# GrafikXxxxxxxYyyyyyyyyyy/StableDiffusion

Measured on AMD Instinct MI355X. Metric: denoise-loop latents/s (512px, 50-step DDIM, batch 4), higher is better.
Workload: dtype f16; 1 GPU; SD1.5 512x512, 50-step DDIM, batch 4/GPU, CFG on (UNet batch 8), UNet + VAE decode HIP kernels; global_batch=4, parallelism=dp1

## Files before the change

include/sd_engine.h:

```cpp
#ifndef SD_ENGINE_H
#define SD_ENGINE_H

#include <stdint.h>

#ifdef __cplusplus
extern "C" {
#endif

#define SD_OK 0
#define SD_ERR_INVALID 1
#define SD_ERR_STATE 2
#define SD_ERR_HIP 3
#define SD_ERR_UNSUPPORTED 4

#define SD_DTYPE_F16 0
#define SD_DTYPE_F32 1

#define SD_MAX_BLOCKS 4

typedef struct sd_unet_config {
    int32_t in_channels;
    int32_t out_channels;
    int32_t num_blocks;
    int32_t block_out_channels[SD_MAX_BLOCKS];
// ... 49 lines not shown
int sd_unet_num_weights(const sd_unet* u);
int sd_unet_weight_info(const sd_unet* u, int index, const char** key, int64_t* shape4, int* ndim);
int sd_unet_set_weight(sd_unet* u, const char* diffusers_key, const void* data,
                       const int64_t* shape, int ndim, int dtype);
int sd_unet_finalize(sd_unet* u);
int sd_unet_forward(sd_unet* u, const void* sample, const float* timesteps, const void* ehs,
                    int ehs_len, const void* add_text, const float* add_time_ids, void* out,
                    int B, int H, int W, void* stream);
int sd_unet_use_graph(sd_unet* u, int enable);
int sd_unet_text_kv_cache(sd_unet* u, int enable);
int sd_unet_forward_ex(sd_unet* u, const void* sample, const float* timesteps, const void* ehs, int ehs_len,
                       const void* add_text, const float* add_time_ids, const void* image_embeds, int n_img, void* out,
                       int B, int H, int W, void* stream);
int sd_unet_set_ip_adapter(sd_unet* u, sd_ip_adapter* adapter);
int sd_unet_set_ip_adapter_scale(sd_unet* u, float scale);
int sd_unet_set_controlnet(sd_unet* u, sd_controlnet* cn);
int sd_unet_forward_cn(sd_unet* u, const void* sample, const float* timesteps, const void* ehs, int ehs_len,
                       const void* add_text, const float* add_time_ids, const void* image_embeds, int n_img,
                       const void* control_image, int n_ctrl, float cond_scale, void* out, int B, int H, int W,
                       void* stream);
int sd_unet_forward_cfg(sd_unet* u, const void* latents, const float* timesteps, const void* ehs, int ehs_len,
                        const void* add_text, const float* add_time_ids, const void* image_embeds, int n_img,
                        float in_scale, int share, void* out, int B, int H, int W, void* stream);
int sd_unet_cfg_share(const sd_unet_config* cfg);
int sd_unet_set_freeu(sd_unet* u, int enable, float s1, float s2, float b1, float b2);
int sd_unet_memory(const sd_unet* u, int64_t* weight_bytes, int64_t* workspace_bytes);

int sd_ip_adapter_create(const sd_unet* u, int image_embed_dim, int num_tokens, sd_ip_adapter** out);
int sd_ip_adapter_destroy(sd_ip_adapter* a);
int sd_ip_adapter_num_weights(const sd_ip_adapter* a);
int sd_ip_adapter_weight_info(const sd_ip_adapter* a, int index, const char** key, int64_t* shape4, int* ndim);
int sd_ip_adapter_set_weight(sd_ip_adapter* a, const char* key, const void* data, const int64_t* shape, int ndim,
                             int dtype);
int sd_ip_adapter_finalize(sd_ip_adapter* a);

int sd_controlnet_create(const sd_unet* u, const sd_unet_config* cn_cfg, int conditioning_channels, sd_controlnet** out);
int sd_controlnet_destroy(sd_controlnet* cn);
int sd_controlnet_num_weights(const sd_controlnet* cn);
int sd_controlnet_weight_info(const sd_controlnet* cn, int index, const char** key, int64_t* shape4, int* ndim);
int sd_controlnet_set_weight(sd_controlnet* cn, const char* key, const void* data, const int64_t* shape, int ndim,
                             int dtype);
int sd_controlnet_finalize(sd_controlnet* cn);

int sd_vae_create(const sd_vae_config* cfg, sd_vae** out);
int sd_vae_destroy(sd_vae* v);
int sd_vae_num_weights(const sd_vae* v);
int sd_vae_weight_info(const sd_vae* v, int index, const char** key, int64_t* shape4, int* ndim);
int sd_vae_set_weight(sd_vae* v, const char* diffusers_key, const void* data,
                      const int64_t* shape, int ndim, int dtype);
int sd_vae_finalize(sd_vae* v);
int sd_vae_decode(sd_vae* v, const void* z, void* img, int B, int h, int w, void* stream);
int sd_vae_encode(sd_vae* v, const void* img, void* moments, int B, int H, int W, void* stream);
int sd_vae_encode_range_shift(sd_vae* v, int shift);
int sd_vae_memory(const sd_vae* v, int64_t* weight_bytes, int64_t* workspace_bytes);

int sd_clip_create(const sd_clip_config* cfg, sd_clip** out);
int sd_clip_destroy(sd_clip* c);
int sd_clip_num_weights(const sd_clip* c);
int sd_clip_weight_info(const sd_clip* c, int index, const char** key, int64_t* shape4, int* ndim);
int sd_clip_set_weight(sd_clip* c, const char* key, const void* data, const int64_t* shape, int ndim, int dtype);
int sd_clip_finalize(sd_clip* c);
int sd_clip_forward(sd_clip* c, const int32_t* input_ids, const int32_t* eos_index, void* hidden_states,
                    void* last_hidden, void* pooled, void* text_embeds, int B, int T, void* stream);
int sd_clip_final_layer_norm(sd_clip* c, const void* x, void* y, int64_t rows, void* stream);
int sd_clip_memory(const sd_clip* c, int64_t* weight_bytes, int64_t* workspace_bytes);

int sd_cfg_duplicate(const void* latents, void* out2b, int64_t n_per_batch, int B, float in_scale,
                     void* stream);
int sd_cfg_ddim_step(const void* noise_pred_2b, void* latents, int64_t n, float guidance_scale,
                     float c_x, float c_eps, void* stream);

int sd_cfg_linear_step(const void* noise_pred_2b, void* latents, float* hist_f32, int64_t n,
                       float guidance_scale, float c_x, float c_eps, float c_hist, float h_x, float h_eps,
                       void* stream);

int sd_cfg_rescale_linear_step(const void* noise_pred_2b, void* latents, float* hist_f32, int B, int64_t n_per_sample,
                               float guidance_scale, float guidance_rescale, float c_x, float c_eps, float c_hist,
                               float h_x, float h_eps, float* factors_out, void* stream);

int sd_inpaint_blend(void* latents, const void* image_latents, const void* noise, const void* mask,
                     float a, float b, int B, int C, int H, int W, void* stream);

int sd_images_to_uint8(const void* images_nchw_f16, void* out_nhwc_u8, int B, int C, int H, int W, void* stream);

typedef struct sd_prof_entry {
    char kernel[64];
    double flops;
    double bytes;
    double ms;
    int64_t launches;
} sd_prof_entry;
int sd_prof_enable(int on);
int sd_prof_collect(sd_prof_entry* out, int max_entries, int* n_entries);

int sd_probe_mfma(int iters, float* tflops, void* stream);
int sd_probe_copy(int64_t bytes, int iters, float* gbs, void* stream);
int sd_probe_lds_dma(int64_t region_bytes, int passes, int depth, int shared, float* gbs, void* stream);

int sd_igemm_force(int variant, int splits);
int sd_igemm_plan(const int* geom, const int* flags, int64_t* out, char* name);

int sd_op_conv2d(const void* x_nhwc, const void* w_oihw, const void* bias, const void* rowadd,
                 const void* res_nhwc, void* y_nhwc, int N, int H, int W, int Cin, int Cout,
                 int ksize, int stride, int upsample2x, int geglu, void* stream);
int sd_op_conv3x3_small_cout(const void* x_nhwc, const void* w_oihw, const void* bias, void* y_nchw, int N, int H,
                             int W, int Cin, int Cout, void* stream);
int sd_op_conv2d_groupnorm(const void* x_nhwc, const void* w_oihw, const void* bias, const void* rowadd,
                           const void* res_nhwc, void* y_conv_nhwc, const void* gamma, const void* beta,
                           void* y_gn_nhwc, int N, int H, int W, int Cin, int Cout, int ksize, int stride,
                           int upsample2x, int groups, float eps, int silu, int* stats_from_epilogue, void* stream);
int sd_op_groupnorm_conv2d(const void* x_nhwc, const void* gamma, const void* beta, int groups, float eps, int silu,
                           const void* w_oihw, const void* bias, const void* rowadd, const void* res_nhwc, void* y_nhwc,
                           int N, int H, int W, int Cin, int Cout, int ksize, int iters, float* ms_per_launch, int* fused,
                           void* stream);
int sd_op_unet_conv_in(const void* x_nchw, const void* w_oihw, const void* bias, void* y_nhwc, float* gn_summaries, int groups,
                       int N, int Cin, int H, int W, int Cout, int iters, float* ms_per_launch, void* stream);
int sd_op_unet_conv_out(const void* x_nhwc, const void* gamma, const void* beta, int groups, float eps, int silu,
                        const void* w_oihw, const void* bias, void* y_nchw, int N, int H, int W, int C, int Cout, int iters,
                        float* ms_per_launch, void* stream);
int sd_op_ffn_geglu(const void* x, const void* ln_gamma, const void* ln_beta, float ln_eps, const void* w1, const void* b1,
                    const void* w2, const void* b2, void* y, int M, int C, int iters, float* ms_per_launch, int* fused,
                    void* stream);
int sd_op_linear_rowstats(const void* x, const void* w0, const void* b0, const void* res, void* y1, float* stat, int M,
                          int K, int C, int* parts, int* part_w, int* producer, void* stream);
int sd_op_ln_linear(const void* y1, const float* stat, int parts, int part_w, const void* gamma, const void* beta, float eps,
                    const void* w1, const void* b1, void* y2, int M, int C, int O, int geglu, int rows_scaled, float row_scale,
                    int* consumer, void* stream);
int sd_op_ln_ffn_geglu(const void* x, const float* stat, int parts, int part_w, const void* ln_gamma, const void* ln_beta,
                       float ln_eps, const void* w1, const void* b1, const void* w2, const void* b2, void* y, int M, int C,
                       int* fused, void* stream);
int sd_bench_conv2d(const void* x_nhwc, const void* w_oihw, void* y_nhwc, int N, int H, int W, int Cin,
                    int Cout, int ksize, int stride, int upsample2x, int geglu, int iters,
                    float* ms_per_launch, void* stream);
int sd_op_groupnorm(const void* x_nhwc, const void* gamma, const void* beta, void* y_nhwc,
                    int N, int HW, int C, int groups, float eps, int silu, void* stream);
int sd_op_groupnorm_concat(const void* x_nhwc, int Ca, int Cb, const void* gamma, const void* beta, void* y_nhwc, int N, int HW,
                           int groups, float eps, int silu, void* stream);
int sd_bench_groupnorm(const void* x_nhwc, const void* gamma, const void* beta, void* y_nhwc,
                       int N, int HW, int C, int groups, float eps, int silu, int iters,
                       float* ms_per_launch, void* stream);
int sd_op_timestep_sinusoid(const float* t, float* out, int count, int dim, int flip_sin_to_cos, float freq_shift,
                            void* stream);
int sd_op_small_linear(const float* x, const void* w_f16, const float* bias, float* y, int B, int K, int n_out,
                       int silu_in, int silu_out, void* stream);
int sd_op_freeu(void* cat_nhwc, int N, int H, int W, int C1, int C2, float b, float s, void* stream);
int sd_op_layernorm(const void* x, const void* gamma, const void* beta, void* y, int rows, int C,
                    float eps, void* stream);
int sd_op_attention(const void* q, const void* k, const void* v, void* out, int B, int Tq, int Tk,
                    int heads, int d, int ldq, int ldk, int ldv, int ldo, void* stream);
int sd_op_attention_ex(const void* q, const void* k, const void* v, void* out, int B, int Tq, int Tk,
                       int heads, int d, int ldq, int ldk, int ldv, int ldo, int causal, int prescaled,
                       void* stream);
int sd_attention_plan(int B, int Tq, int Tk, int heads, int d, int causal, int prescaled, int* out5);
int sd_op_ip_cross_attention(const void* q, const void* k, const void* v, const void* k_ip, const void* v_ip, void* out,
                             int B, int Tq, int L, int T_ip, int heads, int d, int ldq, int ldk, int ldv, int ldk_ip,
                             int ldv_ip, int ldo, float ip_scale, int prescaled, int iters, float* ms_per_launch,
                             void* stream);

typedef struct sd_cn_problem {
    const void* x; int64_t ldx;
    const void* w;
    const float* bias;
    void* y; int64_t ldy;
    int M, C;
} sd_cn_problem;
int sd_op_controlnet_residuals(const sd_cn_problem* problems, int count, float scale, int mode, int iters,
                               float* ms_per_launch, void* stream);
int sd_op_controlnet_cond_embed(sd_controlnet* cn, const void* image, int n, int H, int W, void* out, int iters,
                                float* ms_per_launch, void* stream);

#ifdef __cplusplus
}
#endif
#endif
```

stablediffusion_amd/_lib.py:

```python
from __future__ import annotations

import ctypes as C
import os

_HERE = os.path.dirname(os.path.abspath(__file__))
LIB_PATH = os.path.join(_HERE, "libsd_engine.so")

SD_MAX_BLOCKS = 4
SD_DTYPE_F16 = 0
SD_DTYPE_F32 = 1


class SdUNetConfig(C.Structure):
    _fields_ = [
        ("in_channels", C.c_int32),
        ("out_channels", C.c_int32),
        ("num_blocks", C.c_int32),
        ("block_out_channels", C.c_int32 * SD_MAX_BLOCKS),
        ("down_block_has_attn", C.c_int32 * SD_MAX_BLOCKS),
        ("up_block_has_attn", C.c_int32 * SD_MAX_BLOCKS),
        ("num_heads", C.c_int32 * SD_MAX_BLOCKS),
        ("transformer_layers", C.c_int32 * SD_MAX_BLOCKS),
        ("layers_per_block", C.c_int32),
        ("cross_attention_dim", C.c_int32),
        ("use_linear_projection", C.c_int32),
        ("norm_num_groups", C.c_int32),
        ("norm_eps", C.c_float),
        ("flip_sin_to_cos", C.c_int32),
        ("freq_shift", C.c_float),
        ("addition_time_embed_dim", C.c_int32),
        ("projection_class_embeddings_input_dim", C.c_int32),
    ]


class SdVAEConfig(C.Structure):
    _fields_ = [
        ("in_channels", C.c_int32),
        ("out_channels", C.c_int32),
        ("latent_channels", C.c_int32),
        ("num_blocks", C.c_int32),
        ("block_out_channels", C.c_int32 * SD_MAX_BLOCKS),
        ("layers_per_block", C.c_int32),
        ("norm_num_groups", C.c_int32),
    ]


class SdClipConfig(C.Structure):
    _fields_ = [
        ("vocab_size", C.c_int32),
        ("hidden_size", C.c_int32),
        ("intermediate_size", C.c_int32),
        ("num_layers", C.c_int32),
        ("num_heads", C.c_int32),
        ("max_positions", C.c_int32),
        ("hidden_act", C.c_int32),
        ("projection_dim", C.c_int32),
        ("layer_norm_eps", C.c_float),
    ]


class SdProfEntry(C.Structure):
    _fields_ = [("kernel", C.c_char * 64), ("flops", C.c_double), ("bytes", C.c_double),
                ("ms", C.c_double), ("launches", C.c_int64)]


class SdCnProblem(C.Structure):
    _fields_ = [("x", C.c_void_p), ("ldx", C.c_int64), ("w", C.c_void_p), ("bias", C.c_void_p),
                ("y", C.c_void_p), ("ldy", C.c_int64), ("M", C.c_int), ("C", C.c_int)]


_P = C.c_void_p
_I = C.c_int
_I64 = C.c_int64
_F = C.c_float
SIGNATURES = {
    "sd_last_error": (C.c_char_p, []),
    "sd_engine_version": (_I, []),
    "sd_engine_arch": (C.c_char_p, []),
    "sd_unet_create": (_I, [C.POINTER(SdUNetConfig), C.POINTER(_P)]),
    "sd_unet_destroy": (_I, [_P]),
    "sd_unet_num_weights": (_I, [_P]),
    "sd_unet_weight_info": (_I, [_P, _I, C.POINTER(C.c_char_p), C.POINTER(_I64), C.POINTER(_I)]),
    "sd_unet_set_weight": (_I, [_P, C.c_char_p, _P, C.POINTER(_I64), _I, _I]),
    "sd_unet_finalize": (_I, [_P]),
    "sd_unet_forward": (_I, [_P, _P, _P, _P, _I, _P, _P, _P, _I, _I, _I, _P]),
    "sd_unet_use_graph": (_I, [_P, _I]),
    "sd_unet_text_kv_cache": (_I, [_P, _I]),
    "sd_unet_memory": (_I, [_P, C.POINTER(_I64), C.POINTER(_I64)]),
    "sd_unet_forward_ex": (_I, [_P, _P, _P, _P, _I, _P, _P, _P, _I, _P, _I, _I, _I, _P]),
    "sd_unet_forward_cfg": (_I, [_P, _P, _P, _P, _I, _P, _P, _P, _I, _F, _I, _P, _I, _I, _I, _P]),
    "sd_unet_cfg_share": (_I, [C.POINTER(SdUNetConfig)]),
    "sd_unet_set_ip_adapter": (_I, [_P, _P]),
    "sd_unet_set_ip_adapter_scale": (_I, [_P, _F]),
    "sd_unet_set_freeu": (_I, [_P, _I, _F, _F, _F, _F]),
    "sd_ip_adapter_create": (_I, [_P, _I, _I, C.POINTER(_P)]),
    "sd_ip_adapter_destroy": (_I, [_P]),
    "sd_ip_adapter_num_weights": (_I, [_P]),
    "sd_ip_adapter_weight_info": (_I, [_P, _I, C.POINTER(C.c_char_p), C.POINTER(_I64), C.POINTER(_I)]),
    "sd_ip_adapter_set_weight": (_I, [_P, C.c_char_p, _P, C.POINTER(_I64), _I, _I]),
    "sd_ip_adapter_finalize": (_I, [_P]),
    "sd_unet_set_controlnet": (_I, [_P, _P]),
    "sd_unet_forward_cn": (_I, [_P, _P, _P, _P, _I, _P, _P, _P, _I, _P, _I, _F, _P, _I, _I, _I, _P]),
    "sd_controlnet_create": (_I, [_P, C.POINTER(SdUNetConfig), _I, C.POINTER(_P)]),
    "sd_controlnet_destroy": (_I, [_P]),
    "sd_controlnet_num_weights": (_I, [_P]),
    "sd_controlnet_weight_info": (_I, [_P, _I, C.POINTER(C.c_char_p), C.POINTER(_I64), C.POINTER(_I)]),
    "sd_controlnet_set_weight": (_I, [_P, C.c_char_p, _P, C.POINTER(_I64), _I, _I]),
    "sd_controlnet_finalize": (_I, [_P]),
    "sd_vae_create": (_I, [C.POINTER(SdVAEConfig), C.POINTER(_P)]),
    "sd_vae_destroy": (_I, [_P]),
    "sd_vae_num_weights": (_I, [_P]),
    "sd_vae_weight_info": (_I, [_P, _I, C.POINTER(C.c_char_p), C.POINTER(_I64), C.POINTER(_I)]),
    "sd_vae_set_weight": (_I, [_P, C.c_char_p, _P, C.POINTER(_I64), _I, _I]),
    "sd_vae_finalize": (_I, [_P]),
    "sd_vae_decode": (_I, [_P, _P, _P, _I, _I, _I, _P]),
    "sd_vae_encode": (_I, [_P, _P, _P, _I, _I, _I, _P]),
    "sd_vae_encode_range_shift": (_I, [_P, _I]),
    "sd_vae_memory": (_I, [_P, C.POINTER(_I64), C.POINTER(_I64)]),
    "sd_clip_create": (_I, [C.POINTER(SdClipConfig), C.POINTER(_P)]),
    "sd_clip_destroy": (_I, [_P]),
    "sd_clip_num_weights": (_I, [_P]),
    "sd_clip_weight_info": (_I, [_P, _I, C.POINTER(C.c_char_p), C.POINTER(_I64), C.POINTER(_I)]),
    "sd_clip_set_weight": (_I, [_P, C.c_char_p, _P, C.POINTER(_I64), _I, _I]),
    "sd_clip_finalize": (_I, [_P]),
    "sd_clip_forward": (_I, [_P, _P, _P, _P, _P, _P, _P, _I, _I, _P]),
    "sd_clip_final_layer_norm": (_I, [_P, _P, _P, _I64, _P]),
    "sd_clip_memory": (_I, [_P, C.POINTER(_I64), C.POINTER(_I64)]),
    "sd_op_attention_ex": (_I, [_P, _P, _P, _P, _I, _I, _I, _I, _I, _I, _I, _I, _I, _I, _I, _P]),
    "sd_cfg_duplicate": (_I, [_P, _P, _I64, _I, _F, _P]),
    "sd_cfg_ddim_step": (_I, [_P, _P, _I64, _F, _F, _F, _P]),
    "sd_inpaint_blend": (_I, [_P, _P, _P, _P, _F, _F, _I, _I, _I, _I, _P]),
    "sd_images_to_uint8": (_I, [_P, _P, _I, _I, _I, _I, _P]),
    "sd_cfg_linear_step": (_I, [_P, _P, _P, _I64, _F, _F, _F, _F, _F, _F, _P]),
    "sd_cfg_rescale_linear_step": (_I, [_P, _P, _P, _I, _I64, _F, _F, _F, _F, _F, _F, _F, _P, _P]),
    "sd_igemm_force": (_I, [_I, _I]),
    "sd_igemm_plan": (_I, [C.POINTER(_I), C.POINTER(_I), C.POINTER(_I64), C.c_char_p]),
    "sd_probe_mfma": (_I, [_I, C.POINTER(_F), _P]),
    "sd_probe_lds_dma": (_I, [_I64, _I, _I, _I, C.POINTER(_F), _P]),
    "sd_probe_copy": (_I, [_I64, _I, C.POINTER(_F), _P]),
    "sd_prof_enable": (_I, [_I]),
    "sd_prof_collect": (_I, [C.POINTER(SdProfEntry), _I, C.POINTER(_I)]),
    "sd_op_conv2d": (_I, [_P, _P, _P, _P, _P, _P, _I, _I, _I, _I, _I, _I, _I, _I, _I, _P]),
    "sd_op_conv3x3_small_cout": (_I, [_P, _P, _P, _P, _I, _I, _I, _I, _I, _P]),
    "sd_op_conv2d_groupnorm": (_I, [_P, _P, _P, _P, _P, _P, _P, _P, _P, _I, _I, _I, _I, _I, _I, _I, _I, _I, _F, _I,
                                    C.POINTER(_I), _P]),
    "sd_op_groupnorm_conv2d": (_I, [_P, _P, _P, _I, _F, _I, _P, _P, _P, _P, _P, _I, _I, _I, _I, _I, _I, _I, C.POINTER(_F),
                                    C.POINTER(_I), _P]),
    "sd_op_unet_conv_in": (_I, [_P, _P, _P, _P, _P, _I, _I, _I, _I, _I, _I, _I, C.POINTER(_F), _P]),
    "sd_op_unet_conv_out": (_I, [_P, _P, _P, _I, _F, _I, _P, _P, _P, _I, _I, _I, _I, _I, _I, C.POINTER(_F), _P]),
    "sd_op_ffn_geglu": (_I, [_P, _P, _P, _F, _P, _P, _P, _P, _P, _I, _I, _I, C.POINTER(_F), C.POINTER(_I), _P]),
    "sd_op_linear_rowstats": (_I, [_P, _P, _P, _P, _P, _P, _I, _I, _I, C.POINTER(_I), C.POINTER(_I), C.POINTER(_I), _P]),
    "sd_op_ln_linear": (_I, [_P, _P, _I, _I, _P, _P, _F, _P, _P, _P, _I, _I, _I, _I, _I, _F, C.POINTER(_I), _P]),
    "sd_op_ln_ffn_geglu": (_I, [_P, _P, _I, _I, _P, _P, _F, _P, _P, _P, _P, _P, _I, _I, C.POINTER(_I), _P]),
    "sd_bench_conv2d": (_I, [_P, _P, _P, _I, _I, _I, _I, _I, _I, _I, _I, _I, _I, C.POINTER(_F), _P]),
    "sd_op_groupnorm": (_I, [_P, _P, _P, _P, _I, _I, _I, _I, _F, _I, _P]),
    "sd_op_groupnorm_concat": (_I, [_P, _I, _I, _P, _P, _P, _I, _I, _I, _F, _I, _P]),
    "sd_bench_groupnorm": (_I, [_P, _P, _P, _P, _I, _I, _I, _I, _F, _I, _I, C.POINTER(_F), _P]),
    "sd_op_timestep_sinusoid": (_I, [_P, _P, _I, _I, _I, _F, _P]),
    "sd_op_small_linear": (_I, [_P, _P, _P, _P, _I, _I, _I, _I, _I, _P]),
    "sd_op_freeu": (_I, [_P, _I, _I, _I, _I, _I, _F, _F, _P]),
    "sd_op_layernorm": (_I, [_P, _P, _P, _P, _I, _I, _F, _P]),
    "sd_op_attention": (_I, [_P, _P, _P, _P, _I, _I, _I, _I, _I, _I, _I, _I, _I, _P]),
    "sd_attention_plan": (_I, [_I, _I, _I, _I, _I, _I, _I, C.POINTER(_I)]),
    "sd_op_ip_cross_attention": (_I, [_P, _P, _P, _P, _P, _P, _I, _I, _I, _I, _I, _I, _I, _I, _I, _I, _I, _I, _F, _I, _I,
                                      C.POINTER(_F), _P]),
    "sd_op_controlnet_residuals": (_I, [C.POINTER(SdCnProblem), _I, _F, _I, _I, C.POINTER(_F), _P]),
    "sd_op_controlnet_cond_embed": (_I, [_P, _P, _I, _I, _I, _P, _I, C.POINTER(_F), _P]),
}

_lib = None


class EngineError(RuntimeError):
    pass


def load():
    global _lib
    if _lib is not None:
        return _lib
    if not os.path.exists(LIB_PATH):
        raise EngineError(
            f"{LIB_PATH} not found: build it with `python -m stablediffusion_amd.build` "
            "(hipcc --offload-arch=gfx950). The HIP engine is mandatory; there is no CPU fallback.")
    import torch
    lib = C.CDLL(LIB_PATH)
    for name, (res, args) in SIGNATURES.items():
        fn = getattr(lib, name)
        fn.restype = res
        fn.argtypes = args
    _lib = lib
    return lib


def check(rc: int, what: str = ""):
    if rc != 0:
        msg = load().sd_last_error()
        raise EngineError(f"{what}: error {rc}: {msg.decode() if msg else '?'}")


def require_gpu():
    import torch
    if not torch.cuda.is_available():
        raise EngineError("no HIP device visible: the gfx950 engine cannot run (and nothing else will run in its place)")
```

stablediffusion_amd/build.py:

```python
from __future__ import annotations

import os
import subprocess
import sys
from concurrent.futures import ThreadPoolExecutor

HERE = os.path.dirname(os.path.abspath(__file__))
CSRC = os.path.join(HERE, "csrc")
OUT = os.path.join(HERE, "libsd_engine.so")
SOURCES = ["igemm.hip", "igemm2.hip", "igemm3.hip", "wsgemm.hip", "pgemm.hip", "ffn.hip", "edge.hip", "norm.hip", "attention.hip", "ip_attention.hip", "controlnet.hip", "freeu.hip", "misc.hip", "probe.hip", "runtime.cpp", "unet.cpp", "controlnet.cpp", "vae.cpp", "clip.cpp", "capi.cpp"]
FLAGS = ["-O3", "--offload-arch=gfx950", "-fPIC", "-std=c++17", "-Wall", "-Wno-unused-function",
         "-ffp-contract=fast", "-mllvm", "-amdgpu-mfma-vgpr-form"]


def _stale(target, deps):
    if not os.path.exists(target):
        return True
    t = os.path.getmtime(target)
    return any(os.path.getmtime(d) > t for d in deps)


def build(force: bool = False, verbose: bool = False) -> str:
    hipcc = os.environ.get("HIPCC", "/opt/rocm/bin/hipcc")
    objdir = os.path.join(HERE, "build")
    os.makedirs(objdir, exist_ok=True)
    headers = [os.path.join(CSRC, f) for f in os.listdir(CSRC) if f.endswith((".h", ".inc"))]
    headers.append(os.path.join(os.path.dirname(HERE), "include", "sd_engine.h"))
    jobs = []
    objs = []
    for src in SOURCES:
        s = os.path.join(CSRC, src)
        o = os.path.join(objdir, src + ".o")
        objs.append(o)
        if force or _stale(o, [s] + headers):
            jobs.append([hipcc, *FLAGS, "-x", "hip", "-c", s, "-o", o])

    def run(cmd):
        if verbose:
            print(" ".join(cmd), flush=True)
        r = subprocess.run(cmd, capture_output=True, text=True)
        if r.returncode != 0:
            raise RuntimeError("build failed: %s\n%s\n%s" % (" ".join(cmd), r.stdout, r.stderr))
        if verbose and r.stderr.strip():
            print(r.stderr, file=sys.stderr)

    if jobs:
        with ThreadPoolExecutor(max_workers=min(8, len(jobs))) as ex:
            list(ex.map(run, jobs))
    if jobs or force or _stale(OUT, objs):
        run([hipcc, "--offload-arch=gfx950", "-shared", "-fPIC", "-o", OUT, *objs])
    return OUT


if __name__ == "__main__":
    print(build(force="--force" in sys.argv, verbose=True))
```

stablediffusion_amd/csrc/capi.cpp:

```cpp
#include <cmath>
#include <cstdio>
#include <new>

#include "model.h"
#include <cstdlib>

using namespace sd;

struct sd_unet { UNet impl; explicit sd_unet(const sd_unet_config& c) : impl(c) {} };
struct sd_vae { VAE impl; explicit sd_vae(const sd_vae_config& c) : impl(c) {} };
struct sd_clip { CLIP impl; explicit sd_clip(const sd_clip_config& c) : impl(c) {} };
struct sd_controlnet {
    ControlNet impl;
    sd_controlnet(const sd_unet_config& c, int cc) : impl(c, cc) {}
};
struct sd_ip_adapter {
    IPAdapter impl;
    sd_ip_adapter(const sd_unet_config& c, int d, int n) : impl(c, d, n) {}
    ~sd_ip_adapter() { if (impl.attached) impl.attached->set_ip_adapter(nullptr); }
};

namespace {

int weight_info(const WeightStore& ws, int index, const char** key, int64_t* shape4, int* ndim) {
    if (index < 0 || index >= (int)ws.order.size()) { set_error("weight index out of range"); return SD_ERR_INVALID; }
    const std::string& k = ws.order[(size_t)index];
    const RawTensor& t = ws.tensors.at(k);
    *key = k.c_str();
    *ndim = (int)t.shape.size();
    for (int i = 0; i < 4; ++i) shape4[i] = i < *ndim ? t.shape[(size_t)i] : 1;
    return SD_OK;
}

bool bad_cfg(const sd_unet_config* c) {
    if (!c || c->num_blocks < 1 || c->num_blocks > SD_MAX_BLOCKS) return true;
    for (int i = 0; i < c->num_blocks; ++i) {
        if (c->block_out_channels[i] % 64 != 0 || c->block_out_channels[i] % c->norm_num_groups != 0) return true;
        if (c->num_heads[i] <= 0 || c->block_out_channels[i] % c->num_heads[i] != 0) return true;
        if ((c->down_block_has_attn[i] || c->up_block_has_attn[c->num_blocks - 1 - i]) &&
            !attention_supported(c->block_out_channels[i] / c->num_heads[i])) return true;
    }
    if (c->addition_time_embed_dim > 0) {
        const int ad = c->addition_time_embed_dim, pin = c->projection_class_embeddings_input_dim;
        if ((ad & 1) || pin % 64 != 0 || pin - 6 * ad <= 0) return true;
    }
    return c->cross_attention_dim % 64 != 0 || c->in_channels <= 0 || c->in_channels > 16;
}

bool same_topology(const sd_unet_config& a, const sd_unet_config& b) {
    if (a.in_channels != b.in_channels || a.out_channels != b.out_channels || a.num_blocks != b.num_blocks ||
        a.layers_per_block != b.layers_per_block || a.cross_attention_dim != b.cross_attention_dim ||
        a.use_linear_projection != b.use_linear_projection || a.norm_num_groups != b.norm_num_groups ||
        a.norm_eps != b.norm_eps || a.flip_sin_to_cos != b.flip_sin_to_cos || a.freq_shift != b.freq_shift ||
        a.addition_time_embed_dim != b.addition_time_embed_dim ||
        a.projection_class_embeddings_input_dim != b.projection_class_embeddings_input_dim)
        return false;
    for (int i = 0; i < SD_MAX_BLOCKS; ++i)
        if (a.block_out_channels[i] != b.block_out_channels[i] || a.down_block_has_attn[i] != b.down_block_has_attn[i] ||
            a.up_block_has_attn[i] != b.up_block_has_attn[i] || a.num_heads[i] != b.num_heads[i] ||
            a.transformer_layers[i] != b.transformer_layers[i])
            return false;
    return true;
}

bool controlnet_fits(const sd_unet_config& u, const sd_unet_config& n, std::string* why) {
    if (n.num_blocks != u.num_blocks || n.layers_per_block != u.layers_per_block) {
        *why = "num_blocks / layers_per_block differ from the UNet's";
        return false;
    }
    for (int i = 0; i < u.num_blocks; ++i)
        if (n.block_out_channels[i] != u.block_out_channels[i]) { *why = "block_out_channels differ from the UNet's"; return false; }
    if (n.cross_attention_dim != u.cross_attention_dim) { *why = "cross_attention_dim differs from the UNet's"; return false; }
    if (n.in_channels != u.in_channels) { *why = "in_channels differs from the UNet's (9-channel inpaint UNets take no ControlNet)"; return false; }
    if (n.addition_time_embed_dim != u.addition_time_embed_dim ||
        n.projection_class_embeddings_input_dim != u.projection_class_embeddings_input_dim) {
        *why = "text_time conditioning differs from the UNet's";
        return false;
    }
    return true;
}

}

extern "C" {

const char* sd_last_error(void) { return sd::last_error().c_str(); }
int sd_engine_version(void) { return 1; }
const char* sd_engine_arch(void) { return "gfx950"; }

int sd_unet_create(const sd_unet_config* cfg, sd_unet** out) {
    if (!out) { set_error("null out"); return SD_ERR_INVALID; }
    if (bad_cfg(cfg)) {
        set_error("sd_unet_create: unsupported config (channels must be multiples of 64 and of the group "
                  "count, head dims in {32,40,64,80,128,160}, cross_attention_dim % 64 == 0, text_time: even "
                  "addition_time_embed_dim and projection_class_embeddings_input_dim % 64 == 0 and > 6 x it)");
        return SD_ERR_UNSUPPORTED;
    }
    *out = new (std::nothrow) sd_unet(*cfg);
    if (!*out) { set_error("out of host memory"); return SD_ERR_INVALID; }
    return SD_OK;
}
int sd_unet_destroy(sd_unet* u) { delete u; return SD_OK; }
int sd_unet_num_weights(const sd_unet* u) { return u ? (int)u->impl.ws.order.size() : 0; }
int sd_unet_weight_info(const sd_unet* u, int index, const char** key, int64_t* shape4, int* ndim) {
    if (!u) { set_error("null handle"); return SD_ERR_INVALID; }
    return weight_info(u->impl.ws, index, key, shape4, ndim);
}
int sd_unet_set_weight(sd_unet* u, const char* key, const void* data, const int64_t* shape, int ndim, int dtype) {
    if (!u || !key || !data || !shape) { set_error("null argument"); return SD_ERR_INVALID; }
    if (u->impl.finalized) { set_error("set_weight after finalize"); return SD_ERR_STATE; }
    return u->impl.ws.set(key, data, shape, ndim, dtype);
}
int sd_unet_finalize(sd_unet* u) {
    if (!u) { set_error("null handle"); return SD_ERR_INVALID; }
    return u->impl.finalize();
}
int sd_unet_forward(sd_unet* u, const void* sample, const float* timesteps, const void* ehs, int ehs_len,
                    const void* add_text, const float* add_time_ids, void* out, int B, int H, int W,
                    void* stream) {
    if (!u || !sample || !timesteps || !ehs || !out) { set_error("null argument"); return SD_ERR_INVALID; }
    return u->impl.forward(static_cast<const half_t*>(sample), timesteps, static_cast<const half_t*>(ehs),
                           ehs_len, static_cast<const half_t*>(add_text), add_time_ids,
                           static_cast<half_t*>(out), B, H, W, static_cast<hipStream_t>(stream));
}
int sd_unet_use_graph(sd_unet* u, int enable) {
    if (!u) { set_error("null handle"); return SD_ERR_INVALID; }
    u->impl.graph_enabled = enable != 0;
    return SD_OK;
}
int sd_unet_text_kv_cache(sd_unet* u, int enable) {
    if (!u) { set_error("null handle"); return SD_ERR_INVALID; }
    u->impl.kv_cache_on = enable != 0;
    u->impl.kv_valid = false;
    u->impl.ipkv_valid = false;
    u->impl.cond_valid = false;
    u->impl.cnkv_valid = false;
    return SD_OK;
}
int sd_unet_forward_ex(sd_unet* u, const void* sample, const float* timesteps, const void* ehs, int ehs_len,
                       const void* add_text, const float* add_time_ids, const void* image_embeds, int n_img, void* out,
                       int B, int H, int W, void* stream) {
    if (!u || !sample || !timesteps || !ehs || !out) { set_error("null argument"); return SD_ERR_INVALID; }
    return u->impl.forward(static_cast<const half_t*>(sample), timesteps, static_cast<const half_t*>(ehs),
                           ehs_len, static_cast<const half_t*>(add_text), add_time_ids,
                           static_cast<half_t*>(out), B, H, W, static_cast<hipStream_t>(stream),
                           static_cast<const half_t*>(image_embeds), image_embeds ? n_img : 0);
}
int sd_unet_set_ip_adapter(sd_unet* u, sd_ip_adapter* a) {
    if (!u) { set_error("null handle"); return SD_ERR_INVALID; }
    if (a) {
        if (!a->impl.finalized) { set_error("sd_unet_set_ip_adapter: adapter not finalized"); return SD_ERR_STATE; }
        if (!same_topology(a->impl.cfg, u->impl.cfg)) {
            set_error("sd_unet_set_ip_adapter: the adapter was created for another UNet configuration");
            return SD_ERR_INVALID;
        }
    }
    u->impl.set_ip_adapter(a ? &a->impl : nullptr);
    return SD_OK;
}
int sd_unet_set_controlnet(sd_unet* u, sd_controlnet* cn) {
    if (!u) { set_error("null handle"); return SD_ERR_INVALID; }
    if (cn) {
        if (!cn->impl.finalized) { set_error("sd_unet_set_controlnet: ControlNet not finalized"); return SD_ERR_STATE; }
        std::string why;
        if (!controlnet_fits(u->impl.cfg, cn->impl.cfg, &why)) { set_error("sd_unet_set_controlnet: " + why); return SD_ERR_INVALID; }
    }
    u->impl.set_controlnet(cn ? &cn->impl : nullptr);
    return SD_OK;
}
int sd_unet_forward_cn(sd_unet* u, const void* sample, const float* timesteps, const void* ehs, int ehs_len,
                       const void* add_text, const float* add_time_ids, const void* image_embeds, int n_img,
                       const void* control_image, int n_ctrl, float cond_scale, void* out, int B, int H, int W,
                       void* stream) {
    if (!u || !sample || !timesteps || !ehs || !out) { set_error("null argument"); return SD_ERR_INVALID; }
    return u->impl.forward(static_cast<const half_t*>(sample), timesteps, static_cast<const half_t*>(ehs),
                           ehs_len, static_cast<const half_t*>(add_text), add_time_ids,
                           static_cast<half_t*>(out), B, H, W, static_cast<hipStream_t>(stream),
                           static_cast<const half_t*>(image_embeds), image_embeds ? n_img : 0,
                           static_cast<const half_t*>(control_image), control_image ? n_ctrl : 0, cond_scale);
}
int sd_unet_forward_cfg(sd_unet* u, const void* latents, const float* timesteps, const void* ehs, int ehs_len,
                        const void* add_text, const float* add_time_ids, const void* image_embeds, int n_img,
                        float in_scale, int share, void* out, int B, int H, int W, void* stream) {
    if (!u || !latents || !timesteps || !ehs || !out) { set_error("null argument"); return SD_ERR_INVALID; }
    if (!(in_scale == in_scale)) { set_error("sd_unet_forward_cfg: in_scale is NaN"); return SD_ERR_INVALID; }
    return u->impl.forward_cfg(static_cast<const half_t*>(latents), timesteps, static_cast<const half_t*>(ehs), ehs_len,
                               static_cast<const half_t*>(add_text), add_time_ids,
                               static_cast<const half_t*>(image_embeds), image_embeds ? n_img : 0, in_scale, share != 0,
                               static_cast<half_t*>(out), B, H, W, static_cast<hipStream_t>(stream));
}
int sd_unet_cfg_share(const sd_unet_config* cfg) { return cfg && sd::unet_cfg_share_eligible(*cfg) ? 1 : 0; }
int sd_unet_set_ip_adapter_scale(sd_unet* u, float scale) {
    if (!u) { set_error("null handle"); return SD_ERR_INVALID; }
    if (!(scale == scale)) { set_error("sd_unet_set_ip_adapter_scale: NaN"); return SD_ERR_INVALID; }
    u->impl.ip_scale = scale;
    return SD_OK;
}
int sd_unet_set_freeu(sd_unet* u, int enable, float s1, float s2, float b1, float b2) {
    if (!u) { set_error("null handle"); return SD_ERR_INVALID; }
    if (!enable) { u->impl.freeu_on = false; return SD_OK; }
    if (!std::isfinite(s1) || !std::isfinite(s2) || !std::isfinite(b1) || !std::isfinite(b2)) {
        set_error("sd_unet_set_freeu: s1, s2, b1, b2 must be finite");
        return SD_ERR_INVALID;
    }
    u->impl.freeu_on = true;
    u->impl.freeu_s1 = s1; u->impl.freeu_s2 = s2; u->impl.freeu_b1 = b1; u->impl.freeu_b2 = b2;
    return SD_OK;
}

int sd_ip_adapter_create(const sd_unet* u, int image_embed_dim, int num_tokens, sd_ip_adapter** out) {
    if (!u || !out) { set_error("null argument"); return SD_ERR_INVALID; }
    const sd_unet_config& c = u->impl.cfg;
    if (c.cross_attention_dim % 64 != 0) { set_error("sd_ip_adapter_create: cross_attention_dim % 64 != 0"); return SD_ERR_UNSUPPORTED; }
    if (num_tokens < 1 || num_tokens > 16) { set_error("sd_ip_adapter_create: num_tokens must be in [1, 16]"); return SD_ERR_UNSUPPORTED; }
    if (image_embed_dim <= 0 || image_embed_dim % 64 != 0) {
        set_error("sd_ip_adapter_create: image_embed_dim must be a positive multiple of 64");
        return SD_ERR_UNSUPPORTED;
    }
    for (const auto& site : unet_xattn_sites(c, true)) {
        int heads = 0;
        for (int i = 0; i < c.num_blocks; ++i)
            if (c.block_out_channels[i] == site.second) heads = c.num_heads[i];
        if (heads <= 0 || !ip_attention_supported(site.second / heads)) {
            set_error("sd_ip_adapter_create: head dim of " + site.first + " not in {32, 40, 64, 80, 160}");
            return SD_ERR_UNSUPPORTED;
        }
    }
    *out = new (std::nothrow) sd_ip_adapter(c, image_embed_dim, num_tokens);
    if (!*out) { set_error("out of host memory"); return SD_ERR_INVALID; }
    return SD_OK;
}
int sd_ip_adapter_destroy(sd_ip_adapter* a) { delete a; return SD_OK; }
int sd_ip_adapter_num_weights(const sd_ip_adapter* a) { return a ? (int)a->impl.ws.order.size() : 0; }
int sd_ip_adapter_weight_info(const sd_ip_adapter* a, int index, const char** key, int64_t* shape4, int* ndim) {
    if (!a) { set_error("null handle"); return SD_ERR_INVALID; }
    return weight_info(a->impl.ws, index, key, shape4, ndim);
}
int sd_ip_adapter_set_weight(sd_ip_adapter* a, const char* key, const void* data, const int64_t* shape, int ndim,
                             int dtype) {
    if (!a || !key || !data || !shape) { set_error("null argument"); return SD_ERR_INVALID; }
    if (a->impl.finalized) { set_error("set_weight after finalize"); return SD_ERR_STATE; }
    return a->impl.ws.set(key, data, shape, ndim, dtype);
}
int sd_ip_adapter_finalize(sd_ip_adapter* a) {
    if (!a) { set_error("null handle"); return SD_ERR_INVALID; }
    return a->impl.finalize();
}
int sd_controlnet_create(const sd_unet* u, const sd_unet_config* cn_cfg, int conditioning_channels, sd_controlnet** out) {
    if (!u || !cn_cfg || !out) { set_error("null argument"); return SD_ERR_INVALID; }
    if (conditioning_channels != 3) { set_error("sd_controlnet_create: conditioning_channels must be 3"); return SD_ERR_UNSUPPORTED; }
    sd_unet_config c = *cn_cfg;
    for (int i = 0; i < SD_MAX_BLOCKS; ++i) c.up_block_has_attn[i] = 0;
    if (bad_cfg(&c)) { set_error("sd_controlnet_create: unsupported encoder configuration"); return SD_ERR_UNSUPPORTED; }
    std::string why;
    if (!controlnet_fits(u->impl.cfg, c, &why)) { set_error("sd_controlnet_create: " + why); return SD_ERR_INVALID; }
    if (u->impl.cfg.in_channels != 4) { set_error("sd_controlnet_create: the UNet must take 4 latent channels"); return SD_ERR_INVALID; }
    if (1 + c.num_blocks * c.layers_per_block + (c.num_blocks - 1) + 1 > kCnMaxProblems) {
        set_error("sd_controlnet_create: more residual sites than one grouped launch takes (16)");
        return SD_ERR_UNSUPPORTED;
    }
    *out = new (std::nothrow) sd_controlnet(c, conditioning_channels);
    if (!*out) { set_error("out of host memory"); return SD_ERR_INVALID; }
    return SD_OK;
}
int sd_controlnet_destroy(sd_controlnet* cn) { delete cn; return SD_OK; }
int sd_controlnet_num_weights(const sd_controlnet* cn) { return cn ? (int)cn->impl.ws.order.size() : 0; }
int sd_controlnet_weight_info(const sd_controlnet* cn, int index, const char** key, int64_t* shape4, int* ndim) {
    if (!cn) { set_error("null handle"); return SD_ERR_INVALID; }
    return weight_info(cn->impl.ws, index, key, shape4, ndim);
}
int sd_controlnet_set_weight(sd_controlnet* cn, const char* key, const void* data, const int64_t* shape, int ndim,
                             int dtype) {
    if (!cn || !key || !data || !shape) { set_error("null argument"); return SD_ERR_INVALID; }
    if (cn->impl.finalized) { set_error("set_weight after finalize"); return SD_ERR_STATE; }
    return cn->impl.ws.set(key, data, shape, ndim, dtype);
}
int sd_controlnet_finalize(sd_controlnet* cn) {
    if (!cn) { set_error("null handle"); return SD_ERR_INVALID; }
    return cn->impl.finalize();
}
int sd_unet_memory(const sd_unet* u, int64_t* weight_bytes, int64_t* workspace_bytes) {
    if (!u) { set_error("null handle"); return SD_ERR_INVALID; }
    if (weight_bytes) *weight_bytes = u->impl.ws.packed_bytes();
    if (workspace_bytes) *workspace_bytes = (int64_t)u->impl.arena.capacity();
    return SD_OK;
}

int sd_vae_create(const sd_vae_config* cfg, sd_vae** out) {
    if (!out || !cfg) { set_error("null argument"); return SD_ERR_INVALID; }
    bool bad = cfg->num_blocks < 1 || cfg->num_blocks > SD_MAX_BLOCKS || cfg->latent_channels > 8;
    for (int i = 0; !bad && i < cfg->num_blocks; ++i)
        bad = cfg->block_out_channels[i] % 64 != 0;
    if (!bad) bad = !attention_supported(cfg->block_out_channels[cfg->num_blocks - 1]);
    if (bad) { set_error("sd_vae_create: unsupported config"); return SD_ERR_UNSUPPORTED; }
    *out = new (std::nothrow) sd_vae(*cfg);
    if (!*out) { set_error("out of host memory"); return SD_ERR_INVALID; }
    return SD_OK;
}
int sd_vae_destroy(sd_vae* v) { delete v; return SD_OK; }
int sd_vae_num_weights(const sd_vae* v) { return v ? (int)v->impl.ws.order.size() : 0; }
int sd_vae_weight_info(const sd_vae* v, int index, const char** key, int64_t* shape4, int* ndim) {
    if (!v) { set_error("null handle"); return SD_ERR_INVALID; }
    return weight_info(v->impl.ws, index, key, shape4, ndim);
}
int sd_vae_set_weight(sd_vae* v, const char* key, const void* data, const int64_t* shape, int ndim, int dtype) {
    if (!v || !key || !data || !shape) { set_error("null argument"); return SD_ERR_INVALID; }
    if (v->impl.finalized) { set_error("set_weight after finalize"); return SD_ERR_STATE; }
    return v->impl.ws.set(key, data, shape, ndim, dtype);
}
int sd_vae_finalize(sd_vae* v) {
    if (!v) { set_error("null handle"); return SD_ERR_INVALID; }
    return v->impl.finalize();
}
int sd_vae_decode(sd_vae* v, const void* z, void* img, int B, int h, int w, void* stream) {
    if (!v || !z || !img) { set_error("null argument"); return SD_ERR_INVALID; }
    return v->impl.decode(static_cast<const half_t*>(z), static_cast<half_t*>(img), B, h, w,
                          static_cast<hipStream_t>(stream));
}
int sd_vae_encode(sd_vae* v, const void* img, void* moments, int B, int H, int W, void* stream) {
    if (!v || !img || !moments) { set_error("null argument"); return SD_ERR_INVALID; }
    return v->impl.encode(static_cast<const half_t*>(img), static_cast<half_t*>(moments), B, H, W,
                          static_cast<hipStream_t>(stream));
}
int sd_vae_encode_range_shift(sd_vae* v, int shift) {
    if (!v || shift < 0 || shift > 14) { set_error("sd_vae_encode_range_shift: shift in 0..14"); return SD_ERR_INVALID; }
    v->impl.encode_shift = shift;
    return SD_OK;
}
int sd_vae_memory(const sd_vae* v, int64_t* weight_bytes, int64_t* workspace_bytes) {
    if (!v) { set_error("null handle"); return SD_ERR_INVALID; }
    if (weight_bytes) *weight_bytes = v->impl.ws.packed_bytes();
    if (workspace_bytes) *workspace_bytes = (int64_t)v->impl.arena.capacity();
    return SD_OK;
}

int sd_clip_create(const sd_clip_config* cfg, sd_clip** out) {
    if (!out || !cfg) { set_error("null argument"); return SD_ERR_INVALID; }
    const bool bad = cfg->vocab_size < 1 || cfg->num_layers < 1 || cfg->num_heads < 1 || cfg->max_positions < 1 ||
                     cfg->hidden_size % 64 != 0 || cfg->intermediate_size % 64 != 0 || cfg->hidden_size > 2048 ||
                     cfg->hidden_size % cfg->num_heads != 0 || !attention_supported(cfg->hidden_size / cfg->num_heads) ||
                     (cfg->hidden_act != 0 && cfg->hidden_act != 1) || cfg->projection_dim < 0;
    if (bad) { set_error("sd_clip_create: unsupported config (hidden / intermediate % 64, head dim, activation)"); return SD_ERR_UNSUPPORTED; }
    *out = new (std::nothrow) sd_clip(*cfg);
    if (!*out) { set_error("out of host memory"); return SD_ERR_INVALID; }
    return SD_OK;
}
int sd_clip_destroy(sd_clip* c) { delete c; return SD_OK; }
// ... 608 lines not shown
    const int n = timed ? iters + 2 : 1;
    for (int it = 0; it < n && !rc; ++it) {
        if (timed && it == 2) SD_HIP_CHECK(hipEventRecord(e0, s));
        rc = launch_conv_tail(p, s);
    }
    if (timed && !rc) {
        SD_HIP_CHECK(hipEventRecord(e1, s));
        SD_HIP_CHECK(hipEventSynchronize(e1));
        float ms = 0.f;
        SD_HIP_CHECK(hipEventElapsedTime(&ms, e0, e1));
        *ms_per_launch = ms / (float)iters;
    }
    if (e0) { (void)hipEventDestroy(e0); (void)hipEventDestroy(e1); }
    hipError_t e = hipStreamSynchronize(s);
    if (!rc && e != hipSuccess) { set_error(hipGetErrorString(e)); rc = SD_ERR_HIP; }
    return rc;
}

int sd_bench_conv2d(const void* x, const void* w_oihw, void* y, int N, int H, int W, int Cin, int Cout, int ksize,
                    int stride, int upsample2x, int geglu, int iters, float* ms_per_launch, void* stream) {
    if (iters < 1 || !ms_per_launch) { set_error("sd_bench_conv2d: bad arguments"); return SD_ERR_INVALID; }
    return conv2d_impl(x, w_oihw, nullptr, nullptr, nullptr, y, N, H, W, Cin, Cout, ksize, stride, upsample2x, geglu,
                       stream, iters, ms_per_launch);
}

int sd_op_groupnorm(const void* x, const void* gamma_f32, const void* beta_f32, void* y, int N, int HW, int C,
                    int groups, float eps, int silu, void* stream) {
    hipStream_t s = static_cast<hipStream_t>(stream);
    DevScope scope;
    float* scratch = nullptr;
    SD_DEV_ALLOC(scope, scratch, (size_t)gn_scratch_floats(N, HW, C, groups) * 4);
    int rc = launch_groupnorm(static_cast<const half_t*>(x), C, static_cast<const float*>(gamma_f32),
                              static_cast<const float*>(beta_f32), static_cast<half_t*>(y), C, N, HW, C, groups,
                              eps, silu, scratch, s);
    hipError_t e = hipStreamSynchronize(s);
    if (!rc && e != hipSuccess) { set_error(hipGetErrorString(e)); rc = SD_ERR_HIP; }
    return rc;
}

int sd_op_groupnorm_concat(const void* x, int Ca, int Cb, const void* gamma_f32, const void* beta_f32, void* y, int N, int HW,
                           int groups, float eps, int silu, void* stream) {
    hipStream_t s = static_cast<hipStream_t>(stream);
    const int C = Ca + Cb;
    if (!x || !gamma_f32 || !beta_f32 || !y || Ca < 8 || Cb < 8 || groups < 1 || C % groups != 0 || Cb % groups != 0) {
        set_error("sd_op_groupnorm_concat: bad arguments"); return SD_ERR_INVALID;
    }
    const int u = gn_cat_unit(Ca, Cb, groups), ub = Cb / groups;
    if (!(u >= 8 || u == 4) || (C / groups) % ub != 0 || Ca % ub != 0 || !(ub >= 8 || ub == 4)) {
        set_error("sd_op_groupnorm_concat: the halves' sub-groups do not tile the groups"); return SD_ERR_INVALID;
    }
    const int Ga = Ca / u;
    DevScope scope;
    float *sa = nullptr, *sb = nullptr, *fin = nullptr, *scratch = nullptr;
    SD_DEV_ALLOC(scope, sa, (size_t)gn_scratch_floats(N, HW, Ca, Ga) * 4);
    SD_DEV_ALLOC(scope, sb, (size_t)gn_scratch_floats(N, HW, Cb, groups) * 4);
    SD_DEV_ALLOC(scope, fin, (size_t)N * groups * 2 * 4);
    SD_DEV_ALLOC(scope, scratch, (size_t)gn_scratch_floats(N, HW, C, groups) * 4);
    const half_t* xh = static_cast<const half_t*>(x);
    GnStats sta, stb, stc;
    int rc = launch_gn_stats(xh, C, N, HW, Ca, Ga, sa, &sta, s);
    if (!rc) rc = launch_gn_stats(xh + Ca, C, N, HW, Cb, groups, sb, &stb, s);
    if (!rc) rc = launch_gn_cat_finalize(sta, Ga, Ca, stb, groups, Cb, fin, N, HW, groups, s);
    stc.part = fin; stc.S = 1; stc.rows = HW;
    if (!rc) rc = launch_groupnorm(xh, C, static_cast<const float*>(gamma_f32), static_cast<const float*>(beta_f32),
                                   static_cast<half_t*>(y), C, N, HW, C, groups, eps, silu, scratch, s, &stc);
    hipError_t e = hipStreamSynchronize(s);
    if (!rc && e != hipSuccess) { set_error(hipGetErrorString(e)); rc = SD_ERR_HIP; }
    return rc;
}

int sd_bench_groupnorm(const void* x, const void* gamma_f32, const void* beta_f32, void* y, int N, int HW, int C,
                       int groups, float eps, int silu, int iters, float* ms_per_launch, void* stream) {
    if (iters < 1 || !ms_per_launch) { set_error("sd_bench_groupnorm: bad arguments"); return SD_ERR_INVALID; }
    hipStream_t s = static_cast<hipStream_t>(stream);
    DevScope scope;
    float* scratch = nullptr;
    SD_DEV_ALLOC(scope, scratch, (size_t)gn_scratch_floats(N, HW, C, groups) * 4);
    hipEvent_t e0, e1;
    SD_HIP_CHECK(hipEventCreate(&e0));
    SD_HIP_CHECK(hipEventCreate(&e1));
    int rc = 0;
    static const bool apply_only = getenv("SD_GN_BENCH_APPLY") != nullptr;
    GnStats st;
    float* scratch2 = nullptr;
    if (apply_only && gn_wants_stats(HW, C, groups)) {
        SD_DEV_ALLOC(scope, scratch2, (size_t)gn_scratch_floats(N, HW, C, groups) * 4);
        rc = launch_gn_stats(static_cast<const half_t*>(x), C, N, HW, C, groups, scratch2, &st, s);
    }
    for (int i = 0; i < iters + 2 && !rc; ++i) {
        if (i == 2) (void)hipEventRecord(e0, s);
        rc = launch_groupnorm(static_cast<const half_t*>(x), C, static_cast<const float*>(gamma_f32),
                              static_cast<const float*>(beta_f32), static_cast<half_t*>(y), C, N, HW, C, groups,
                              eps, silu, scratch, s, st.part ? &st : nullptr);
    }
    (void)hipEventRecord(e1, s);
    hipError_t e = hipEventSynchronize(e1);
    float ms = 0.f;
    if (e == hipSuccess) e = hipEventElapsedTime(&ms, e0, e1);
    *ms_per_launch = ms / iters;
    (void)hipEventDestroy(e0);
    (void)hipEventDestroy(e1);
    if (!rc && e != hipSuccess) { set_error(hipGetErrorString(e)); rc = SD_ERR_HIP; }
    return rc;
}

int sd_op_timestep_sinusoid(const float* t, float* out, int count, int dim, int flip_sin_to_cos, float freq_shift,
                            void* stream) {
    if (!t || !out || count < 1 || dim < 2 || (dim & 1)) { set_error("sd_op_timestep_sinusoid: bad arguments"); return SD_ERR_INVALID; }
    return launch_timestep_sinusoid(t, 1, out, count, dim, flip_sin_to_cos, freq_shift, dim, static_cast<hipStream_t>(stream));
}

int sd_op_small_linear(const float* x, const void* w_f16, const float* bias, float* y, int B, int K, int n_out, int silu_in,
                       int silu_out, void* stream) {
    if (!x || !w_f16 || !y || B < 1 || K < 1 || n_out < 1) { set_error("sd_op_small_linear: bad arguments"); return SD_ERR_INVALID; }
    return launch_small_linear(x, K, static_cast<const half_t*>(w_f16), bias, y, n_out, B, K, n_out, silu_in, silu_out,
                               static_cast<hipStream_t>(stream));
}

int sd_op_layernorm(const void* x, const void* gamma_f32, const void* beta_f32, void* y, int rows, int C, float eps,
                    void* stream) {
    return launch_layernorm(static_cast<const half_t*>(x), C, static_cast<const float*>(gamma_f32),
                            static_cast<const float*>(beta_f32), static_cast<half_t*>(y), C, rows, C, eps,
                            static_cast<hipStream_t>(stream));
}

int sd_op_freeu(void* cat_nhwc, int N, int H, int W, int C1, int C2, float b, float s, void* stream) {
    if (!cat_nhwc) { set_error("sd_op_freeu: null argument"); return SD_ERR_INVALID; }
    return launch_freeu(static_cast<half_t*>(cat_nhwc), (long)C1 + C2, N, H, W, C1, C2, b, s, static_cast<hipStream_t>(stream));
}

int sd_op_attention(const void* q, const void* k, const void* v, void* out, int B, int Tq, int Tk, int heads, int d,
                    int ldq, int ldk, int ldv, int ldo, void* stream) {
    return launch_attention(static_cast<const half_t*>(q), static_cast<const half_t*>(k),
                            static_cast<const half_t*>(v), static_cast<half_t*>(out), B, Tq, Tk, heads, d, ldq, ldk,
                            ldv, ldo, static_cast<hipStream_t>(stream));
}

int sd_op_attention_ex(const void* q, const void* k, const void* v, void* out, int B, int Tq, int Tk, int heads, int d,
                       int ldq, int ldk, int ldv, int ldo, int causal, int prescaled, void* stream) {
    return launch_attention(static_cast<const half_t*>(q), static_cast<const half_t*>(k),
                            static_cast<const half_t*>(v), static_cast<half_t*>(out), B, Tq, Tk, heads, d, ldq, ldk,
                            ldv, ldo, static_cast<hipStream_t>(stream), causal, prescaled);
}

int sd_attention_plan(int B, int Tq, int Tk, int heads, int d, int causal, int prescaled, int* out5) {
    if (!out5) { set_error("sd_attention_plan: null argument"); return SD_ERR_INVALID; }
    const AttnPlan pl = attention_plan(B, Tq, Tk, heads, d, causal, prescaled);
    if (pl.D == 0) { set_error("attention: unsupported head dim " + std::to_string(d)); return SD_ERR_UNSUPPORTED; }
    const int o[5] = {pl.D, pl.QT, pl.KT, pl.PRESC, pl.NWV};
    for (int i = 0; i < 5; ++i) out5[i] = o[i];
    return SD_OK;
}

int sd_op_ip_cross_attention(const void* q, const void* k, const void* v, const void* k_ip, const void* v_ip, void* out,
                             int B, int Tq, int L, int T_ip, int heads, int d, int ldq, int ldk, int ldv, int ldk_ip,
                             int ldv_ip, int ldo, float ip_scale, int prescaled, int iters, float* ms_per_launch,
                             void* stream) {
    const half_t *qh = static_cast<const half_t*>(q), *kh = static_cast<const half_t*>(k), *vh = static_cast<const half_t*>(v);
    const half_t *kih = static_cast<const half_t*>(k_ip), *vih = static_cast<const half_t*>(v_ip);
    half_t* oh = static_cast<half_t*>(out);
    hipStream_t s = static_cast<hipStream_t>(stream);
    auto fused = [&]() {
        return launch_ip_attention(qh, kh, vh, kih, vih, oh, B, Tq, L, T_ip, heads, d, ldq, ldk, ldv, ldk_ip, ldv_ip, ldo,
                                   ip_scale, prescaled, s);
    };
    int rc = fused();
    if (rc || iters <= 0) return rc;
    if (!ms_per_launch) { set_error("sd_op_ip_cross_attention: ms_per_launch required with iters > 0"); return SD_ERR_INVALID; }
    if (!attention_supported(d)) { set_error("sd_op_ip_cross_attention: timing needs a head dim of the text kernel"); return SD_ERR_UNSUPPORTED; }
    half_t* tmp = nullptr;
    SD_HIP_CHECK(hipMalloc(reinterpret_cast<void**>(&tmp), (size_t)B * Tq * heads * d * sizeof(half_t)));
    const long ldt = (long)heads * d;
    auto text = [&]() {
        return launch_attention(qh, kh, vh, oh, B, Tq, L, heads, d, ldq, ldk, ldv, ldo, s, 0, prescaled);
    };
    auto unfused = [&]() {
        int r = text();
        if (!r) r = launch_attention(qh, kih, vih, tmp, B, Tq, T_ip, heads, d, ldq, ldk_ip, ldv_ip, ldt, s, 0, prescaled);
        if (!r) r = launch_axpy_f16(oh, ldo, tmp, ldt, (long)B * Tq, heads * d, ip_scale, s);
        return r;
    };
    hipEvent_t e0 = nullptr, e1 = nullptr;
    if (hipEventCreate(&e0) != hipSuccess || hipEventCreate(&e1) != hipSuccess) rc = SD_ERR_HIP;
    for (int variant = 0; variant < 3 && !rc; ++variant) {
        auto one = [&]() { return variant == 0 ? fused() : variant == 1 ? text() : unfused(); };
        for (int it = 0; it < 2 && !rc; ++it) rc = one();
        if (rc) break;
        (void)hipEventRecord(e0, s);
        for (int it = 0; it < iters && !rc; ++it) rc = one();
        (void)hipEventRecord(e1, s);
        float ms = 0.f;
        hipError_t e = hipEventSynchronize(e1);
        if (e == hipSuccess) e = hipEventElapsedTime(&ms, e0, e1);
        if (e != hipSuccess) { set_error(hipGetErrorString(e)); rc = SD_ERR_HIP; }
        ms_per_launch[variant] = ms / (float)iters;
    }
    if (!rc) rc = fused();
    if (!rc && hipStreamSynchronize(s) != hipSuccess) rc = SD_ERR_HIP;
    if (e0) (void)hipEventDestroy(e0);
    if (e1) (void)hipEventDestroy(e1);
    (void)hipFree(tmp);
    return rc;
}

}

namespace {
template <class F>
int run_op_on_arena(hipStream_t s, int iters, float* ms, F body) {
    Arena arena;
    Ctx dry{&arena, s, true};
    arena.begin(true);
    body(dry);
    if (dry.err) return dry.err;
    if (int rc = arena.reserve(arena.peak() > 0 ? arena.peak() : 256)) return rc;
    auto live = [&]() {
        Ctx c{&arena, s, false};
        arena.begin(false);
        body(c);
        return c.err;
    };
    int rc = live();
    if (!rc && iters > 0) {
        if (!ms) { set_error("ms_per_launch required with iters > 0"); return SD_ERR_INVALID; }
        hipEvent_t e0 = nullptr, e1 = nullptr;
        if (hipEventCreate(&e0) != hipSuccess || hipEventCreate(&e1) != hipSuccess) rc = SD_ERR_HIP;
        if (!rc) rc = live();
        if (!rc) (void)hipEventRecord(e0, s);
        for (int it = 0; it < iters && !rc; ++it) rc = live();
        if (!rc) {
            (void)hipEventRecord(e1, s);
            float t = 0.f;
            hipError_t e = hipEventSynchronize(e1);
            if (e == hipSuccess) e = hipEventElapsedTime(&t, e0, e1);
            if (e != hipSuccess) { set_error(hipGetErrorString(e)); rc = SD_ERR_HIP; }
            *ms = t / (float)iters;
        }
        if (e0) (void)hipEventDestroy(e0);
        if (e1) (void)hipEventDestroy(e1);
    }
    const hipError_t e = hipStreamSynchronize(s);
    if (!rc && e != hipSuccess) { set_error(hipGetErrorString(e)); rc = SD_ERR_HIP; }
    return rc;
}
}

extern "C" {

int sd_op_controlnet_residuals(const sd_cn_problem* problems, int count, float scale, int mode, int iters,
                               float* ms_per_launch, void* stream) {
    if (!problems || count < 1 || count > kCnMaxProblems) { set_error("sd_op_controlnet_residuals: 1..16 problems"); return SD_ERR_INVALID; }
    if (mode != 0 && mode != 1) { set_error("sd_op_controlnet_residuals: mode must be 0 (grouped) or 1 (unfused)"); return SD_ERR_INVALID; }
    hipStream_t s = static_cast<hipStream_t>(stream);
    CnResParams rp;
    rp.scale = scale;
    for (int i = 0; i < count; ++i) {
        const sd_cn_problem& q = problems[i];
        CnResProblem& d = rp.p[rp.count++];
        d.x = static_cast<const half_t*>(q.x); d.ldx = q.ldx; d.w = static_cast<const half_t*>(q.w); d.bias = q.bias;
        d.y = static_cast<half_t*>(q.y); d.ldy = q.ldy; d.M = q.M; d.C = q.C; d.first = rp.total;
        if (q.C <= 0 || q.C % 64 != 0 || q.M <= 0) { set_error("sd_op_controlnet_residuals: C % 64 == 0 and M >= 1 required"); return SD_ERR_UNSUPPORTED; }
        rp.total += cn_residual_tiles(q.M, q.C);
    }
    if (!cn_residual_supported(rp)) { set_error("sd_op_controlnet_residuals: unsupported strides or alignment"); return SD_ERR_UNSUPPORTED; }
    if (mode == 0) return run_op_on_arena(s, iters, ms_per_launch, [&](Ctx& c) { if (!c.dry) c.err = launch_cn_residual(rp, s); });
    std::vector<ConvW> ws((size_t)count);
    std::vector<void*> owned;
    int rc = 0;
    for (int i = 0; i < count && !rc; ++i) {
        const sd_cn_problem& q = problems[i];
        const long rows = ((long)q.C + kWeightRowPad - 1) / kWeightRowPad * kWeightRowPad;
        void *w = nullptr, *b = nullptr;
        if (hipMalloc(&w, (size_t)rows * q.C * sizeof(half_t)) != hipSuccess || hipMalloc(&b, (size_t)rows * sizeof(float)) != hipSuccess) {
            set_error("sd_op_controlnet_residuals: out of device memory"); rc = SD_ERR_HIP;
        }
        if (w) owned.push_back(w);
        if (b) owned.push_back(b);
        if (rc) break;
        if (hipMemsetAsync(w, 0, (size_t)rows * q.C * sizeof(half_t), s) != hipSuccess ||
            hipMemsetAsync(b, 0, (size_t)rows * sizeof(float), s) != hipSuccess ||
            hipMemcpyAsync(w, q.w, (size_t)q.C * q.C * sizeof(half_t), hipMemcpyDeviceToDevice, s) != hipSuccess ||
            hipMemcpyAsync(b, q.bias, (size_t)q.C * sizeof(float), hipMemcpyDeviceToDevice, s) != hipSuccess) {
            set_error("sd_op_controlnet_residuals: copy failed"); rc = SD_ERR_HIP;
        }
        ConvW& cw = ws[(size_t)i];
        cw.w = static_cast<half_t*>(w); cw.bias = static_cast<float*>(b); cw.cin = q.C; cw.cout = q.C; cw.ks = 1; cw.K = q.C;
    }
    if (!rc && scale != 0.f)
        rc = run_op_on_arena(s, iters, ms_per_launch, [&](Ctx& c) {
            for (int i = 0; i < count; ++i) {
                const sd_cn_problem& q = problems[i];
                View y(static_cast<half_t*>(q.y), q.ldy, q.C);
                ConvFuse f;
                f.acc_scale = scale; f.bias_scale = scale;
                op_conv(c, ws[(size_t)i], View(const_cast<half_t*>(static_cast<const half_t*>(q.x)), q.ldx, q.C), 1, q.M, 1,
                        y, 1, 0, nullptr, 0, &y, 0, -1, 0, &f);
            }
        });
    (void)hipStreamSynchronize(s);
    for (void* p : owned) (void)hipFree(p);
    return rc;
}

int sd_op_controlnet_cond_embed(sd_controlnet* cn, const void* image, int n, int H, int W, void* out, int iters,
                                float* ms_per_launch, void* stream) {
    if (!cn || !image || !out) { set_error("null argument"); return SD_ERR_INVALID; }
// ... 10 lines not shown
```

stablediffusion_amd/csrc/controlnet.cpp:

```cpp
#include "model.h"

namespace sd {

namespace {
const char* kCond = "controlnet_cond_embedding";
const int kCondOut[ControlNet::kCondLayers] = {16, 16, 32, 32, 96, 96, 256};
const int kCondStride[ControlNet::kCondLayers] = {1, 1, 2, 1, 2, 1, 2};
std::string cond_name(int l) { return l == 0 ? std::string(kCond) + ".conv_in" : std::string(kCond) + ".blocks." + std::to_string(l - 1); }
}

ControlNet::ControlNet(const sd_unet_config& c, int conditioning_channels) : Encoder(c), cond_channels(conditioning_channels) {
    declare_encoder();
    int cin = cond_channels;
    for (int l = 0; l < kCondLayers; ++l) {
        cond_cin[l] = cin; cond_cout[l] = kCondOut[l]; cond_stride[l] = kCondStride[l];
        ws.declare(cond_name(l) + ".weight", {kCondOut[l], cin, 3, 3});
        ws.declare(cond_name(l) + ".bias", {kCondOut[l]});
        cin = kCondOut[l];
    }
    const int c0 = cfg.block_out_channels[0];
    ws.declare(std::string(kCond) + ".conv_out.weight", {c0, cin, 3, 3});
    ws.declare(std::string(kCond) + ".conv_out.bias", {c0});
    int si = 0;
    auto zc = [&](int C) {
        const std::string p = "controlnet_down_blocks." + std::to_string(si++);
        ws.declare(p + ".weight", {C, C, 1, 1});
        ws.declare(p + ".bias", {C});
    };
    zc(c0);
    for (int i = 0; i < cfg.num_blocks; ++i) {
        for (int j = 0; j < cfg.layers_per_block; ++j) zc(cfg.block_out_channels[i]);
        if (i != cfg.num_blocks - 1) zc(cfg.block_out_channels[i]);
    }
    const int mid = cfg.block_out_channels[cfg.num_blocks - 1];
    ws.declare("controlnet_mid_block.weight", {mid, mid, 1, 1});
    ws.declare("controlnet_mid_block.bias", {mid});
}

ControlNet::~ControlNet() {
    if (attached) attached->set_controlnet(nullptr);
}

int ControlNet::finalize() {
    if (finalized) return 0;
    std::string missing;
    if (!ws.complete(&missing)) { set_error("controlnet finalize: weight not set: " + missing); return 2; }
    int rc;
    std::vector<std::string> tw, tb;
    temb_total = 0;
    kv_total = 0;
    kv_keys.clear();
    if ((rc = pack_encoder(&tw, &tb))) return rc;
    for (int l = 0; l < kCondLayers; ++l) {
        cond_w[l] = static_cast<float*>(ws.dmalloc((size_t)cond_cout[l] * cond_cin[l] * 9 * sizeof(float)));
        cond_b[l] = static_cast<float*>(ws.dmalloc((size_t)cond_cout[l] * sizeof(float)));
        if (!cond_w[l] || !cond_b[l]) return 3;
        if ((rc = launch_cn_pack_cond(ws.raw(cond_name(l) + ".weight")->dev, cond_w[l], cond_cout[l], cond_cin[l], 0))) return rc;
        if ((rc = launch_f16_to_f32(ws.raw(cond_name(l) + ".bias")->dev, cond_b[l], cond_cout[l], 0))) return rc;
    }
    if ((rc = ws.pack_conv(std::string(kCond) + ".conv_out", &cond_out))) return rc;
    zero.assign((size_t)num_skips(), ConvW());
    for (int si = 0; si < num_skips(); ++si)
        if ((rc = ws.pack_conv("controlnet_down_blocks." + std::to_string(si), &zero[(size_t)si]))) return rc;
    if ((rc = ws.pack_conv("controlnet_mid_block", &zero_mid))) return rc;
    if ((rc = ws.pack_rows(tw, tb, &temb_stack))) return rc;
    if (!kv_keys.empty() && (rc = ws.pack_rows(kv_keys, {}, &kv_all))) return rc;
    kv_keys.clear();
    SD_HIP_CHECK(hipDeviceSynchronize());
    ws.free_raw();
    finalized = true;
    return 0;
}

void ControlNet::run_cond_embed(Ctx& c, const half_t* image, int n, int H, int W, View out) {
    Arena& a = *c.arena;
    const size_t mk = a.mark();
    const half_t* x = image;
    int ih = 8 * H, iw = 8 * W;
    for (int l = 0; l < kCondLayers; ++l) {
        CnCondConvParams p;
        p.x = x; p.nchw = l == 0;
        p.w = cond_w[l]; p.bias = cond_b[l];
        p.N = n; p.IH = ih; p.IW = iw; p.Cin = cond_cin[l]; p.Cout = cond_cout[l]; p.stride = cond_stride[l]; p.silu = 1;
        p.OH = (ih - 1) / p.stride + 1; p.OW = (iw - 1) / p.stride + 1;
        half_t* y = a.alloc_h((long)n * p.OH * p.OW * p.Cout);
        p.y = y;
        if (!c.dry && !c.err) {
            const double M = (double)n * p.OH * p.OW;
            prof_open(c.stream, "cn_cond_conv_kernel", 2.0 * M * p.Cout * 9.0 * p.Cin, 2.0 * (M * p.Cout + (double)n * ih * iw * p.Cin));
            c.err = launch_cn_cond_conv(p, c.stream);
            prof_close(c.stream);
        }
        x = y; ih = p.OH; iw = p.OW;
    }
    op_conv(c, cond_out, View(const_cast<half_t*>(x), cond_cout[kCondLayers - 1], cond_cout[kCondLayers - 1]), n, H, W, out);
    a.release(mk);
}

int ControlNet::run(Ctx& c, const half_t* sample, const float* timesteps, View text_kv, int L, const half_t* add_text,
                    const float* add_time_ids, int B, int H, int W, View emb, const std::vector<View>& sites, View mid) {
    Arena& a = *c.arena;
    const int G = cfg.norm_num_groups;
    const size_t mk = a.mark();
    float* tproj = nullptr;
    if (int rc = run_temb(c, timesteps, add_text, add_time_ids, B, &tproj)) return rc;
    ctx_gnpool_init(c, B, (long)H * W, G);
    auto stat = [&](int, long HW, int C) -> GnStatBuf* { return gn_wants_stats(HW, C, G) ? ctx_gnbuf(c) : nullptr; };
    GnStatBuf* xs = nullptr;
    run_conv_in(c, sample, B, H, W, sites[0], stat(0, (long)H * W, cfg.block_out_channels[0]), &emb, &xs);
    int h = H, w = W;
    View x = run_down(c, sites[0], xs, B, h, w, text_kv, L, tproj, [&](int si) { return sites[(size_t)si]; }, stat);
    run_mid(c, x, xs, B, h, w, text_kv, L, tproj, mid);
    a.release(mk);
    return c.err;
}

void UNet::set_controlnet(ControlNet* n) {
    if (cn == n) return;
    if (cn) cn->attached = nullptr;
    if (n) {
        if (n->attached && n->attached != this) n->attached->set_controlnet(nullptr);
        n->attached = this;
    }
    cn = n;
    cond_valid = false;
    cnkv_valid = false;
    planned_key = -1;
}

int UNet::run_controlnet(Ctx& c, const half_t* sample, const float* timesteps, const half_t* ehs, int L,
                         const half_t* add_text, const float* add_time_ids, int B, int H, int W, const half_t* control,
                         int n_ctrl, const std::vector<View>& sites, View mid) {
    Arena& a = *c.arena;
    const bool go = !c.dry;
    hipStream_t s = c.stream;
    const int C0 = cn->cfg.block_out_channels[0];
    const long HWC = (long)H * W * C0;
    const bool cached = kv_cache_on && !graph_enabled && cond_cache != nullptr;
    half_t* cond = cached ? cond_cache : a.alloc_h((long)B * HWC);
    const bool hit = cached && cond_valid && cond_src == control && cond_B == B && cond_n == n_ctrl && cond_H == H &&
                     cond_W == W;
    if (c.dry || !hit) {
        cn->run_cond_embed(c, control, n_ctrl, H, W, View(cond, C0, C0));
        for (int b = n_ctrl; b < B && go && !c.err; b += n_ctrl) {
            const hipError_t e = hipMemcpyAsync(cond + (long)b * HWC, cond, (size_t)n_ctrl * HWC * sizeof(half_t),
                                                hipMemcpyDeviceToDevice, s);
            if (e != hipSuccess) { set_error(hipGetErrorString(e)); c.err = 3; }
        }
        if (cached && go && !c.err) { cond_valid = true; cond_src = control; cond_B = B; cond_n = n_ctrl; cond_H = H; cond_W = W; }
    }
    const int ctx = cfg.cross_attention_dim;
    const bool kc = kv_cache_on && !graph_enabled && cnkv_cache != nullptr;
    View kv(kc ? cnkv_cache : a.alloc_h((long)B * L * cn->kv_total), cn->kv_total, cn->kv_total);
    const bool khit = kc && cnkv_valid && cnkv_src == ehs && cnkv_B == B && cnkv_L == L;
    if (c.dry || !khit) {
        op_conv(c, cn->kv_all, View(const_cast<half_t*>(ehs), ctx, ctx), B, L, 1, kv);
        if (kc && go && !c.err) { cnkv_valid = true; cnkv_src = ehs; cnkv_B = B; cnkv_L = L; }
    }
    const View ip_kv = c.ip_kv;
    c.ip_kv = View();
    const int rc = cn->run(c, sample, timesteps, kv, L, add_text, add_time_ids, B, H, W, View(cond, C0, C0), sites, mid);
    c.ip_kv = ip_kv;
    return rc;
}

}
```

stablediffusion_amd/csrc/engine.h:

```cpp
#pragma once
#include <map>
#include <string>
#include <unordered_map>
#include <vector>

#include "kernels.h"

namespace sd {

struct View {
    half_t* p = nullptr;
    long ld = 0;
    int C = 0;
    View() {}
    View(half_t* p_, long ld_, int C_) : p(p_), ld(ld_), C(C_) {}
    View slice(int c0, int c) const { return View(p + c0, ld, c); }
};

class Arena {
  public:
    ~Arena();
    int reserve(size_t bytes);
    void begin(bool dry) { dry_ = dry; off_ = 0; if (dry) peak_ = 0; }
    void* alloc(size_t bytes);
    half_t* alloc_h(long n) { return static_cast<half_t*>(alloc((size_t)n * sizeof(half_t))); }
    float* alloc_f(long n) { return static_cast<float*>(alloc((size_t)n * sizeof(float))); }
    size_t mark() const { return off_; }
    void release(size_t m) { off_ = m; }
    size_t peak() const { return peak_; }
    size_t capacity() const { return cap_; }
    bool dry() const { return dry_; }
    bool overflow() const { return overflow_; }

  private:
    char* base_ = nullptr;
    size_t cap_ = 0, off_ = 0, peak_ = 0;
    bool dry_ = false, overflow_ = false;
};

struct ConvW {
    half_t* w = nullptr;
    float* bias = nullptr;
    int cin = 0, cout = 0, ks = 1;
    long K = 0;
    float* wsum = nullptr;
};
struct RowStat {
    float* p = nullptr;
    int parts = 0;
    int width = 0;
};
struct GnStatBuf {
    float* buf = nullptr;
    GnStats st;
};
struct ConvFuse {
    const RowStat* ln_in = nullptr;
    float ln_eps = 0.f;
    RowStat* stat_out = nullptr;
    GnStatBuf* gn_out = nullptr;
    int gn_groups = 0;
    const struct NormW* gn_in = nullptr;
    GnStats gn_in_stats;
    int gn_in_groups = 0;
    float gn_in_eps = 0.f;
    int gn_in_silu = 0;
    float acc_scale = 1.f, bias_scale = 1.f;
};
struct NormW {
    float* gamma = nullptr;
    float* beta = nullptr;
    float* gb = nullptr;
    int C = 0;
};

struct RawTensor {
    std::vector<int64_t> shape;
    half_t* dev = nullptr;
    long numel = 0;
};

class WeightStore {
  public:
    ~WeightStore();
    void declare(const std::string& key, std::vector<int64_t> shape);
    int set(const std::string& key, const void* data, const int64_t* shape, int ndim, int dtype);
    bool complete(std::string* missing) const;
    const RawTensor* raw(const std::string& key) const;
    int pack_conv(const std::string& prefix, ConvW* out, bool has_bias = true);
    int pack_rows(const std::vector<std::string>& weight_keys, const std::vector<std::string>& bias_keys,
                  ConvW* out);
    int pack_geglu(const std::string& prefix, ConvW* out);
    int pack_norm(const std::string& prefix, NormW* out);
    int fold_ln(ConvW* w, const NormW& ln, int rows_scaled, float row_scale);
    void free_raw();
    void* dmalloc(size_t bytes);
    int64_t packed_bytes() const { return packed_bytes_; }

    std::vector<std::string> order;
    std::unordered_map<std::string, RawTensor> tensors;

  private:
    int host_floats(const std::string& key, std::vector<float>* out) const;
    std::vector<void*> owned_;
    int64_t packed_bytes_ = 0;
};

struct Ctx {
    Arena* arena;
    hipStream_t stream;
    bool dry;
    int err = 0;
    static constexpr int kGnPool = 4;
    GnStatBuf gnpool[kGnPool];
    int gn_next = 0;
    int gn_groups = 0;
    View ip_kv;
    int ip_T = 0;
    float ip_scale = 1.f;
};
void ctx_gnpool_init(Ctx& c, int N, long HW_max, int G);
GnStatBuf* ctx_gnbuf(Ctx& c);

struct ProfAgg { double flops = 0, bytes = 0, ms = 0; long launches = 0; };
void prof_enable(bool on);
bool prof_enabled();
void prof_open(hipStream_t s, const char* kernel, double flops, double bytes);
void prof_close(hipStream_t s);
int prof_collect(std::map<std::string, ProfAgg>* out);

void op_conv(Ctx& c, const ConvW& w, View x, int N, int H, int W, View y, int stride = 1, int up = 0,
             const float* rowadd = nullptr, int rowadd_ld = 0, const View* res = nullptr, int geglu = 0,
             int pad = -1, int act = 0, const ConvFuse* fuse = nullptr);
inline long rowstat_floats(long M, int C) { return M * ((C + 63) / 64) * 2; }
inline long gnstat_floats(int N, long HW, int G) { const long t = (HW + 63) / 64; return (long)N * (t > 64 ? t : 64) * G * 2; }
void op_groupnorm(Ctx& c, const NormW& n, View x, View y, int N, long HW, int G, float eps, int silu,
                  const GnStatBuf* pre = nullptr);
void op_gn_conv(Ctx& c, const NormW& n, const ConvW& w, View x, int N, int H, int W, View y, int G, float eps, int silu,
                const GnStatBuf* pre, const float* rowadd = nullptr, int rowadd_ld = 0, const View* res = nullptr,
                const ConvFuse* fuse = nullptr);
void op_layernorm(Ctx& c, const NormW& n, View x, View y, long rows, float eps);
bool op_ffn_fused(Ctx& c, const ConvW& ff1, const ConvW& ff2, View x, const RowStat& x_stat, float ln_eps, long M, View y);
void op_attention(Ctx& c, View q, View k, View v, View out, int B, int Tq, int Tk, int heads, int d, int causal = 0,
                  int prescaled = 0);
void op_ip_attention(Ctx& c, View q, View k, View v, View k_ip, View v_ip, View out, int B, int Tq, int L, int T_ip,
                     int heads, int d, float ip_scale);

}
```

stablediffusion_amd/csrc/kernels.h:

```cpp
#pragma once
#include "common.h"

namespace sd {

struct IGemmParams {
    const half_t* x; long ldx;
    const half_t* w;
    const float* bias;
    const float* rowadd; int rowadd_ld;
    const half_t* res; long ldres;
    half_t* y; long ldy;
    int N, H, W, Cin;
    int OH, OW, Cout;
    int KS, stride, pad, up;
    int M, K;
    int geglu;
    int mfast = 0;
    int act = 0;
    float* rowstat_out = nullptr;
    int rowstat_parts = 0;
    const float* ln_stat = nullptr;
    int ln_parts = 0, ln_C = 0, ln_part_w = 0;
    float ln_eps = 0.f;
    const float* ln_wsum = nullptr;
    float* gnstat_out = nullptr;
    int gn_groups = 0;
    const float* gni_part = nullptr;
    int gni_S = 0;
    long gni_rows = 0;
    int gni_groups = 0;
    float gni_eps = 0.f;
    int gni_silu = 0;
    const float* gni_gb = nullptr;
    int dbg_unchecked = 0;
    float acc_scale = 1.f, bias_scale = 1.f;
};
bool igemm2_gn_fusable(const IGemmParams& p, int groups);
int launch_igemm(const IGemmParams& p, hipStream_t s);
const char* igemm_variant(const IGemmParams& p);
bool igemm2_supported(const IGemmParams& p);
void igemm2_force(int variant, int splits);
struct IGemmRequest {
    float* rowstat = nullptr;
    float* gnstat = nullptr;
    int gn_groups = 0;
    bool no_workspace = false;
};
constexpr int kKindPgemmGeglu = 100;
constexpr int kKindIgemm1 = -1;
constexpr int kKindBadVariant = -2;
struct IGemmPlan {
    int kind = kKindIgemm1;
    int variant = -1;
    int splits = 1;
    long partial_floats = 0;
    int bm = 0, bn = 0;
    bool rowstats = false;
    int rs_parts = 1, rs_part_w = 0;
    bool gnstats = false;
    int gn_rows = 0;
    bool scales_ok = false;
    char name[64] = "";
};
IGemmPlan igemm2_plan(IGemmParams& p, const IGemmRequest& rq = IGemmRequest());
int launch_igemm2(const IGemmParams& p, float* partial, hipStream_t s, const IGemmPlan* plan = nullptr);
bool igemm3_supported(const IGemmParams& p);
int launch_igemm3(const IGemmParams& p, int mfast, hipStream_t s);
constexpr int kWeightRowPad = 256;
bool wsgemm_supported(const IGemmParams& p);
int wsgemm_rowstat_parts(const IGemmParams& p);
int launch_wsgemm(const IGemmParams& p, hipStream_t s);
bool pgemm_geglu_supported(const IGemmParams& p);
int launch_pgemm_geglu(const IGemmParams& p, hipStream_t s);

struct FfnParams {
    const half_t* x; long ldx;
    half_t* y; long ldy;
    const half_t* w1; const float* b1; const float* wsum1; int w1_rows;
    const half_t* w2; const float* b2; int w2_rows;
    const float* ln_stat; int ln_parts; float ln_eps;
    int M, C, hidden;
    int ln_part_w;
};
bool ffn_fused_supported(const FfnParams& p);
int launch_ffn_fused(const FfnParams& p, hipStream_t s);

long gn_scratch_floats(int N, long HW, int C, int G);
struct GnStats {
    const float* part = nullptr;
    int S = 0;
    long rows = 0;
};
bool gn_wants_stats(long HW, int C, int G);
int launch_groupnorm(const half_t* x, long ldx, const float* gamma, const float* beta,
                     half_t* y, long ldy, int N, long HW, int C, int G, float eps, int silu,
                     float* scratch, hipStream_t s, const GnStats* pre = nullptr);
int launch_gn_stats(const half_t* x, long ldx, int N, long HW, int C, int G, float* scratch, GnStats* st, hipStream_t s);
int launch_gn_finalize(GnStats* st, float* out, int N, long HW, int C, int G, hipStream_t s);
int gn_cat_unit(int Ca, int Cb, int G);
int launch_gn_cat_finalize(const GnStats& sa, int Ga, int Ca, const GnStats& sb, int Gb, int Cb, float* out, int N, long HW, int G,
                           hipStream_t s);
int launch_layernorm(const half_t* x, long ldx, const float* gamma, const float* beta,
                     half_t* y, long ldy, long rows, int C, float eps, hipStream_t s);
int launch_row_stats(const half_t* x, long ldx, float* stat, long rows, int C, hipStream_t s);
int launch_ln_fold(half_t* w, long K, int rows, const float* gamma, const float* beta, const float* bias_in,
                   float* bias, float* wsum, int rows_scaled, float row_scale, hipStream_t s);

int launch_attention(const half_t* q, const half_t* k, const half_t* v, half_t* out,
                     int B, int Tq, int Tk, int heads, int d,
                     long ldq, long ldk, long ldv, long ldo, hipStream_t s, int causal = 0, int prescaled = 0);
bool attention_supported(int d);
struct AttnPlan { int D, QT, KT, PRESC, NWV; };
AttnPlan attention_plan(int B, int Tq, int Tk, int heads, int d, int causal, int prescaled);
int launch_ip_attention(const half_t* q, const half_t* k, const half_t* v, const half_t* kip, const half_t* vip,
                        half_t* out, int B, int Tq, int L, int Tip, int heads, int d, long ldq, long ldk, long ldv,
                        long ldki, long ldvi, long ldo, float ip_scale, int prescaled, hipStream_t s);
bool ip_attention_supported(int d);
int launch_axpy_f16(half_t* y, long ldy, const half_t* x, long ldx, long rows, int cols, float a, hipStream_t s);

constexpr int kCnMaxProblems = 16;
struct CnResProblem {
    const half_t* x = nullptr; long ldx = 0;
    const half_t* w = nullptr;
    const float* bias = nullptr;
    half_t* y = nullptr; long ldy = 0;
    int M = 0, C = 0;
    int first = 0;
};
struct CnResParams {
    CnResProblem p[kCnMaxProblems];
    int count = 0, total = 0;
    float scale = 1.f;
};
int cn_residual_tiles(int M, int C);
bool cn_residual_supported(const CnResParams& p);
int launch_cn_residual(const CnResParams& p, hipStream_t s);
struct CnCondConvParams {
    const half_t* x = nullptr; int nchw = 0;
    const float* w = nullptr; const float* bias = nullptr;
    half_t* y = nullptr;
    int N = 0, IH = 0, IW = 0, Cin = 0, OH = 0, OW = 0, Cout = 0, stride = 1, silu = 1;
};
bool cn_cond_conv_supported(const CnCondConvParams& p);
int launch_cn_cond_conv(const CnCondConvParams& p, hipStream_t s);
int launch_cn_pack_cond(const half_t* w_oihw, float* out, int O, int I, hipStream_t s);

int launch_freeu(half_t* x, long ld, int N, int H, int W, int C1, int C2, float b, float s, hipStream_t st);

int launch_timestep_sinusoid(const float* t, int t_stride, float* out, int count, int dim, int flip, float shift,
                             long out_ld, hipStream_t s);
int launch_small_linear(const float* x, long ldx, const half_t* w, const float* bias, float* y,
                        long ldy, int B, int K, int Nout, int silu_in, int silu_out, hipStream_t s);
int launch_add_f32(float* y, const float* x, long n, int silu, hipStream_t s);
int launch_f16_to_f32(const half_t* x, float* y, long n, hipStream_t s);
int launch_f32_to_f16(const float* x, half_t* y, long n, hipStream_t s);
int launch_im2col_nchw3x3(const half_t* x, half_t* col, int N, int C, int H, int W, int Kpad,
                          hipStream_t s);
int launch_nhwc_to_nchw(const half_t* x, long ldx, half_t* y, int N, long HW, int C, hipStream_t s);
int launch_nchw_to_nhwc(const half_t* x, half_t* y, long ldy, int N, long HW, int C, hipStream_t s);
int launch_pointwise_nchw(const half_t* x, const half_t* w, const float* bias, half_t* y, int N,
                          int Cin, int Cout, long HW, hipStream_t s);
constexpr long kSmallCoutMinPixels = 131072;
int launch_conv3x3_small_cout(const half_t* x, long ldx, const half_t* w, long K, const float* bias, half_t* y_nchw,
                              int N, int H, int W, int Cin, int Cout, hipStream_t s);
struct HeadParams {
    const half_t* x_nchw = nullptr;
    const half_t* w = nullptr; long K = 0;
    const float* bias = nullptr;
    half_t* y = nullptr; long ldy = 0;
    float* gnstat_out = nullptr; int G = 0;
    int N = 0, Cin = 0, H = 0, W = 0, Cout = 0;
};
bool conv_head_supported(const HeadParams& p);
int launch_conv_head(const HeadParams& p, hipStream_t s);
struct TailParams {
    const half_t* x = nullptr; long ldx = 0;
    const float* gn_part = nullptr; int gn_S = 0; long gn_rows = 0;
    int G = 0; float eps = 0.f; const float* gamma = nullptr; const float* beta = nullptr; int silu = 0;
    const half_t* w = nullptr; long K = 0; const float* bias = nullptr;
    half_t* y = nullptr;
    int N = 0, H = 0, W = 0, C = 0, Cout = 0;
};
bool conv_tail_supported(const TailParams& p);
int launch_conv_tail(const TailParams& p, hipStream_t s);
int launch_pack_conv(const half_t* w_oihw, half_t* wp, int O, int I, int KH, int KW, long Kpad,
                     hipStream_t s);
int launch_cfg_duplicate(const half_t* lat, half_t* out, long n_total, float scale, hipStream_t s);
constexpr int kRowDupMax = 8;
struct RowDupSeg {
    const void* src = nullptr;
    void* dst = nullptr;
    long ld_bytes = 0, row_bytes = 0, rows = 0;
};
int launch_row_dup(const RowDupSeg* segs, int count, hipStream_t s);
int launch_scale_copy_f16(const half_t* x, half_t* out, long n, float scale, hipStream_t s);
int launch_dup_f32(const float* x, float* out, long n, hipStream_t s);
int launch_clip_embed(const int* ids, const half_t* tok, const half_t* pos, half_t* out, int B, int T, int H, int vocab,
                      hipStream_t s);
int launch_gather_rows(const half_t* x, long ldx, const int* idx, half_t* out16, float* out32, int B, int T, int H,
                       hipStream_t s);
int launch_inpaint_blend(half_t* lat, const half_t* img, const half_t* noise, const half_t* mask, float a, float b, int B,
                         int C, long HW, hipStream_t s);
int launch_scale_f16(half_t* x, long n, float scale, hipStream_t s);
int launch_image_to_uint8(const half_t* img, unsigned char* out, int B, int C, long HW, hipStream_t s);
int launch_cfg_linear(const half_t* eps2b, half_t* lat, float* hist, long n, float g, float cx, float ce, float ch,
                      float hx, float he, hipStream_t s);
int launch_cfg_ddim(const half_t* eps2b, half_t* lat, long n, float g, float cx, float ce,
                    hipStream_t s);
int launch_cfg_rescale_linear(const half_t* eps2b, half_t* lat, float* hist, int B, long n, float g, float phi, float cx,
                              float ce, float ch, float hx, float he, float* factors, hipStream_t s);

int probe_mfma(int iters, float* tflops, hipStream_t s);
int probe_copy(long bytes, int iters, float* gbs, hipStream_t s);
int probe_dma(long region_bytes, int passes, int depth, int shared, float* gbs, hipStream_t s);

}
```

stablediffusion_amd/csrc/model.h:

```cpp
#pragma once
#include "../../include/sd_engine.h"
#include "engine.h"

#include <functional>

namespace sd {

const std::string& last_error();

struct Resnet {
    NormW n1, n2;
    ConvW c1, c2, sc;
    bool has_sc = false;
    int temb_off = -1;
    int cin = 0, cout = 0;
};
struct TBlock {
    NormW ln1, ln2, ln3;
    ConvW qkv, out1, q2, out2, ff1, ff2;
    int kv_off = 0;
    int ip_kv_off = 0;
    bool fold = false;
};
struct Xformer {
    NormW gn;
    ConvW pin, pout;
    std::vector<TBlock> blocks;
    int C = 0, heads = 1;
};
struct VaeAttn {
    NormW gn;
    ConvW qkv, out;
    int C = 0;
};

struct CfgShare {
    std::vector<RowDupSeg> segs;
};

void run_resnet(Ctx& c, const Resnet& r, View x, int N, int H, int W, View out, int G, float eps,
                const float* tproj, int tproj_ld, const GnStatBuf* x_stats = nullptr, GnStatBuf** out_stats = nullptr,
                float stream_scale = 1.f, GnStatBuf* out_buf = nullptr, int out_groups = 0);
void run_xformer(Ctx& c, const Xformer& t, View x, int N, int H, int W, View out, int G, View text_kv, int L,
                 const GnStatBuf* x_stats = nullptr, GnStatBuf** out_stats = nullptr, GnStatBuf* out_buf = nullptr,
                 int out_groups = 0, const CfgShare* share = nullptr);

struct UNet;

std::vector<std::pair<std::string, int>> unet_xattn_sites(const sd_unet_config& cfg, bool mid_last);

struct IPAdapter {
    IPAdapter(const sd_unet_config& c, int image_embed_dim, int num_tokens);
    int finalize();

    sd_unet_config cfg;
    int d_img = 0, n_tok = 0;
    WeightStore ws;
    bool finalized = false;
    ConvW proj;
    NormW norm;
    ConvW kv_all;
    int kv_total = 0;
    UNet* attached = nullptr;
};

struct Encoder {
    explicit Encoder(const sd_unet_config& c) : cfg(c) {}

    sd_unet_config cfg;
    WeightStore ws;
    ConvW conv_in, te1, te2, ae1, ae2, temb_stack;
    ConvW kv_all;
    std::vector<std::string> kv_keys;
    std::vector<std::vector<Resnet>> down_res;
    std::vector<std::vector<Xformer>> down_att;
    std::vector<ConvW> down_ds;
    Resnet mid_r0, mid_r1;
    Xformer mid_att;
    int temb_total = 0;
    int kv_total = 0;

    int num_skips() const;
    using SkipDst = std::function<View(int si)>;
    using SkipStat = std::function<GnStatBuf*(int si, long HW, int C)>;

  protected:
    void declare_encoder();
    int pack_encoder(std::vector<std::string>* tw, std::vector<std::string>* tb);
    int pack_resnet(const std::string& p, Resnet* r, std::vector<std::string>* tw, std::vector<std::string>* tb);
    int pack_xformer(const std::string& p, Xformer* x, int heads, int depth);
    int run_temb(Ctx& c, const float* timesteps, const half_t* add_text, const float* add_time_ids, int B, float** tproj,
                 int rows_alloc = 0);
    void run_conv_in(Ctx& c, const half_t* sample, int B, int H, int W, View y0, GnStatBuf* gb, const View* res,
                     GnStatBuf** xs);
    View run_down(Ctx& c, View x, GnStatBuf*& xs, int B, int& h, int& w, View text_kv, int L, const float* tproj,
                  const SkipDst& dst, const SkipStat& stat, const CfgShare* share = nullptr);
    void run_mid(Ctx& c, View x, GnStatBuf* xs, int B, int h, int w, View text_kv, int L, const float* tproj, View dst);
};

struct ControlNet : Encoder {
    ControlNet(const sd_unet_config& c, int conditioning_channels);
    ~ControlNet();
    int finalize();

    int cond_channels = 3;
    bool finalized = false;
    static constexpr int kCondLayers = 7;
    float* cond_w[kCondLayers] = {};
    float* cond_b[kCondLayers] = {};
    int cond_cin[kCondLayers] = {}, cond_cout[kCondLayers] = {}, cond_stride[kCondLayers] = {};
    ConvW cond_out;
    std::vector<ConvW> zero;
    ConvW zero_mid;
    UNet* attached = nullptr;

    void run_cond_embed(Ctx& c, const half_t* image, int n, int H, int W, View out);
    int run(Ctx& c, const half_t* sample, const float* timesteps, View text_kv, int L, const half_t* add_text,
            const float* add_time_ids, int B, int H, int W, View emb, const std::vector<View>& sites, View mid);
};

bool unet_cfg_share_eligible(const sd_unet_config& cfg);

struct CfgIn {
    const half_t* latents = nullptr;
    float in_scale = 1.f;
};

struct UNet : Encoder {
    explicit UNet(const sd_unet_config& c);
    int finalize();
    int forward_cfg(const half_t* latents, const float* timesteps, const half_t* ehs, int L, const half_t* add_text,
                    const float* add_time_ids, const half_t* image_embeds, int n_img, float in_scale, bool share,
                    half_t* out, int B, int H, int W, hipStream_t stream);
    bool cfg_share_active(bool share) const;
    char* cfg_slab = nullptr;
    size_t cfg_cap = 0;
    int forward(const half_t* sample, const float* timesteps, const half_t* ehs, int L,
                const half_t* add_text, const float* add_time_ids, half_t* out, int B, int H, int W,
                hipStream_t stream, const half_t* image_embeds = nullptr, int n_img = 0,
                const half_t* control = nullptr, int n_ctrl = 0, float cn_scale = 0.f, const CfgIn* cfg_in = nullptr);
    void set_ip_adapter(IPAdapter* a);
    void set_controlnet(ControlNet* n);

    Arena arena;
    bool finalized = false;
    long planned_key = -1;
    long planned_cn = -1;

    bool graph_enabled = false;
    hipStream_t gstream = nullptr;
    hipEvent_t ev_in = nullptr, ev_out = nullptr;
    hipGraphExec_t gexec = nullptr;
    long graph_key = -1;
    char* io_slab = nullptr;
    size_t io_cap = 0;
    int forward_graph(const half_t* sample, const float* timesteps, const half_t* ehs, int L, const half_t* add_text,
                      const float* add_time_ids, half_t* out, int B, int H, int W, hipStream_t stream);
    ~UNet();

    bool kv_cache_on = false, kv_valid = false;
    half_t* kv_cache = nullptr;
    size_t kv_cap = 0;
    const half_t* kv_src = nullptr;
    int kv_B = 0, kv_L = 0;

    IPAdapter* ip = nullptr;
    float ip_scale = 1.f;
    bool ipkv_valid = false;
    half_t* ipkv_cache = nullptr;
    size_t ipkv_cap = 0;
    const half_t* ipkv_src = nullptr;
    int ipkv_B = 0, ipkv_n = 0;

    ControlNet* cn = nullptr;
    bool cond_valid = false, cnkv_valid = false;
    half_t* cond_cache = nullptr;
    size_t cond_cap = 0;
    const half_t* cond_src = nullptr;
    int cond_B = 0, cond_n = 0, cond_H = 0, cond_W = 0;
    half_t* cnkv_cache = nullptr;
    size_t cnkv_cap = 0;
    const half_t* cnkv_src = nullptr;
    int cnkv_B = 0, cnkv_L = 0;

    bool freeu_on = false;
    float freeu_s1 = 1.f, freeu_s2 = 1.f, freeu_b1 = 1.f, freeu_b2 = 1.f;

    ConvW conv_out;
    NormW norm_out;
    std::vector<std::vector<Resnet>> up_res;
    std::vector<std::vector<Xformer>> up_att;
    std::vector<ConvW> up_us;

  private:
    int run(Ctx& c, const half_t* sample, const float* timesteps, const half_t* ehs, int L,
            const half_t* add_text, const float* add_time_ids, half_t* out, int B, int H, int W,
            const half_t* image_embeds = nullptr, int n_img = 0, const half_t* control = nullptr, int n_ctrl = 0,
            float cn_scale = 0.f, const CfgIn* cfg_in = nullptr);
    int run_controlnet(Ctx& c, const half_t* sample, const float* timesteps, const half_t* ehs, int L,
                       const half_t* add_text, const float* add_time_ids, int B, int H, int W, const half_t* control,
                       int n_ctrl, const std::vector<View>& sites, View mid);
};

struct VAE {
    explicit VAE(const sd_vae_config& c);
    int finalize();
    int decode(const half_t* z, half_t* img, int B, int h, int w, hipStream_t stream);
    int encode(const half_t* img, half_t* moments, int B, int H, int W, hipStream_t stream);
    int encode_shift = 0;

    sd_vae_config cfg;
    WeightStore ws;
    Arena arena;
    bool finalized = false;
    long planned_key = -1;

    half_t* pq_w = nullptr; float* pq_b = nullptr;
    ConvW d_conv_in, d_conv_out;
    NormW d_norm_out;
    Resnet d_mid0, d_mid1;
    VaeAttn d_attn;
    std::vector<std::vector<Resnet>> d_up;
    std::vector<ConvW> d_us;
    half_t* q_w = nullptr; float* q_b = nullptr;
    ConvW e_conv_in, e_conv_out;
    NormW e_norm_out;
    Resnet e_mid0, e_mid1;
    VaeAttn e_attn;
    std::vector<std::vector<Resnet>> e_down;
    std::vector<ConvW> e_ds;

  private:
    int pack_resnet(const std::string& p, Resnet* r);
    int pack_attn(const std::string& p, VaeAttn* a);
    int pack_pointwise(const std::string& p, half_t** w, float** b);
    void run_attn(Ctx& c, const VaeAttn& a, View x, int N, int H, int W, View out, const GnStatBuf* x_stats,
                  GnStatBuf** out_stats, float stream_scale = 1.f);
    int run_decode(Ctx& c, const half_t* z, half_t* img, int B, int h, int w);
    int run_encode(Ctx& c, const half_t* img, half_t* moments, int B, int H, int W, float stream_scale);
};

struct ClipLayer {
    NormW ln1, ln2;
    ConvW qkv, out, fc1, fc2;
};
struct CLIP {
    explicit CLIP(const sd_clip_config& c);
    int finalize();
    int forward(const int* ids, const int* eos_index, half_t* hidden_states, half_t* last_hidden, half_t* pooled,
                half_t* text_embeds, int B, int T, hipStream_t stream);
    int final_layer_norm(const half_t* x, half_t* y, long rows, hipStream_t stream);

    sd_clip_config cfg;
    WeightStore ws;
    Arena arena;
    bool finalized = false;
    long planned_key = -1;
    half_t* tok = nullptr;
    half_t* pos = nullptr;
    half_t* proj = nullptr;
    std::vector<ClipLayer> layers;
    NormW final_ln;

  private:
    int run(Ctx& c, const int* ids, const int* eos_index, half_t* hidden_states, half_t* last_hidden, half_t* pooled,
            half_t* text_embeds, int B, int T);
};

}
```

stablediffusion_amd/csrc/runtime.cpp:

```cpp
#include "engine.h"

#include <atomic>
#include <cstdio>
#include <mutex>
#include <cstdlib>
#include <cstring>

namespace sd {

static thread_local std::string g_last_error;
void set_error(const std::string& msg) { g_last_error = msg; }
const std::string& last_error() { return g_last_error; }

Arena::~Arena() {
    if (base_) (void)hipFree(base_);
}

int Arena::reserve(size_t bytes) {
    if (bytes <= cap_) return 0;
    if (base_) { (void)hipFree(base_); base_ = nullptr; cap_ = 0; }
    SD_HIP_CHECK(hipMalloc(reinterpret_cast<void**>(&base_), bytes));
    cap_ = bytes;
    return 0;
}
// ... 301 lines not shown
    GnStatBuf* gn_out = fuse ? fuse->gn_out : nullptr;
    IGemmParams p;
    p.x = x.p; p.ldx = x.ld;
    p.w = w.w; p.bias = w.bias;
    p.rowadd = rowadd; p.rowadd_ld = rowadd_ld;
    p.res = res ? res->p : nullptr; p.ldres = res ? res->ld : 0;
    p.y = y.p; p.ldy = y.ld;
    p.N = N; p.H = H; p.W = W; p.Cin = (w.ks == 1) ? (int)w.K : w.cin;
    p.KS = w.ks; p.stride = stride; p.up = up;
    p.pad = pad >= 0 ? pad : (w.ks == 3 ? 1 : 0);
    const int IH = H << up, IW = W << up;
    if (stride == 1) {
        p.OH = IH; p.OW = IW;
    } else if (p.pad == 0) {
        p.OH = (IH + 1 - w.ks) / stride + 1; p.OW = (IW + 1 - w.ks) / stride + 1;
    } else {
        p.OH = (IH + 2 * p.pad - w.ks) / stride + 1; p.OW = (IW + 2 * p.pad - w.ks) / stride + 1;
    }
    p.Cout = w.cout;
    p.M = N * p.OH * p.OW;
    p.K = (int)w.K;
    p.geglu = geglu;
    p.act = act;
    if (ln_in) {
        if (!w.wsum) { set_error("op_conv: LayerNorm statistics passed to a linear without folded weights"); c.err = 1; return; }
        p.ln_stat = ln_in->p; p.ln_parts = ln_in->parts; p.ln_part_w = ln_in->width; p.ln_C = (int)w.K; p.ln_eps = ln_eps; p.ln_wsum = w.wsum;
    }
    if (fuse && fuse->gn_in) {
        p.gni_part = fuse->gn_in_stats.part; p.gni_S = fuse->gn_in_stats.S; p.gni_rows = fuse->gn_in_stats.rows;
        p.gni_groups = fuse->gn_in_groups; p.gni_eps = fuse->gn_in_eps; p.gni_silu = fuse->gn_in_silu;
        p.gni_gb = fuse->gn_in->gb;
        if (c.dry) p.gni_part = reinterpret_cast<const float*>(8);
    }
    if (fuse && (fuse->acc_scale != 1.f || fuse->bias_scale != 1.f)) { p.acc_scale = fuse->acc_scale; p.bias_scale = fuse->bias_scale; }
    const IGemmPlan plan = igemm2_plan(p, IGemmRequest{stat_out ? stat_out->p : nullptr, gn_out ? gn_out->buf : nullptr,
                                                       fuse ? fuse->gn_groups : 0});
    const bool v2 = plan.kind != kKindIgemm1;
    if ((p.acc_scale != 1.f || p.bias_scale != 1.f) && !plan.scales_ok) { set_error("op_conv: output scaling needs the LDS-DMA kernels (not GEGLU / weight-stationary)"); c.err = 1; return; }
    if (ln_in && !v2) { set_error("op_conv: the LayerNorm fold needs the LDS-DMA kernel"); c.err = 1; return; }
    if (act && !v2) { set_error("op_conv: activation epilogue needs the LDS-DMA kernel (Cin % 64, Cout % 8)"); c.err = 1; return; }
    if (gn_out) {
        gn_out->st = GnStats();
        if (plan.gnstats) { gn_out->st.part = gn_out->buf; gn_out->st.rows = plan.gn_rows; gn_out->st.S = p.OH * p.OW / plan.gn_rows; }
    }
    const bool own_stats = plan.rowstats;
    if (stat_out) { stat_out->parts = plan.rs_parts; stat_out->width = plan.rs_part_w; }
    float* partial = plan.partial_floats > 0 ? c.arena->alloc_f(plan.partial_floats) : nullptr;
    if (c.dry || c.err) return;
    if (prof_enabled()) {
        const double kreal = (double)w.ks * w.ks * w.cin;
        const double in_px = (double)N * H * W;
        const char* name = plan.name;
        static const bool by_shape = getenv("SD_PROF_SHAPES") != nullptr;
        char nbuf[64];
        if (v2 && by_shape) {
            snprintf(nbuf, sizeof(nbuf), "%s%d/k%d %dx%dx%d ks%d%s%s%s%s%s%s", plan.kind == kKindPgemmGeglu ? "pg" : "v", plan.variant,
                     plan.splits, p.M, p.Cout, p.K, p.KS, res ? " res" : "", geglu ? " geglu" : "", p.ln_stat ? " ln" : "",
                     p.rowstat_out ? " rs" : "", p.gnstat_out ? " gs" : "", p.gni_part ? " gn" : "");
            name = nbuf;
        }
        prof_open(c.stream, name, 2.0 * p.M * w.cout * kreal,
                  2.0 * (in_px * (w.ks == 1 ? (double)w.K : w.cin) + (double)w.cout * w.K +
                         (double)p.M * (geglu ? w.cout / 2 : w.cout) * (res ? 2 : 1)));
    }
    c.err = launch_igemm2(p, partial, c.stream, &plan);
    prof_close(c.stream);
    if (stat_out && !own_stats && !c.err) {
        prof_open(c.stream, "row_stats_kernel", 0.0, 2.0 * p.M * w.cout);
        c.err = launch_row_stats(y.p, y.ld, stat_out->p, p.M, w.cout, c.stream);
        prof_close(c.stream);
    }
}

void op_groupnorm(Ctx& c, const NormW& n, View x, View y, int N, long HW, int G, float eps, int silu,
                  const GnStatBuf* pre) {
    float* scratch = c.arena->alloc_f(gn_scratch_floats(N, HW, n.C, G));
    if (c.dry || c.err) return;
    const GnStats* st = (pre && pre->st.part && gn_wants_stats(HW, n.C, G)) ? &pre->st : nullptr;
    const bool own_pass = gn_wants_stats(HW, n.C, G) && !st;
    const char* gname = own_pass ? "groupnorm(stats+apply)" : "groupnorm(apply)";
    static thread_local char gbuf[64];
    static const bool gn_by_shape = getenv("SD_PROF_SHAPES") != nullptr;
    if (gn_by_shape && prof_enabled()) {
        snprintf(gbuf, sizeof(gbuf), "gn%s %ldx%d%s", own_pass ? "(stats+apply)" : (st ? "(apply)" : "(fused)"), (long)N * HW, n.C, silu ? " silu" : "");
        gname = gbuf;
    }
    prof_open(c.stream, gname, 0.0, (own_pass ? 6.0 : 4.0) * N * HW * n.C);
    c.err = launch_groupnorm(x.p, x.ld, n.gamma, n.beta, y.p, y.ld, N, HW, n.C, G, eps, silu, scratch, c.stream, st);
    prof_close(c.stream);
}

void op_gn_conv(Ctx& c, const NormW& n, const ConvW& w, View x, int N, int H, int W, View y, int G, float eps, int silu,
                const GnStatBuf* pre, const float* rowadd, int rowadd_ld, const View* res, const ConvFuse* fuse) {
    static const bool off = getenv("SD_GN_FUSE") == nullptr || getenv("SD_NO_GN_FUSE") != nullptr;
    const long HW = (long)H * W;
    IGemmParams q;
    q.x = x.p; q.ldx = x.ld; q.N = N; q.H = H; q.W = W; q.Cin = (w.ks == 1) ? (int)w.K : w.cin;
    q.KS = w.ks; q.stride = 1; q.up = 0; q.pad = w.ks == 3 ? 1 : 0; q.OH = H; q.OW = W; q.Cout = w.cout;
    q.M = N * H * W; q.K = (int)w.K;
    const bool fused = !off && n.gb && n.C == q.Cin && igemm2_gn_fusable(q, G);
    if (!fused) {
        const size_t mk = c.arena->mark();
        View hn(c.arena->alloc_h((long)N * HW * n.C), n.C, n.C);
        op_groupnorm(c, n, x, hn, N, HW, G, eps, silu, pre);
        op_conv(c, w, hn, N, H, W, y, 1, 0, rowadd, rowadd_ld, res, 0, -1, 0, fuse);
        c.arena->release(mk);
        return;
    }
    const size_t mk = c.arena->mark();
    ConvFuse f = fuse ? *fuse : ConvFuse();
    f.gn_in = &n; f.gn_in_groups = G; f.gn_in_eps = eps; f.gn_in_silu = silu;
    float* scratch = c.arena->alloc_f(gn_scratch_floats(N, HW, n.C, G) + (long)N * G * 2);
    if (pre && pre->st.part) {
        f.gn_in_stats = pre->st;
        if (f.gn_in_stats.S > 64 && !c.dry && !c.err) {
            prof_open(c.stream, "gn_finalize_kernel", 0.0, 8.0 * N * f.gn_in_stats.S * G);
            c.err = launch_gn_finalize(&f.gn_in_stats, scratch, N, HW, n.C, G, c.stream);
            prof_close(c.stream);
        }
    } else if (!c.dry && !c.err) {
        static thread_local char gbuf[64];
        static const bool by_shape = getenv("SD_PROF_SHAPES") != nullptr;
        const char* name = "groupnorm(stats)";
        if (by_shape && prof_enabled()) { snprintf(gbuf, sizeof(gbuf), "gn(stats) %ldx%d", (long)N * HW, n.C); name = gbuf; }
        prof_open(c.stream, name, 0.0, 2.0 * N * HW * n.C);
        c.err = launch_gn_stats(x.p, x.ld, N, HW, n.C, G, scratch, &f.gn_in_stats, c.stream);
        prof_close(c.stream);
    }
    op_conv(c, w, x, N, H, W, y, 1, 0, rowadd, rowadd_ld, res, 0, -1, 0, &f);
    c.arena->release(mk);
}

bool op_ffn_fused(Ctx& c, const ConvW& ff1, const ConvW& ff2, View x, const RowStat& x_stat, float ln_eps, long M, View y) {
    FfnParams p;
    p.x = x.p; p.ldx = x.ld; p.y = y.p; p.ldy = y.ld;
    p.w1 = ff1.w; p.b1 = ff1.bias; p.wsum1 = ff1.wsum;
    p.w1_rows = (int)(((long)ff1.cout + kWeightRowPad - 1) / kWeightRowPad * kWeightRowPad);
    p.w2 = ff2.w; p.b2 = ff2.bias;
    p.w2_rows = (int)(((long)ff2.cout + kWeightRowPad - 1) / kWeightRowPad * kWeightRowPad);
    p.ln_stat = x_stat.p; p.ln_parts = x_stat.parts; p.ln_part_w = x_stat.width; p.ln_eps = ln_eps;
    p.M = (int)M; p.C = (int)ff1.K; p.hidden = (int)ff2.K;
    if (c.dry) p.ln_stat = reinterpret_cast<const float*>(8);
    if (ff1.ks != 1 || ff2.ks != 1 || ff2.cout != ff1.K || ff1.cout != 2 * ff2.K || x.C != p.C || !ff1.wsum) return false;
    if (c.dry ? !(p.C == 320 && p.hidden == 1280 && M % 128 == 0 && M / 128 >= 64 && !getenv("SD_NO_FFN_FUSE")) : !ffn_fused_supported(p))
        return false;
    if (c.dry || c.err) return true;
    prof_open(c.stream, "ffn_fused_kernel", 2.0 * M * ((double)ff1.cout * ff1.K + (double)ff2.cout * ff2.K),
              2.0 * ((double)M * p.C * 2 + (double)ff1.cout * ff1.K + (double)ff2.cout * ff2.K));
    c.err = launch_ffn_fused(p, c.stream);
    prof_close(c.stream);
    return true;
}

void op_layernorm(Ctx& c, const NormW& n, View x, View y, long rows, float eps) {
    if (c.dry || c.err) return;
    prof_open(c.stream, "layernorm_kernel", 0.0, 4.0 * rows * n.C);
    c.err = launch_layernorm(x.p, x.ld, n.gamma, n.beta, y.p, y.ld, rows, n.C, eps, c.stream);
    prof_close(c.stream);
}

void op_attention(Ctx& c, View q, View k, View v, View out, int B, int Tq, int Tk, int heads, int d, int causal,
                  int prescaled) {
    if (c.dry || c.err) return;
    if (prof_enabled()) {
        static thread_local char name[32];
        snprintf(name, sizeof(name), "attn_kernel<%d>", d);
        prof_open(c.stream, name, 4.0 * B * heads * (double)Tq * Tk * d,
                  2.0 * B * heads * d * (2.0 * Tq + 2.0 * Tk));
    }
    c.err = launch_attention(q.p, k.p, v.p, out.p, B, Tq, Tk, heads, d, q.ld, k.ld, v.ld, out.ld, c.stream, causal, prescaled);
    prof_close(c.stream);
}

void op_ip_attention(Ctx& c, View q, View k, View v, View k_ip, View v_ip, View out, int B, int Tq, int L, int T_ip,
                     int heads, int d, float ip_scale) {
    if (c.dry || c.err) return;
    if (prof_enabled()) {
        static thread_local char name[32];
        snprintf(name, sizeof(name), "ip_xattn_kernel<%d>", d);
        prof_open(c.stream, name, 4.0 * B * heads * (double)Tq * (L + T_ip) * d,
                  2.0 * B * heads * d * (2.0 * Tq + 2.0 * L + 2.0 * T_ip));
    }
    c.err = launch_ip_attention(q.p, k.p, v.p, k_ip.p, v_ip.p, out.p, B, Tq, L, T_ip, heads, d, q.ld, k.ld, v.ld, k_ip.ld,
                                v_ip.ld, out.ld, ip_scale, 1, c.stream);
    prof_close(c.stream);
}

}
```

stablediffusion_amd/csrc/unet.cpp:

```cpp
#include <algorithm>
#include <vector>

#include "model.h"
#include <cmath>
#include <cstdlib>

namespace sd {

void declare_resnet(WeightStore& ws, const std::string& p, int cin, int cout, int temb) {
    ws.declare(p + ".norm1.weight", {cin});
    ws.declare(p + ".norm1.bias", {cin});
    ws.declare(p + ".conv1.weight", {cout, cin, 3, 3});
    ws.declare(p + ".conv1.bias", {cout});
    if (temb) {
        ws.declare(p + ".time_emb_proj.weight", {cout, temb});
        ws.declare(p + ".time_emb_proj.bias", {cout});
    }
    ws.declare(p + ".norm2.weight", {cout});
    ws.declare(p + ".norm2.bias", {cout});
    ws.declare(p + ".conv2.weight", {cout, cout, 3, 3});
    ws.declare(p + ".conv2.bias", {cout});
    if (cin != cout) {
        ws.declare(p + ".conv_shortcut.weight", {cout, cin, 1, 1});
        ws.declare(p + ".conv_shortcut.bias", {cout});
// ... 74 lines not shown
    declare_xformer(ws, "mid_block.attentions.0", mid, cfg.transformer_layers[nb - 1], ctx, lin);
    declare_resnet(ws, "mid_block.resnets.1", mid, mid, temb);
}

UNet::UNet(const sd_unet_config& c) : Encoder(c) {
    declare_encoder();
    const int nb = cfg.num_blocks;
    const int* boc = cfg.block_out_channels;
    const int temb = boc[0] * 4;
    const int ctx = cfg.cross_attention_dim;
    const bool lin = cfg.use_linear_projection != 0;
    int out_ch;
    out_ch = boc[nb - 1];
    for (int i = 0; i < nb; ++i) {
        const int prev = out_ch;
        out_ch = boc[nb - 1 - i];
        const int in_ch = boc[nb - 1 - (i + 1 < nb ? i + 1 : nb - 1)];
        const std::string p = "up_blocks." + std::to_string(i);
        for (int j = 0; j < cfg.layers_per_block + 1; ++j) {
            const int skip = (j == cfg.layers_per_block) ? in_ch : out_ch;
            const int rin = (j == 0) ? prev : out_ch;
            declare_resnet(ws, p + ".resnets." + std::to_string(j), rin + skip, out_ch, temb);
            if (cfg.up_block_has_attn[i])
                declare_xformer(ws, p + ".attentions." + std::to_string(j), out_ch,
                                cfg.transformer_layers[nb - 1 - i], ctx, lin);
        }
        if (i != nb - 1) {
            ws.declare(p + ".upsamplers.0.conv.weight", {out_ch, out_ch, 3, 3});
            ws.declare(p + ".upsamplers.0.conv.bias", {out_ch});
        }
    }
    ws.declare("conv_norm_out.weight", {boc[0]});
    ws.declare("conv_norm_out.bias", {boc[0]});
    ws.declare("conv_out.weight", {cfg.out_channels, boc[0], 3, 3});
    ws.declare("conv_out.bias", {cfg.out_channels});
}

int Encoder::pack_resnet(const std::string& p, Resnet* r, std::vector<std::string>* tw, std::vector<std::string>* tb) {
    int rc;
    if ((rc = ws.pack_norm(p + ".norm1", &r->n1))) return rc;
    if ((rc = ws.pack_conv(p + ".conv1", &r->c1))) return rc;
    if ((rc = ws.pack_norm(p + ".norm2", &r->n2))) return rc;
    if ((rc = ws.pack_conv(p + ".conv2", &r->c2))) return rc;
    r->cin = r->c1.cin; r->cout = r->c1.cout;
    r->has_sc = ws.raw(p + ".conv_shortcut.weight") != nullptr;
    if (r->has_sc && (rc = ws.pack_conv(p + ".conv_shortcut", &r->sc))) return rc;
    if (tw) {
        r->temb_off = temb_total;
        temb_total += r->cout;
        tw->push_back(p + ".time_emb_proj.weight");
        tb->push_back(p + ".time_emb_proj.bias");
    }
    return 0;
}

int Encoder::pack_xformer(const std::string& p, Xformer* x, int heads, int depth) {
    int rc;
    if ((rc = ws.pack_norm(p + ".norm", &x->gn))) return rc;
    if ((rc = ws.pack_conv(p + ".proj_in", &x->pin))) return rc;
    if ((rc = ws.pack_conv(p + ".proj_out", &x->pout))) return rc;
    x->C = x->pin.cout;
    x->heads = heads;
    x->blocks.resize((size_t)depth);
    for (int d = 0; d < depth; ++d) {
        TBlock& b = x->blocks[(size_t)d];
        const std::string q = p + ".transformer_blocks." + std::to_string(d);
        if ((rc = ws.pack_norm(q + ".norm1", &b.ln1))) return rc;
        if ((rc = ws.pack_norm(q + ".norm2", &b.ln2))) return rc;
        if ((rc = ws.pack_norm(q + ".norm3", &b.ln3))) return rc;
        if ((rc = ws.pack_rows({q + ".attn1.to_q.weight", q + ".attn1.to_k.weight", q + ".attn1.to_v.weight"}, {}, &b.qkv))) return rc;
        if ((rc = ws.pack_conv(q + ".attn1.to_out.0", &b.out1))) return rc;
        if ((rc = ws.pack_conv(q + ".attn2.to_q", &b.q2, false))) return rc;
        const float qs = 1.4426950408889634f / sqrtf((float)(x->C / heads));
        b.kv_off = kv_total;
        b.ip_kv_off = kv_total;
        kv_total += 2 * x->C;
        kv_keys.push_back(q + ".attn2.to_k.weight");
        kv_keys.push_back(q + ".attn2.to_v.weight");
        if ((rc = ws.pack_conv(q + ".attn2.to_out.0", &b.out2))) return rc;
        if ((rc = ws.pack_geglu(q + ".ff.net.0.proj", &b.ff1))) return rc;
        if ((rc = ws.pack_conv(q + ".ff.net.2", &b.ff2))) return rc;
        static const bool no_fold = getenv("SD_NO_LN_FOLD") != nullptr;
        b.fold = !no_fold;
        if (b.fold) {
            if ((rc = ws.fold_ln(&b.qkv, b.ln1, x->C, qs))) return rc;
            if ((rc = ws.fold_ln(&b.q2, b.ln2, x->C, qs))) return rc;
            if ((rc = ws.fold_ln(&b.ff1, b.ln3, 0, 1.0f))) return rc;
        } else {
            if ((rc = launch_scale_f16(b.qkv.w, (long)x->C * b.qkv.K, qs, 0))) return rc;
            if ((rc = launch_scale_f16(b.q2.w, (long)x->C * b.q2.K, qs, 0))) return rc;
        }
    }
    return 0;
}

int Encoder::pack_encoder(std::vector<std::string>* tw, std::vector<std::string>* tb) {
    const int nb = cfg.num_blocks;
    int rc;
    if ((rc = ws.pack_conv("conv_in", &conv_in))) return rc;
    if ((rc = ws.pack_conv("time_embedding.linear_1", &te1))) return rc;
    if ((rc = ws.pack_conv("time_embedding.linear_2", &te2))) return rc;
    if (cfg.addition_time_embed_dim > 0) {
        if ((rc = ws.pack_conv("add_embedding.linear_1", &ae1))) return rc;
        if ((rc = ws.pack_conv("add_embedding.linear_2", &ae2))) return rc;
    }
    down_res.assign((size_t)nb, {}); down_att.assign((size_t)nb, {}); down_ds.assign((size_t)nb, ConvW());
    for (int i = 0; i < nb; ++i) {
        const std::string p = "down_blocks." + std::to_string(i);
        down_res[i].resize((size_t)cfg.layers_per_block);
        if (cfg.down_block_has_attn[i]) down_att[i].resize((size_t)cfg.layers_per_block);
        for (int j = 0; j < cfg.layers_per_block; ++j) {
            if ((rc = pack_resnet(p + ".resnets." + std::to_string(j), &down_res[i][j], tw, tb))) return rc;
            if (cfg.down_block_has_attn[i] &&
                (rc = pack_xformer(p + ".attentions." + std::to_string(j), &down_att[i][j], cfg.num_heads[i],
                                   cfg.transformer_layers[i]))) return rc;
        }
        if (i != nb - 1 && (rc = ws.pack_conv(p + ".downsamplers.0.conv", &down_ds[i]))) return rc;
    }
    if ((rc = pack_resnet("mid_block.resnets.0", &mid_r0, tw, tb))) return rc;
    if ((rc = pack_xformer("mid_block.attentions.0", &mid_att, cfg.num_heads[nb - 1], cfg.transformer_layers[nb - 1]))) return rc;
    if ((rc = pack_resnet("mid_block.resnets.1", &mid_r1, tw, tb))) return rc;
    return 0;
}

int UNet::finalize() {
    if (finalized) return 0;
    std::string missing;
    if (!ws.complete(&missing)) { set_error("finalize: weight not set: " + missing); return 2; }
    const int nb = cfg.num_blocks;
    int rc;
    std::vector<std::string> tw, tb;
    temb_total = 0;
    kv_total = 0;
    kv_keys.clear();
    if ((rc = pack_encoder(&tw, &tb))) return rc;
    up_res.assign((size_t)nb, {}); up_att.assign((size_t)nb, {}); up_us.assign((size_t)nb, ConvW());
    for (int i = 0; i < nb; ++i) {
        const std::string p = "up_blocks." + std::to_string(i);
        up_res[i].resize((size_t)cfg.layers_per_block + 1);
        if (cfg.up_block_has_attn[i]) up_att[i].resize((size_t)cfg.layers_per_block + 1);
        for (int j = 0; j < cfg.layers_per_block + 1; ++j) {
            if ((rc = pack_resnet(p + ".resnets." + std::to_string(j), &up_res[i][j], &tw, &tb))) return rc;
            if (cfg.up_block_has_attn[i] &&
                (rc = pack_xformer(p + ".attentions." + std::to_string(j), &up_att[i][j], cfg.num_heads[nb - 1 - i],
                                   cfg.transformer_layers[nb - 1 - i]))) return rc;
        }
        if (i != nb - 1 && (rc = ws.pack_conv(p + ".upsamplers.0.conv", &up_us[i]))) return rc;
    }
    if ((rc = ws.pack_norm("conv_norm_out", &norm_out))) return rc;
    if ((rc = ws.pack_conv("conv_out", &conv_out))) return rc;
    if ((rc = ws.pack_rows(tw, tb, &temb_stack))) return rc;
    if (!kv_keys.empty() && (rc = ws.pack_rows(kv_keys, {}, &kv_all))) return rc;
    kv_keys.clear();
    SD_HIP_CHECK(hipDeviceSynchronize());
    ws.free_raw();
    finalized = true;
    return 0;
}

std::vector<std::pair<std::string, int>> unet_xattn_sites(const sd_unet_config& cfg, bool mid_last) {
    const int nb = cfg.num_blocks;
    const int* boc = cfg.block_out_channels;
    std::vector<std::pair<std::string, int>> down, up, mid;
    auto add = [](std::vector<std::pair<std::string, int>>& v, const std::string& p, int depth, int C) {
        for (int k = 0; k < depth; ++k) v.emplace_back(p + ".transformer_blocks." + std::to_string(k), C);
    };
    for (int i = 0; i < nb; ++i)
        if (cfg.down_block_has_attn[i])
            for (int j = 0; j < cfg.layers_per_block; ++j)
                add(down, "down_blocks." + std::to_string(i) + ".attentions." + std::to_string(j), cfg.transformer_layers[i], boc[i]);
    add(mid, "mid_block.attentions.0", cfg.transformer_layers[nb - 1], boc[nb - 1]);
    for (int i = 0; i < nb; ++i)
        if (cfg.up_block_has_attn[i])
            for (int j = 0; j < cfg.layers_per_block + 1; ++j)
                add(up, "up_blocks." + std::to_string(i) + ".attentions." + std::to_string(j),
                    cfg.transformer_layers[nb - 1 - i], boc[nb - 1 - i]);
    std::vector<std::pair<std::string, int>> all = down;
    const auto& second = mid_last ? up : mid;
    const auto& third = mid_last ? mid : up;
    all.insert(all.end(), second.begin(), second.end());
    all.insert(all.end(), third.begin(), third.end());
    return all;
}

namespace {
const char* kIpProj = "encoder_hid_proj.image_projection_layers.0";
}

IPAdapter::IPAdapter(const sd_unet_config& c, int image_embed_dim, int num_tokens)
    : cfg(c), d_img(image_embed_dim), n_tok(num_tokens) {
    const int ctx = cfg.cross_attention_dim;
    const std::string p = kIpProj;
    ws.declare(p + ".image_embeds.weight", {(int64_t)n_tok * ctx, d_img});
    ws.declare(p + ".image_embeds.bias", {(int64_t)n_tok * ctx});
    ws.declare(p + ".norm.weight", {ctx});
    ws.declare(p + ".norm.bias", {ctx});
    for (const auto& site : unet_xattn_sites(cfg, true)) {
        ws.declare(site.first + ".attn2.processor.to_k_ip.0.weight", {site.second, ctx});
        ws.declare(site.first + ".attn2.processor.to_v_ip.0.weight", {site.second, ctx});
    }
}

int IPAdapter::finalize() {
    if (finalized) return 0;
    std::string missing;
    if (!ws.complete(&missing)) { set_error("ip adapter finalize: weight not set: " + missing); return 2; }
    const std::string p = kIpProj;
    int rc;
    if ((rc = ws.pack_conv(p + ".image_embeds", &proj))) return rc;
    if ((rc = ws.pack_norm(p + ".norm", &norm))) return rc;
    std::vector<std::string> keys;
    kv_total = 0;
    for (const auto& site : unet_xattn_sites(cfg, false)) {
        keys.push_back(site.first + ".attn2.processor.to_k_ip.0.weight");
        keys.push_back(site.first + ".attn2.processor.to_v_ip.0.weight");
        kv_total += 2 * site.second;
    }
    if ((rc = ws.pack_rows(keys, {}, &kv_all))) return rc;
    SD_HIP_CHECK(hipDeviceSynchronize());
    ws.free_raw();
    finalized = true;
    return 0;
}

void UNet::set_ip_adapter(IPAdapter* a) {
    if (ip == a) return;
    if (ip) ip->attached = nullptr;
    if (a) {
        if (a->attached && a->attached != this) a->attached->set_ip_adapter(nullptr);
        a->attached = this;
    }
    ip = a;
    ipkv_valid = false;
    planned_key = -1;
}

void run_resnet(Ctx& c, const Resnet& r, View x, int N, int H, int W, View out, int G, float eps,
                const float* tproj, int tproj_ld, const GnStatBuf* x_stats, GnStatBuf** out_stats, float stream_scale,
                GnStatBuf* out_buf, int out_groups) {
    Arena& a = *c.arena;
    const size_t mk = a.mark();
    const long M = (long)N * H * W;
    const float s = stream_scale, eps_s = eps * s * s;
    View h2(a.alloc_h(M * r.cout), r.cout, r.cout);
    const long HW = (long)H * W;
    ConvFuse f1;
    f1.gn_out = gn_wants_stats(HW, r.cout, G) ? ctx_gnbuf(c) : nullptr;
    f1.gn_groups = G;
    f1.acc_scale = s; f1.bias_scale = s;
    op_gn_conv(c, r.n1, r.c1, x, N, H, W, h2, G, eps_s, 1, x_stats, tproj ? tproj + r.temb_off : nullptr, tproj_ld, nullptr, &f1);
    View res = x;
    if (r.has_sc) {
        res = View(a.alloc_h(M * r.cout), r.cout, r.cout);
        ConvFuse fs;
        fs.bias_scale = s;
        op_conv(c, r.sc, x, N, H, W, res, 1, 0, nullptr, 0, nullptr, 0, -1, 0, s != 1.f ? &fs : nullptr);
    }
    ConvFuse f2;
    f2.gn_out = (out_stats && gn_wants_stats(HW, r.cout, G)) ? (out_buf ? out_buf : ctx_gnbuf(c)) : nullptr;
    f2.gn_groups = out_groups > 0 ? out_groups : G;
    f2.acc_scale = s; f2.bias_scale = s;
    op_gn_conv(c, r.n2, r.c2, h2, N, H, W, out, G, eps_s, 1, f1.gn_out, nullptr, 0, &res, &f2);
    if (out_stats) *out_stats = f2.gn_out;
    a.release(mk);
}

void run_xformer(Ctx& c, const Xformer& t, View x, int N, int H, int W, View out, int G, View text_kv, int L,
                 const GnStatBuf* x_stats, GnStatBuf** out_stats, GnStatBuf* out_buf, int out_groups, const CfgShare* share) {
    Arena& a = *c.arena;
    const size_t mk = a.mark();
    const int C = t.C;
    const int T = H * W;
    const long M = (long)N * T;
    const int d = C / t.heads;
    const bool fold = !t.blocks.empty() && t.blocks[0].fold;
    int Np = share ? N / 2 : N;
    long Mp = (long)Np * T;
    View hn(a.alloc_h(M * C), C, C);
    op_groupnorm(c, t.gn, x, hn, Np, T, G, 1e-6f, 0, x_stats);
    View cur(a.alloc_h(M * C), C, C), nxt(a.alloc_h(M * C), C, C);
    RowStat st_cur, st_t2, st_t3;
    if (fold) {
        st_cur.p = a.alloc_f(rowstat_floats(M, C));
        st_t2.p = a.alloc_f(rowstat_floats(M, C));
        st_t3.p = a.alloc_f(rowstat_floats(M, C));
    }
    ConvFuse f_cur, f_t2, f_t3, f_ln1, f_ln2, f_ln3;
    f_cur.stat_out = &st_cur; f_t2.stat_out = &st_t2; f_t3.stat_out = &st_t3;
    f_ln1.ln_in = &st_cur; f_ln2.ln_in = &st_t2; f_ln3.ln_in = &st_t3;
    f_ln1.ln_eps = f_ln2.ln_eps = f_ln3.ln_eps = 1e-5f;
    op_conv(c, t.pin, hn, Np, H, W, cur, 1, 0, nullptr, 0, nullptr, 0, -1, 0, fold ? &f_cur : nullptr);
    for (size_t bi = 0; bi < t.blocks.size(); ++bi) {
        const TBlock& b = t.blocks[bi];
        const bool more = bi + 1 < t.blocks.size();
        const size_t mb = a.mark();
        View n(fold ? nullptr : a.alloc_h(M * C), C, C);
        View qkv(a.alloc_h(M * 3 * C), 3 * C, 3 * C);
        if (fold) {
            op_conv(c, b.qkv, cur, Np, H, W, qkv, 1, 0, nullptr, 0, nullptr, 0, -1, 0, &f_ln1);
        } else {
            op_layernorm(c, b.ln1, cur, n, Mp, 1e-5f);
            op_conv(c, b.qkv, n, Np, H, W, qkv);
        }
        View att(a.alloc_h(M * C), C, C);
        op_attention(c, qkv.slice(0, C), qkv.slice(C, C), qkv.slice(2 * C, C), att, Np, T, T, t.heads, d, 0, 1);
        View t2(a.alloc_h(M * C), C, C);
        op_conv(c, b.out1, att, Np, H, W, t2, 1, 0, nullptr, 0, &cur, 0, -1, 0, fold ? &f_t2 : nullptr);
        View q(a.alloc_h(M * C), C, C);
        if (fold) {
            op_conv(c, b.q2, t2, Np, H, W, q, 1, 0, nullptr, 0, nullptr, 0, -1, 0, &f_ln2);
        } else {
            op_layernorm(c, b.ln2, t2, n, Mp, 1e-5f);
            op_conv(c, b.q2, n, Np, H, W, q);
        }
        if (Np != N) {
            std::vector<RowDupSeg> segs = share->segs;
            for (const View& v : {q, t2, x}) {
                RowDupSeg g;
                g.src = v.p; g.dst = v.p + Mp * v.ld;
                g.ld_bytes = v.ld * 2; g.row_bytes = (long)v.C * 2; g.rows = Mp;
                segs.push_back(g);
            }
            if (!c.dry && !c.err) {
                double bytes = 0;
                for (const RowDupSeg& g : segs) bytes += 2.0 * g.rows * g.row_bytes;
                prof_open(c.stream, "row_dup_kernel", 0.0, bytes);
                c.err = launch_row_dup(segs.data(), (int)segs.size(), c.stream);
                prof_close(c.stream);
            }
            Np = N; Mp = M;
        }
        if (c.ip_kv.p && c.ip_scale != 0.f)
            op_ip_attention(c, q, text_kv.slice(b.kv_off, C), text_kv.slice(b.kv_off + C, C), c.ip_kv.slice(b.ip_kv_off, C),
                            c.ip_kv.slice(b.ip_kv_off + C, C), att, N, T, L, c.ip_T, t.heads, d, c.ip_scale);
        else
            op_attention(c, q, text_kv.slice(b.kv_off, C), text_kv.slice(b.kv_off + C, C), att, N, T, L, t.heads, d, 0, 1);
        View t3(a.alloc_h(M * C), C, C);
        op_conv(c, b.out2, att, N, H, W, t3, 1, 0, nullptr, 0, &t2, 0, -1, 0, fold ? &f_t3 : nullptr);
        if (!(fold && !more && op_ffn_fused(c, b.ff1, b.ff2, t3, st_t3, 1e-5f, M, nxt))) {
            View g(a.alloc_h(M * 4 * C), 4 * C, 4 * C);
            if (fold) {
                op_conv(c, b.ff1, t3, N, H, W, g, 1, 0, nullptr, 0, nullptr, 1, -1, 0, &f_ln3);
            } else {
                op_layernorm(c, b.ln3, t3, n, M, 1e-5f);
                op_conv(c, b.ff1, n, N, H, W, g, 1, 0, nullptr, 0, nullptr, 1);
            }
            op_conv(c, b.ff2, g, N, H, W, nxt, 1, 0, nullptr, 0, &t3, 0, -1, 0, (fold && more) ? &f_cur : nullptr);
        }
        a.release(mb);
        View tmp = cur; cur = nxt; nxt = tmp;
    }
    ConvFuse fo;
    fo.gn_out = (out_stats && gn_wants_stats(T, C, G)) ? (out_buf ? out_buf : ctx_gnbuf(c)) : nullptr;
    fo.gn_groups = out_groups > 0 ? out_groups : G;
    op_conv(c, t.pout, cur, N, H, W, out, 1, 0, nullptr, 0, &x, 0, -1, 0, &fo);
    if (out_stats) *out_stats = fo.gn_out;
    a.release(mk);
}

int Encoder::run_temb(Ctx& c, const float* timesteps, const half_t* add_text, const float* add_time_ids, int B,
                      float** tproj_out, int rows_alloc) {
    Arena& a = *c.arena;
    const int* boc = cfg.block_out_channels;
    const int temb = boc[0] * 4;
    hipStream_t s = c.stream;
    const bool go = !c.dry;
    float* sinus = a.alloc_f((long)B * boc[0]);
    float* e1 = a.alloc_f((long)B * temb);
    float* emb = a.alloc_f((long)B * temb);
    float* tproj = a.alloc_f((long)std::max(B, rows_alloc) * temb_total);
    *tproj_out = tproj;
    if (go && !c.err) c.err = launch_timestep_sinusoid(timesteps, 1, sinus, B, boc[0], cfg.flip_sin_to_cos, cfg.freq_shift, boc[0], s);
    if (go && !c.err) c.err = launch_small_linear(sinus, boc[0], te1.w, te1.bias, e1, temb, B, boc[0], temb, 0, 1, s);
    const bool aug_path = cfg.addition_time_embed_dim > 0;
    if (go && !c.err) c.err = launch_small_linear(e1, temb, te2.w, te2.bias, emb, temb, B, temb, temb, 0, aug_path ? 0 : 1, s);
    if (aug_path) {
        const int ad = cfg.addition_time_embed_dim;
        const int pin = cfg.projection_class_embeddings_input_dim;
        const int tdim = pin - 6 * ad;
        if (!add_text || !add_time_ids) { set_error("unet: add_text / add_time_ids required for text_time conditioning"); return 1; }
        float* addin = a.alloc_f((long)B * pin);
        float* a1 = a.alloc_f((long)B * temb);
        float* aug = a.alloc_f((long)B * temb);
        float* txt = a.alloc_f((long)B * tdim);
        if (go && !c.err) c.err = launch_f16_to_f32(add_text, txt, (long)B * tdim, s);
        if (go && !c.err) {
            hipError_t e = hipMemcpy2DAsync(addin, (size_t)pin * 4, txt, (size_t)tdim * 4, (size_t)tdim * 4, (size_t)B,
                                            hipMemcpyDeviceToDevice, s);
            if (e != hipSuccess) { set_error(hipGetErrorString(e)); c.err = 3; }
        }
        if (go && !c.err) {
            for (int j = 0; j < 6 && !c.err; ++j)
                c.err = launch_timestep_sinusoid(add_time_ids + j, 6, addin + tdim + j * ad, B, ad,
                                                         cfg.flip_sin_to_cos, cfg.freq_shift, pin, s);
        }
        if (go && !c.err) c.err = launch_small_linear(addin, pin, ae1.w, ae1.bias, a1, temb, B, pin, temb, 0, 1, s);
        if (go && !c.err) c.err = launch_small_linear(a1, temb, ae2.w, ae2.bias, aug, temb, B, temb, temb, 0, 0, s);
        if (go && !c.err) c.err = launch_add_f32(emb, aug, (long)B * temb, 1, s);
    }
    if (go && !c.err) c.err = launch_small_linear(emb, temb, temb_stack.w, temb_stack.bias, tproj, temb_total, B, temb, temb_total, 0, 0, s);

    return c.err;
}

void Encoder::run_conv_in(Ctx& c, const half_t* sample, int B, int H, int W, View y0, GnStatBuf* gb, const View* res,
                          GnStatBuf** xs) {
    Arena& a = *c.arena;
    const int* boc = cfg.block_out_channels;
    const int G = cfg.norm_num_groups;
    hipStream_t s = c.stream;
    const bool go = !c.dry;
    const size_t mk = a.mark();
    const long M = (long)B * H * W;
    HeadParams hp;
    hp.x_nchw = sample; hp.w = conv_in.w; hp.K = conv_in.K; hp.bias = conv_in.bias; hp.y = y0.p; hp.ldy = y0.ld;
    hp.gnstat_out = (gb && gb->buf) ? gb->buf : nullptr; hp.G = G;
    hp.N = B; hp.Cin = cfg.in_channels; hp.H = H; hp.W = W; hp.Cout = boc[0];
    if (!res && conv_head_supported(hp)) {
        if (gb) {
            gb->st = GnStats();
            if (hp.gnstat_out) { gb->st.part = gb->buf; gb->st.rows = 128; gb->st.S = (int)((long)H * W / 128); }
        }
        if (go && !c.err) {
            prof_open(s, "conv_head_kernel", 2.0 * M * boc[0] * 9.0 * cfg.in_channels, 2.0 * M * (boc[0] + cfg.in_channels));
            c.err = launch_conv_head(hp, s);
            prof_close(s);
        }
        *xs = gb;
    } else {
        half_t* col = a.alloc_h(M * conv_in.K);
        if (go && !c.err) c.err = launch_im2col_nchw3x3(sample, col, B, cfg.in_channels, H, W, (int)conv_in.K, s);
        ConvW pw = conv_in; pw.ks = 1;
        ConvFuse f;
        f.gn_out = gb;
        f.gn_groups = G;
        op_conv(c, pw, View(col, conv_in.K, (int)conv_in.K), B, H, W, y0, 1, 0, nullptr, 0, res, 0, -1, 0, &f);
        *xs = f.gn_out;
    }
    a.release(mk);
}

View Encoder::run_down(Ctx& c, View x, GnStatBuf*& xs, int B, int& h, int& w, View text_kv, int L, const float* tproj,
                       const SkipDst& skip_view, const SkipStat& skip_stat, const CfgShare* share) {
    Arena& a = *c.arena;
    const int nb = cfg.num_blocks;
    const int G = cfg.norm_num_groups;
    const float eps = cfg.norm_eps;
    int skip_i = 1;
    for (int i = 0; i < nb; ++i) {
        for (int j = 0; j < cfg.layers_per_block; ++j) {
            const Resnet& r = down_res[i][j];
            if (cfg.down_block_has_attn[i]) {
                const size_t mk = a.mark();
                View tmp(a.alloc_h((long)B * h * w * r.cout), r.cout, r.cout);
                GnStatBuf* rs = nullptr;
                const CfgShare* sh = (i == 0 && j == 0) ? share : nullptr;
                run_resnet(c, r, x, sh ? B / 2 : B, h, w, tmp, G, eps, tproj, temb_total, xs, &rs);
                View dst = skip_view(skip_i);
                run_xformer(c, down_att[i][j], tmp, B, h, w, dst, G, text_kv, L, rs, &xs, skip_stat(skip_i, (long)h * w, r.cout),
                            0, sh);
                a.release(mk);
                x = dst;
            } else {
                View dst = skip_view(skip_i);
                run_resnet(c, r, x, B, h, w, dst, G, eps, tproj, temb_total, xs, &xs, 1.f, skip_stat(skip_i, (long)h * w, r.cout));
                x = dst;
            }
            ++skip_i;
        }
        if (i != nb - 1) {
            ConvFuse f;
            f.gn_out = skip_stat(skip_i, (long)(h / 2) * (w / 2), down_ds[i].cout);
            View dst = skip_view(skip_i++);
            f.gn_groups = G;
            op_conv(c, down_ds[i], x, B, h, w, dst, 2, 0, nullptr, 0, nullptr, 0, -1, 0, &f);
            xs = f.gn_out;
            h /= 2; w /= 2;
            x = dst;
        }
    }

    return x;
}

void Encoder::run_mid(Ctx& c, View x, GnStatBuf* xs, int B, int h, int w, View text_kv, int L, const float* tproj,
                      View dst) {
    Arena& a = *c.arena;
    const int nb = cfg.num_blocks;
    const int* boc = cfg.block_out_channels;
    const int G = cfg.norm_num_groups;
    const float eps = cfg.norm_eps;
    const int C = boc[nb - 1];
    const long M = (long)B * h * w;
    View m0(a.alloc_h(M * C), C, C), m1(a.alloc_h(M * C), C, C);
    GnStatBuf *s0 = nullptr, *s1 = nullptr;
    run_resnet(c, mid_r0, x, B, h, w, m0, G, eps, tproj, temb_total, xs, &s0);
    run_xformer(c, mid_att, m0, B, h, w, m1, G, text_kv, L, s0, &s1);
    run_resnet(c, mid_r1, m1, B, h, w, dst, G, eps, tproj, temb_total, s1);
}

int Encoder::num_skips() const { return 1 + cfg.num_blocks * cfg.layers_per_block + (cfg.num_blocks - 1); }

int UNet::run(Ctx& c, const half_t* sample, const float* timesteps, const half_t* ehs, int L,
              const half_t* add_text, const float* add_time_ids, half_t* out, int B, int H, int W,
              const half_t* image_embeds, int n_img, const half_t* control, int n_ctrl, float cn_scale, const CfgIn* cfg_in) {
    Arena& a = *c.arena;
    const int nb = cfg.num_blocks;
    const int* boc = cfg.block_out_channels;
    const int G = cfg.norm_num_groups;
    const float eps = cfg.norm_eps;
    hipStream_t s = c.stream;
    const bool go = !c.dry;

    const int Bp = cfg_in ? B / 2 : B;
    CfgShare share;
    if (cfg_in) {
        const long n = (long)Bp * cfg.in_channels * H * W;
        half_t* scaled = a.alloc_h(n);
        sample = cfg_in->latents;
        if (cfg_in->in_scale != 1.f) {
            if (go && !c.err) c.err = launch_scale_copy_f16(cfg_in->latents, scaled, n, cfg_in->in_scale, s);
            sample = scaled;
        }
    }

    float* tproj = nullptr;
    if (int rc = run_temb(c, timesteps, add_text, add_time_ids, Bp, &tproj, B)) return rc;
    if (cfg_in) {
        RowDupSeg g;
        g.src = tproj; g.dst = tproj + (long)Bp * temb_total;
        g.ld_bytes = g.row_bytes = (long)Bp * temb_total * 4; g.rows = 1;
        share.segs.push_back(g);
    }

    const bool kv_cached = kv_cache_on && !graph_enabled && kv_cache != nullptr;
    View text_kv(kv_cached ? kv_cache : a.alloc_h((long)B * L * kv_total), kv_total, kv_total);
    if (!(kv_cached && kv_valid && kv_src == ehs && kv_B == B && kv_L == L)) {
        op_conv(c, kv_all, View(const_cast<half_t*>(ehs), cfg.cross_attention_dim, cfg.cross_attention_dim), B, L, 1, text_kv);
        if (kv_cached && go && !c.err) { kv_valid = true; kv_src = ehs; kv_B = B; kv_L = L; }
    }

    if (ip && image_embeds) {
        const int ctx = cfg.cross_attention_dim, T_ip = n_img * ip->n_tok;
        const long rows = (long)B * n_img, ntc = (long)ip->n_tok * ctx;
        const bool ip_cached = kv_cache_on && !graph_enabled && ipkv_cache != nullptr;
        View ip_kv(ip_cached ? ipkv_cache : a.alloc_h((long)B * T_ip * ip->kv_total), ip->kv_total, ip->kv_total);
        const bool hit = ip_cached && ipkv_valid && ipkv_src == image_embeds && ipkv_B == B && ipkv_n == n_img;
        if (c.dry || !hit) {
            const size_t mk = a.mark();
            float* e32 = a.alloc_f(rows * ip->d_img);
            float* p32 = a.alloc_f(rows * ntc);
            half_t* p16 = a.alloc_h(rows * ntc);
            half_t* tok = a.alloc_h(rows * ntc);
            if (go && !c.err) c.err = launch_f16_to_f32(image_embeds, e32, rows * ip->d_img, s);
            if (go && !c.err) {
                prof_open(s, "small_linear_kernel", 2.0 * rows * ntc * ip->d_img, 2.0 * ntc * ip->d_img);
                c.err = launch_small_linear(e32, ip->d_img, ip->proj.w, ip->proj.bias, p32, ntc, (int)rows, ip->d_img,
                                            (int)ntc, 0, 0, s);
                prof_close(s);
            }
            if (go && !c.err) c.err = launch_f32_to_f16(p32, p16, rows * ntc, s);
            op_layernorm(c, ip->norm, View(p16, ctx, ctx), View(tok, ctx, ctx), rows * ip->n_tok, 1e-5f);
            op_conv(c, ip->kv_all, View(tok, ctx, ctx), B, T_ip, 1, ip_kv);
            a.release(mk);
            if (ip_cached && go && !c.err) { ipkv_valid = true; ipkv_src = image_embeds; ipkv_B = B; ipkv_n = n_img; }
        }
        c.ip_kv = ip_kv;
        c.ip_T = T_ip;
        c.ip_scale = ip_scale;
    }

    struct Cat { half_t* p; int c1, c2, h, w; };
    std::vector<Cat> cats;
    {
        int out_ch = boc[nb - 1];
        int h = H >> (nb - 1), w = W >> (nb - 1);
        for (int i = 0; i < nb; ++i) {
            const int prev = out_ch;
            out_ch = boc[nb - 1 - i];
            const int in_ch = boc[nb - 1 - (i + 1 < nb ? i + 1 : nb - 1)];
            for (int j = 0; j < cfg.layers_per_block + 1; ++j) {
                Cat ct;
                ct.c2 = (j == cfg.layers_per_block) ? in_ch : out_ch;
                ct.c1 = (j == 0) ? prev : out_ch;
                ct.h = h; ct.w = w;
                ct.p = a.alloc_h((long)B * h * w * (ct.c1 + ct.c2));
                cats.push_back(ct);
            }
            if (i != nb - 1) { h *= 2; w *= 2; }
        }
    }
    const int nskip = (int)cats.size();
    int skip_i = 0;
    auto skip_view = [&](int si) {
        const Cat& ct = cats[(size_t)(nskip - 1 - si)];
        return View(ct.p + ct.c1, ct.c1 + ct.c2, ct.c2);
    };

    ctx_gnpool_init(c, B, (long)H * W, G);
    GnStatBuf* xs = nullptr;
    std::vector<GnStatBuf> sst((size_t)nskip);
    GnStatBuf hid;
    if (c.gnpool[0].buf) {
        for (auto& b : sst) b.buf = a.alloc_f(gnstat_floats(B, (long)H * W, G));
        hid.buf = a.alloc_f(gnstat_floats(B, (long)H * W, 128));
    }
    auto skip_stat = [&](int si, long HWs, int C) -> GnStatBuf* {
        return (sst[(size_t)si].buf && gn_wants_stats(HWs, C, G)) ? &sst[(size_t)si] : nullptr;
    };

    const bool use_cn = cn && control && cn_scale != 0.f && !cfg_in;
    const size_t cn_mark = a.mark();
    std::vector<View> cn_sites;
    std::vector<int> cn_rows;
    View cn_mid;
    if (use_cn) {
        int hh = H, ww = W;
        auto site = [&](int C) {
            cn_sites.emplace_back(a.alloc_h((long)B * hh * ww * C), C, C);
            cn_rows.push_back(B * hh * ww);
        };
        site(boc[0]);
        for (int i = 0; i < nb; ++i) {
            for (int j = 0; j < cfg.layers_per_block; ++j) site(boc[i]);
            if (i != nb - 1) { hh /= 2; ww /= 2; site(boc[i]); }
        }
        cn_mid = View(a.alloc_h((long)B * hh * ww * boc[nb - 1]), boc[nb - 1], boc[nb - 1]);
        cn_rows.push_back(B * hh * ww);
        GnStatBuf ring[Ctx::kGnPool];
        for (int i = 0; i < Ctx::kGnPool; ++i) ring[i] = c.gnpool[i];
        const int ring_next = c.gn_next, ring_groups = c.gn_groups;
        if (int rc = run_controlnet(c, sample, timesteps, ehs, L, add_text, add_time_ids, B, H, W, control, n_ctrl, cn_sites,
                                    cn_mid)) return rc;
        for (int i = 0; i < Ctx::kGnPool; ++i) c.gnpool[i] = ring[i];
        c.gn_next = ring_next; c.gn_groups = ring_groups;
    }

    int h = H, w = W;
    run_conv_in(c, sample, Bp, H, W, skip_view(skip_i), skip_stat(skip_i, (long)H * W, boc[0]), nullptr, &xs);
    View x = skip_view(skip_i++);
    if (cfg_in) {
        RowDupSeg g;
        g.src = x.p; g.dst = x.p + (long)Bp * H * W * x.ld;
        g.ld_bytes = x.ld * 2; g.row_bytes = (long)x.C * 2; g.rows = (long)Bp * H * W;
        share.segs.push_back(g);
    }

    x = run_down(c, x, xs, B, h, w, text_kv, L, tproj, [&](int si) { return skip_view(si); },
                 [&](int si, long HWs, int C) { return skip_stat(si, HWs, C); }, cfg_in ? &share : nullptr);

    run_mid(c, x, xs, B, h, w, text_kv, L, tproj, View(cats[0].p, cats[0].c1 + cats[0].c2, cats[0].c1));

    if (use_cn) {
        ConvFuse f;
        f.acc_scale = cn_scale; f.bias_scale = cn_scale;
        for (int si = 0; si <= nskip; ++si) {
            const View xh = si < nskip ? cn_sites[(size_t)si] : cn_mid;
            const View y = si < nskip ? skip_view(si) : View(cats[0].p, cats[0].c1 + cats[0].c2, cats[0].c1);
            const ConvW& zw = si < nskip ? cn->zero[(size_t)si] : cn->zero_mid;
            op_conv(c, zw, xh, 1, cn_rows[(size_t)si], 1, y, 1, 0, nullptr, 0, &y, 0, -1, 0, &f);
        }
    }
    if (use_cn) a.release(cn_mark);

    View final_x;
    int k = 0;
    const GnStatBuf* hid_ready = nullptr;
    int hid_groups = 0;
    static const bool no_cat_env = getenv("SD_GN_CAT") == nullptr;
    const bool no_cat_stats = no_cat_env || use_cn;
    for (int i = 0; i < nb; ++i) {
        for (int j = 0; j < cfg.layers_per_block + 1; ++j, ++k) {
            const Cat& ct = cats[(size_t)k];
            const Resnet& r = up_res[i][j];
            View xin(ct.p, ct.c1 + ct.c2, ct.c1 + ct.c2);
            const bool last_in_block = (j == cfg.layers_per_block);
            const bool fu = freeu_on && i < 2;
            const bool fu_next = freeu_on && (last_in_block ? i + 1 : i) < 2;
            if (fu && go && !c.err) {
                const double elems = (double)B * h * w * (ct.c1 / 2 + ct.c2);
                prof_open(s, "freeu_kernel", 16.0 * B * h * w * ct.c2, 4.0 * elems);
                c.err = launch_freeu(xin.p, xin.ld, B, h, w, ct.c1, ct.c2, i == 0 ? freeu_b1 : freeu_b2,
                                     i == 0 ? freeu_s1 : freeu_s2, s);
                prof_close(s);
            }
            const bool last = last_in_block && i == nb - 1;
            View dst;
            const size_t mk = a.mark();
            if (!last_in_block) {
                const Cat& nx = cats[(size_t)k + 1];
                dst = View(nx.p, nx.c1 + nx.c2, nx.c1);
            } else {
                dst = View(a.alloc_h((long)B * h * w * r.cout), r.cout, r.cout);
            }
            const long HWc = (long)h * w;
            const int Ccat = ct.c1 + ct.c2, si = nskip - 1 - k;
            GnStatBuf catst;
            const GnStatBuf* xin_stats = nullptr;
            if (!no_cat_stats && !fu && hid_ready && hid_ready->st.part && sst[(size_t)si].st.part && gn_wants_stats(HWc, Ccat, G) &&
                ct.c2 % G == 0 && (Ccat / G) % (ct.c2 / G) == 0 && ct.c1 % (ct.c2 / G) == 0) {
                float* fin = a.alloc_f((long)B * G * 2);
                if (go && !c.err) {
                    prof_open(s, "gn_cat_finalize_kernel", 0.0, 8.0 * B * (hid_ready->st.S * hid_groups + sst[(size_t)si].st.S * G));
                    c.err = launch_gn_cat_finalize(hid_ready->st, hid_groups, ct.c1, sst[(size_t)si].st, G, ct.c2, fin, B, HWc, G, s);
                    prof_close(s);
                }
                catst.buf = fin;
                catst.st.part = fin; catst.st.S = 1; catst.st.rows = HWc;
                xin_stats = &catst;
            }
            hid_ready = nullptr;
            int nx_groups = 0;
            if (!last && hid.buf && !no_cat_stats && !fu_next) {
                const Cat& nx = cats[(size_t)k + 1];
                const int u = gn_cat_unit(nx.c1, nx.c2, G);
                if (gn_wants_stats(last_in_block ? HWc * 4 : HWc, nx.c1 + nx.c2, G) && (u >= 8 || u == 4) && nx.c1 / u <= 128) nx_groups = nx.c1 / u;
            }
            const bool hid_here = nx_groups > 0 && !last_in_block;
            GnStatBuf* outp = nullptr;
            xs = nullptr;
            if (cfg.up_block_has_attn[i]) {
                View tmp(a.alloc_h((long)B * h * w * r.cout), r.cout, r.cout);
                GnStatBuf* rs = nullptr;
                run_resnet(c, r, xin, B, h, w, tmp, G, eps, tproj, temb_total, xin_stats, &rs);
                if (last) run_xformer(c, up_att[i][j], tmp, B, h, w, dst, G, text_kv, L, rs, &xs);
                else if (hid_here) run_xformer(c, up_att[i][j], tmp, B, h, w, dst, G, text_kv, L, rs, &outp, &hid, nx_groups);
                else run_xformer(c, up_att[i][j], tmp, B, h, w, dst, G, text_kv, L, rs, nullptr);
            } else {
                if (last) run_resnet(c, r, xin, B, h, w, dst, G, eps, tproj, temb_total, xin_stats, &xs);
                else if (hid_here) run_resnet(c, r, xin, B, h, w, dst, G, eps, tproj, temb_total, xin_stats, &outp, 1.f, &hid, nx_groups);
                else run_resnet(c, r, xin, B, h, w, dst, G, eps, tproj, temb_total, xin_stats, nullptr);
            }
            if (last) {
                final_x = dst;
            } else {
                if (last_in_block) {
                    const Cat& nx = cats[(size_t)k + 1];
                    View up_dst(nx.p, nx.c1 + nx.c2, nx.c1);
                    ConvFuse fu;
                    fu.gn_out = nx_groups > 0 ? &hid : nullptr;
                    fu.gn_groups = nx_groups;
                    op_conv(c, up_us[i], dst, B, h, w, up_dst, 1, 1, nullptr, 0, nullptr, 0, -1, 0, nx_groups > 0 ? &fu : nullptr);
                    outp = fu.gn_out;
                    h *= 2; w *= 2;
                }
                hid_ready = outp;
                hid_groups = nx_groups;
                a.release(mk);
            }
        }
    }

    {
        const int C = boc[0];
        const long M = (long)B * h * w;
        TailParams tp;
        tp.x = final_x.p; tp.ldx = final_x.ld;
        if (xs && xs->st.part) { tp.gn_part = xs->st.part; tp.gn_S = xs->st.S; tp.gn_rows = xs->st.rows; }
        tp.G = G; tp.eps = eps; tp.gamma = norm_out.gamma; tp.beta = norm_out.beta; tp.silu = 1;
        tp.w = conv_out.w; tp.K = conv_out.K; tp.bias = conv_out.bias; tp.y = out;
        tp.N = B; tp.H = h; tp.W = w; tp.C = C; tp.Cout = cfg.out_channels;
        if (go && !c.err && conv_tail_supported(tp)) {
            prof_open(s, "conv_tail_kernel", 2.0 * M * cfg.out_channels * 9.0 * C, 2.0 * M * (C + cfg.out_channels));
            c.err = launch_conv_tail(tp, s);
            prof_close(s);
            return c.err;
        }
        View hn(a.alloc_h(M * C), C, C);
        op_groupnorm(c, norm_out, final_x, hn, B, (long)h * w, G, eps, 1, xs);
        if (cfg.out_channels <= 4 && conv_out.ks == 3 && conv_out.K == 9L * C && M >= kSmallCoutMinPixels) {
            if (go && !c.err) {
                prof_open(s, "conv3x3_small_cout_kernel", 2.0 * M * cfg.out_channels * 9.0 * C, 2.0 * M * (C + cfg.out_channels));
                c.err = launch_conv3x3_small_cout(hn.p, hn.ld, conv_out.w, conv_out.K, conv_out.bias, out, B, h, w, C,
                                                  cfg.out_channels, s);
                prof_close(s);
            }
        } else {
            View y(a.alloc_h(M * cfg.out_channels), cfg.out_channels, cfg.out_channels);
            op_conv(c, conv_out, hn, B, h, w, y);
            if (go && !c.err) c.err = launch_nhwc_to_nchw(y.p, y.ld, out, B, (long)h * w, cfg.out_channels, s);
        }
    }
    return c.err;
}

UNet::~UNet() {
    if (gexec) (void)hipGraphExecDestroy(gexec);
    if (ev_in) (void)hipEventDestroy(ev_in);
    if (ev_out) (void)hipEventDestroy(ev_out);
    if (gstream) (void)hipStreamDestroy(gstream);
    if (io_slab) (void)hipFree(io_slab);
    if (kv_cache) (void)hipFree(kv_cache);
    if (ipkv_cache) (void)hipFree(ipkv_cache);
    if (cond_cache) (void)hipFree(cond_cache);
    if (cnkv_cache) (void)hipFree(cnkv_cache);
    if (cfg_slab) (void)hipFree(cfg_slab);
    if (ip) ip->attached = nullptr;
    if (cn) cn->attached = nullptr;
}

int UNet::forward_graph(const half_t* sample, const float* timesteps, const half_t* ehs, int L,
                        const half_t* add_text, const float* add_time_ids, half_t* out, int B, int H, int W,
                        hipStream_t stream) {
    const bool sdxl = cfg.addition_time_embed_dim > 0;
    const int pdim = sdxl ? cfg.projection_class_embeddings_input_dim - 6 * cfg.addition_time_embed_dim : 0;
    auto up = [](size_t v) { return (v + 255) & ~size_t(255); };
    const size_t n_sample = up((size_t)B * cfg.in_channels * H * W * 2), n_t = up((size_t)B * 4);
    const size_t n_ehs = up((size_t)B * L * cfg.cross_attention_dim * 2), n_text = up((size_t)B * pdim * 2);
    const size_t n_ids = up((size_t)B * 6 * 4), n_out = up((size_t)B * cfg.out_channels * H * W * 2);
    const size_t need = n_sample + n_t + n_ehs + n_text + n_ids + n_out;
    if (!gstream) {
        SD_HIP_CHECK(hipStreamCreateWithFlags(&gstream, hipStreamNonBlocking));
        SD_HIP_CHECK(hipEventCreateWithFlags(&ev_in, hipEventDisableTiming));
        SD_HIP_CHECK(hipEventCreateWithFlags(&ev_out, hipEventDisableTiming));
    }
    if (need > io_cap) {
        SD_HIP_CHECK(hipDeviceSynchronize());
        if (io_slab) (void)hipFree(io_slab);
        io_slab = nullptr; io_cap = 0; graph_key = -1;
        SD_HIP_CHECK(hipMalloc(reinterpret_cast<void**>(&io_slab), need));
        io_cap = need;
    }
    char* ptr = io_slab;
    half_t* g_sample = reinterpret_cast<half_t*>(ptr); ptr += n_sample;
    float* g_t = reinterpret_cast<float*>(ptr); ptr += n_t;
    half_t* g_ehs = reinterpret_cast<half_t*>(ptr); ptr += n_ehs;
    half_t* g_text = sdxl ? reinterpret_cast<half_t*>(ptr) : nullptr; ptr += n_text;
    float* g_ids = sdxl ? reinterpret_cast<float*>(ptr) : nullptr; ptr += n_ids;
    half_t* g_out = reinterpret_cast<half_t*>(ptr);
    SD_HIP_CHECK(hipMemcpyAsync(g_sample, sample, (size_t)B * cfg.in_channels * H * W * 2, hipMemcpyDeviceToDevice, stream));
    SD_HIP_CHECK(hipMemcpyAsync(g_t, timesteps, (size_t)B * 4, hipMemcpyDeviceToDevice, stream));
    SD_HIP_CHECK(hipMemcpyAsync(g_ehs, ehs, (size_t)B * L * cfg.cross_attention_dim * 2, hipMemcpyDeviceToDevice, stream));
    if (sdxl) {
        if (!add_text || !add_time_ids) { set_error("unet: add_text / add_time_ids required for text_time conditioning"); return 1; }
        SD_HIP_CHECK(hipMemcpyAsync(g_text, add_text, (size_t)B * pdim * 2, hipMemcpyDeviceToDevice, stream));
        SD_HIP_CHECK(hipMemcpyAsync(g_ids, add_time_ids, (size_t)B * 6 * 4, hipMemcpyDeviceToDevice, stream));
    }
    const long key = ((long)B << 40) ^ ((long)H << 20) ^ (long)W ^ ((long)L << 52);
    int rc = 0;
    if (key != graph_key || !gexec) {
        graph_enabled = false;
        rc = forward(g_sample, g_t, g_ehs, L, g_text, g_ids, g_out, B, H, W, stream);
        graph_enabled = true;
        if (rc) return rc;
        if (gexec) { (void)hipGraphExecDestroy(gexec); gexec = nullptr; }
        hipGraph_t graph = nullptr;
        SD_HIP_CHECK(hipStreamBeginCapture(gstream, hipStreamCaptureModeRelaxed));
        Ctx ctx{&arena, gstream, false};
        arena.begin(false);
        rc = run(ctx, g_sample, g_t, g_ehs, L, g_text, g_ids, g_out, B, H, W);
        hipError_t e = hipStreamEndCapture(gstream, &graph);
        if (rc) { if (graph) (void)hipGraphDestroy(graph); return rc; }
        if (e != hipSuccess) { set_error(std::string("hipStreamEndCapture: ") + hipGetErrorString(e)); return 3; }
        e = hipGraphInstantiate(&gexec, graph, nullptr, nullptr, 0);
        (void)hipGraphDestroy(graph);
        if (e != hipSuccess) { gexec = nullptr; set_error(std::string("hipGraphInstantiate: ") + hipGetErrorString(e)); return 3; }
        graph_key = key;
    } else {
        SD_HIP_CHECK(hipEventRecord(ev_in, stream));
        SD_HIP_CHECK(hipStreamWaitEvent(gstream, ev_in, 0));
        SD_HIP_CHECK(hipGraphLaunch(gexec, gstream));
        SD_HIP_CHECK(hipEventRecord(ev_out, gstream));
        SD_HIP_CHECK(hipStreamWaitEvent(stream, ev_out, 0));
    }
    SD_HIP_CHECK(hipMemcpyAsync(out, g_out, (size_t)B * cfg.out_channels * H * W * 2, hipMemcpyDeviceToDevice, stream));
    return 0;
}

int UNet::forward(const half_t* sample, const float* timesteps, const half_t* ehs, int L, const half_t* add_text,
                  const float* add_time_ids, half_t* out, int B, int H, int W, hipStream_t stream,
                  const half_t* image_embeds, int n_img, const half_t* control, int n_ctrl, float cn_scale, const CfgIn* cfg_in) {
    if (!finalized) { set_error("unet: forward before finalize"); return 2; }
    if (cfg_in && (B % 2 != 0 || graph_enabled || control || !unet_cfg_share_eligible(cfg))) {
        set_error("unet: shared CFG prefix not available for this call");
        return 2;
    }
    const int div = 1 << (cfg.num_blocks - 1);
    if (B <= 0 || H % div != 0 || W % div != 0) { set_error("unet: H and W must be divisible by 2^(blocks-1)"); return 1; }
    if (ip && !image_embeds) { set_error("unet: an IP-Adapter is attached: image_embeds required"); return 1; }
    if (!ip && image_embeds) { set_error("unet: image_embeds given but no IP-Adapter is attached"); return 1; }
    if (ip) {
        if (n_img < 1 || n_img * ip->n_tok > 64) { set_error("unet: images per prompt x adapter tokens must be in [1, 64]"); return 4; }
        if (L < 1 || L > 160) { set_error("unet: with an IP-Adapter the text length must be in [1, 160]"); return 4; }
        if (graph_enabled) { set_error("unet: graph replay with an IP-Adapter attached is not supported"); return 4; }
    } else {
        n_img = 0;
    }
    if (cn && !control) { set_error("unet: a ControlNet is attached: control image required"); return 1; }
    if (!cn && control) { set_error("unet: control image given but no ControlNet is attached"); return 1; }
    if (cn) {
        if (n_ctrl < 1 || B % n_ctrl != 0) { set_error("unet: the control image count must divide the batch"); return 1; }
        if (!(cn_scale == cn_scale)) { set_error("unet: conditioning scale is NaN"); return 1; }
        if (graph_enabled) { set_error("unet: graph replay with a ControlNet attached is not supported"); return 4; }
    } else {
        n_ctrl = 0;
        cn_scale = 0.f;
    }
    const bool use_cn = cn && cn_scale != 0.f;
    if (freeu_on && graph_enabled) { set_error("unet: graph replay with FreeU enabled is not supported"); return 4; }
    if (graph_enabled && !prof_enabled())
        return forward_graph(sample, timesteps, ehs, L, add_text, add_time_ids, out, B, H, W, stream);
    if (kv_cache_on) {
        const size_t need = (size_t)B * L * kv_total * sizeof(half_t);
        if (need > kv_cap) {
            SD_HIP_CHECK(hipDeviceSynchronize());
            if (kv_cache) (void)hipFree(kv_cache);
            kv_cache = nullptr; kv_cap = 0; kv_valid = false;
            SD_HIP_CHECK(hipMalloc(reinterpret_cast<void**>(&kv_cache), need));
            kv_cap = need;
        }
        if (ip) {
            const size_t ineed = (size_t)B * n_img * ip->n_tok * ip->kv_total * sizeof(half_t);
            if (ineed > ipkv_cap) {
                SD_HIP_CHECK(hipDeviceSynchronize());
                if (ipkv_cache) (void)hipFree(ipkv_cache);
                ipkv_cache = nullptr; ipkv_cap = 0; ipkv_valid = false;
                SD_HIP_CHECK(hipMalloc(reinterpret_cast<void**>(&ipkv_cache), ineed));
                ipkv_cap = ineed;
            }
        }
        if (use_cn) {
            const size_t cneed = (size_t)B * H * W * cn->cfg.block_out_channels[0] * sizeof(half_t);
            if (cneed > cond_cap) {
                SD_HIP_CHECK(hipDeviceSynchronize());
                if (cond_cache) (void)hipFree(cond_cache);
                cond_cache = nullptr; cond_cap = 0; cond_valid = false;
                SD_HIP_CHECK(hipMalloc(reinterpret_cast<void**>(&cond_cache), cneed));
                cond_cap = cneed;
            }
            const size_t kneed = (size_t)B * L * cn->kv_total * sizeof(half_t);
            if (kneed > cnkv_cap) {
                SD_HIP_CHECK(hipDeviceSynchronize());
                if (cnkv_cache) (void)hipFree(cnkv_cache);
                cnkv_cache = nullptr; cnkv_cap = 0; cnkv_valid = false;
                SD_HIP_CHECK(hipMalloc(reinterpret_cast<void**>(&cnkv_cache), kneed));
                cnkv_cap = kneed;
            }
        }
    }
    const long key = ((long)B << 40) ^ ((long)H << 20) ^ (long)W ^ ((long)L << 52) ^ (kv_cache_on ? (1L << 62) : 0) ^
                     (ip ? (long)(n_img * ip->n_tok) << 32 : 0) ^ (cfg_in ? (1L << 61) : 0);
    const long cn_key = use_cn ? n_ctrl : 0;
    if (key != planned_key || cn_key != planned_cn) {
        Ctx dry{&arena, stream, true};
        arena.begin(true);
        int rc = run(dry, sample, timesteps, ehs, L, add_text, add_time_ids, out, B, H, W, image_embeds, n_img, control,
                     n_ctrl, cn_scale, cfg_in);
        if (rc) return rc;
        if (arena.peak() > arena.capacity()) {
            SD_HIP_CHECK(hipDeviceSynchronize());
            rc = arena.reserve(arena.peak());
            if (rc) return rc;
        }
        planned_key = key;
        planned_cn = cn_key;
    }
    Ctx ctx{&arena, stream, false};
    arena.begin(false);
    int rc = run(ctx, sample, timesteps, ehs, L, add_text, add_time_ids, out, B, H, W, image_embeds, n_img, control, n_ctrl,
                 cn_scale, cfg_in);
    if (!rc && arena.overflow()) { set_error("unet: workspace overflow (planner bug)"); return 2; }
    return rc;
}

bool unet_cfg_share_eligible(const sd_unet_config& cfg) {
    return cfg.addition_time_embed_dim == 0 && cfg.num_blocks >= 1 && cfg.down_block_has_attn[0] != 0 &&
           cfg.transformer_layers[0] >= 1;
}

bool UNet::cfg_share_active(bool share) const {
    static const bool off = getenv("SD_NO_CFG_SHARE") != nullptr;
    static const bool gn_cat = getenv("SD_GN_CAT") != nullptr;
    return share && !off && !gn_cat && !graph_enabled && !cn && unet_cfg_share_eligible(cfg);
}

int UNet::forward_cfg(const half_t* latents, const float* timesteps, const half_t* ehs, int L, const half_t* add_text,
                      const float* add_time_ids, const half_t* image_embeds, int n_img, float in_scale, bool share,
                      half_t* out, int B, int H, int W, hipStream_t stream) {
    if (!finalized) { set_error("unet: forward before finalize"); return 2; }
    if (B <= 0 || H <= 0 || W <= 0) { set_error("unet: forward_cfg: empty batch"); return 1; }
    if (cfg_share_active(share)) {
        CfgIn in;
        in.latents = latents;
        in.in_scale = in_scale;
        return forward(nullptr, timesteps, ehs, L, add_text, add_time_ids, out, 2 * B, H, W, stream, image_embeds, n_img,
                       nullptr, 0, 0.f, &in);
    }
    const size_t n = (size_t)B * cfg.in_channels * H * W;
    const size_t lat_bytes = (2 * n * sizeof(half_t) + 255) & ~size_t(255), need = lat_bytes + 2 * (size_t)B * sizeof(float);
    if (need > cfg_cap) {
        SD_HIP_CHECK(hipDeviceSynchronize());
        if (cfg_slab) (void)hipFree(cfg_slab);
        cfg_slab = nullptr; cfg_cap = 0;
        SD_HIP_CHECK(hipMalloc(reinterpret_cast<void**>(&cfg_slab), need));
        cfg_cap = need;
    }
    half_t* lat2 = reinterpret_cast<half_t*>(cfg_slab);
    float* ts2 = reinterpret_cast<float*>(cfg_slab + lat_bytes);
    if (int rc = launch_cfg_duplicate(latents, lat2, (long)n, in_scale, stream)) return rc;
    if (int rc = launch_dup_f32(timesteps, ts2, B, stream)) return rc;
    return forward(lat2, ts2, ehs, L, add_text, add_time_ids, out, 2 * B, H, W, stream, image_embeds, n_img);
}

}
```

Before: 7.753 latents/s.

## Fuse cross-attention with folded LayerNorm, Q and out projections into one kernel

Adds a cross-attention path for the C=320, 8-head transformer blocks. Once per text embedding it precomputes K folded with the LN-folded Q weights, and V folded with the output projection. At runtime a single kernel then does LN via row stats, scores, softmax, the value/out-projection GEMM, bias, residual and output row stats. This removes the separate Q projection, attention and out-projection launches and their intermediate traffic at the largest resolution. In exchange it adds a cache keyed on the KV source and a large LDS footprint. The path is restricted to eligible sites (no IP-adapter, no ControlNet, KV cached).

```diff
diff --git a/include/sd_engine.h b/include/sd_engine.h
--- a/include/sd_engine.h
+++ b/include/sd_engine.h
@@ -225,6 +225,12 @@
                        int heads, int d, int ldq, int ldk, int ldv, int ldo, int causal, int prescaled,
                        void* stream);
 int sd_attention_plan(int B, int Tq, int Tk, int heads, int d, int causal, int prescaled, int* out5);
+int sd_op_xattn_folded(const void* x, int ldx, const float* stat, int parts, int part_w, const void* ln_gamma,
+                       const void* ln_beta, float ln_eps, const void* k, const void* v, int ldkv, const void* wq,
+                       const void* wo, const void* bo, void* y, int ldy, float* stat_out, int B, int rows_per_image, int L,
+                       int heads, int C, int iters, float* ms2, void* stream);
+int sd_xattn_plan(int C, int heads, int rows_per_image, int B, int L, int ln_fold, int kv_cached, int ip_active,
+                  int controlnet, int* out2);
 int sd_op_ip_cross_attention(const void* q, const void* k, const void* v, const void* k_ip, const void* v_ip, void* out,
                              int B, int Tq, int L, int T_ip, int heads, int d, int ldq, int ldk, int ldv, int ldk_ip,
                              int ldv_ip, int ldo, float ip_scale, int prescaled, int iters, float* ms_per_launch,
diff --git a/stablediffusion_amd/_lib.py b/stablediffusion_amd/_lib.py
--- a/stablediffusion_amd/_lib.py
+++ b/stablediffusion_amd/_lib.py
@@ -162,6 +162,9 @@
     "sd_op_layernorm": (_I, [_P, _P, _P, _P, _I, _I, _F, _P]),
     "sd_op_attention": (_I, [_P, _P, _P, _P, _I, _I, _I, _I, _I, _I, _I, _I, _I, _P]),
     "sd_attention_plan": (_I, [_I, _I, _I, _I, _I, _I, _I, C.POINTER(_I)]),
+    "sd_op_xattn_folded": (_I, [_P, _I, _P, _I, _I, _P, _P, _F, _P, _P, _I, _P, _P, _P, _P, _I, _P, _I, _I, _I, _I, _I, _I,
+                                C.POINTER(_F), _P]),
+    "sd_xattn_plan": (_I, [_I, _I, _I, _I, _I, _I, _I, _I, _I, C.POINTER(_I)]),
     "sd_op_ip_cross_attention": (_I, [_P, _P, _P, _P, _P, _P, _I, _I, _I, _I, _I, _I, _I, _I, _I, _I, _I, _I, _F, _I, _I,
                                       C.POINTER(_F), _P]),
     "sd_op_controlnet_residuals": (_I, [C.POINTER(SdCnProblem), _I, _F, _I, _I, C.POINTER(_F), _P]),
diff --git a/stablediffusion_amd/build.py b/stablediffusion_amd/build.py
--- a/stablediffusion_amd/build.py
+++ b/stablediffusion_amd/build.py
@@ -8,7 +8,7 @@
 HERE = os.path.dirname(os.path.abspath(__file__))
 CSRC = os.path.join(HERE, "csrc")
 OUT = os.path.join(HERE, "libsd_engine.so")
-SOURCES = ["igemm.hip", "igemm2.hip", "igemm3.hip", "wsgemm.hip", "pgemm.hip", "ffn.hip", "edge.hip", "norm.hip", "attention.hip", "ip_attention.hip", "controlnet.hip", "freeu.hip", "misc.hip", "probe.hip", "runtime.cpp", "unet.cpp", "controlnet.cpp", "vae.cpp", "clip.cpp", "capi.cpp"]
+SOURCES = ["igemm.hip", "igemm2.hip", "igemm3.hip", "wsgemm.hip", "pgemm.hip", "ffn.hip", "xattn.hip", "edge.hip", "norm.hip", "attention.hip", "ip_attention.hip", "controlnet.hip", "freeu.hip", "misc.hip", "probe.hip", "runtime.cpp", "unet.cpp", "controlnet.cpp", "vae.cpp", "clip.cpp", "capi.cpp"]
 FLAGS = ["-O3", "--offload-arch=gfx950", "-fPIC", "-std=c++17", "-Wall", "-Wno-unused-function",
          "-ffp-contract=fast", "-mllvm", "-amdgpu-mfma-vgpr-form"]
 
diff --git a/stablediffusion_amd/csrc/capi.cpp b/stablediffusion_amd/csrc/capi.cpp
--- a/stablediffusion_amd/csrc/capi.cpp
+++ b/stablediffusion_amd/csrc/capi.cpp
@@ -132,6 +132,7 @@
     if (!u) { set_error("null handle"); return SD_ERR_INVALID; }
     u->impl.kv_cache_on = enable != 0;
     u->impl.kv_valid = false;
+    u->impl.xf_valid = false;
     u->impl.ipkv_valid = false;
     u->impl.cond_valid = false;
     u->impl.cnkv_valid = false;
@@ -193,6 +194,7 @@
 int sd_unet_set_ip_adapter_scale(sd_unet* u, float scale) {
     if (!u) { set_error("null handle"); return SD_ERR_INVALID; }
     if (!(scale == scale)) { set_error("sd_unet_set_ip_adapter_scale: NaN"); return SD_ERR_INVALID; }
+    if ((u->impl.ip_scale != 0.f) != (scale != 0.f)) u->impl.planned_key = -1;
     u->impl.ip_scale = scale;
     return SD_OK;
 }
@@ -1107,6 +1109,89 @@
     return SD_OK;
 }
 
+int sd_xattn_plan(int C, int heads, int rows_per_image, int B, int L, int ln_fold, int kv_cached, int ip_active,
+                  int controlnet, int* out2) {
+    if (!out2) { set_error("sd_xattn_plan: null argument"); return SD_ERR_INVALID; }
+    XattnSite s;
+    s.C = C; s.heads = heads; s.rows_per_image = rows_per_image; s.B = B; s.L = L;
+    s.ln_fold = ln_fold != 0; s.kv_cached = kv_cached != 0; s.ip_active = ip_active != 0; s.controlnet = controlnet != 0;
+    out2[0] = xattn_fold_eligible(s) ? 1 : 0;
+    out2[1] = xattn_folded_shape_ok(C, heads, rows_per_image, B, L) ? 1 : 0;
+    return SD_OK;
+}
+
+int sd_op_xattn_folded(const void* x, int ldx, const float* stat, int parts, int part_w, const void* ln_gamma,
+                       const void* ln_beta, float ln_eps, const void* k, const void* v, int ldkv, const void* wq,
+                       const void* wo, const void* bo, void* y, int ldy, float* stat_out, int B, int rows_per_image, int L,
+                       int heads, int C, int iters, float* ms2, void* stream) {
+    hipStream_t s = static_cast<hipStream_t>(stream);
+    if (!x || !ln_gamma || !ln_beta || !k || !v || !wq || !wo || !bo || !y || (iters > 0 && !ms2)) {
+        set_error("sd_op_xattn_folded: bad arguments");
+        return SD_ERR_INVALID;
+    }
+    if (!xattn_folded_shape_ok(C, heads, rows_per_image, B, L) || ldx < C || ldy < C || ldx % 8 || ldy % 4 || ldkv < C) {
+        set_error("sd_op_xattn_folded: needs C = 320, 8 heads, rows per image % 128 == 0, 1 <= L <= 80");
+        return SD_ERR_UNSUPPORTED;
+    }
+    const long M = (long)B * rows_per_image;
+    const long rp = ((long)C + kWeightRowPad - 1) / kWeightRowPad * kWeightRowPad;
+    DevScope scope;
+    half_t *wqp = nullptr, *wop = nullptr, *kf = nullptr, *vf = nullptr;
+    float *nb = nullptr, *wsum = nullptr, *ks = nullptr, *kb = nullptr, *st = nullptr;
+    SD_DEV_ALLOC(scope, wqp, (size_t)rp * C * 2);
+    SD_DEV_ALLOC(scope, wop, (size_t)rp * C * 2);
+    SD_DEV_ALLOC(scope, nb, (size_t)rp * 4);
+    SD_DEV_ALLOC(scope, wsum, (size_t)rp * 4);
+    SD_DEV_ALLOC(scope, kf, (size_t)xattn_fold_kf_halves(B) * 2);
+    SD_DEV_ALLOC(scope, vf, (size_t)xattn_fold_vf_halves(B) * 2);
+    SD_DEV_ALLOC(scope, ks, (size_t)xattn_fold_aux_floats(B) * 4);
+    SD_DEV_ALLOC(scope, kb, (size_t)xattn_fold_aux_floats(B) * 4);
+    if (!stat) SD_DEV_ALLOC(scope, st, (size_t)M * 2 * 4);
+    SD_HIP_CHECK(hipMemsetAsync(wqp, 0, (size_t)rp * C * 2, s));
+    SD_HIP_CHECK(hipMemsetAsync(wop, 0, (size_t)rp * C * 2, s));
+    SD_HIP_CHECK(hipMemsetAsync(nb, 0, (size_t)rp * 4, s));
+    SD_HIP_CHECK(hipMemsetAsync(wsum, 0, (size_t)rp * 4, s));
+    SD_HIP_CHECK(hipMemcpyAsync(wqp, wq, (size_t)C * C * 2, hipMemcpyDeviceToDevice, s));
+    SD_HIP_CHECK(hipMemcpyAsync(wop, wo, (size_t)C * C * 2, hipMemcpyDeviceToDevice, s));
+    const float qs = 1.4426950408889634f / sqrtf((float)(C / heads));
+    int rc = launch_ln_fold(wqp, C, C, static_cast<const float*>(ln_gamma), static_cast<const float*>(ln_beta), nullptr, nb, wsum, C, qs, s);
+    if (!rc && !stat) rc = launch_row_stats(static_cast<const half_t*>(x), ldx, st, M, C, s);
+    if (rc) return rc;
+    XattnFoldParams fp;
+    fp.k = static_cast<const half_t*>(k); fp.ldk = ldkv; fp.v = static_cast<const half_t*>(v); fp.ldv = ldkv;
+    fp.wq = wqp; fp.bq = nb; fp.wo = wop;
+    fp.kf = kf; fp.vf = vf; fp.ks = ks; fp.kb = kb;
+    fp.B = B; fp.L = L; fp.C = C; fp.heads = heads;
+    XattnParams p;
+    p.x = static_cast<const half_t*>(x); p.ldx = ldx; p.y = static_cast<half_t*>(y); p.ldy = ldy;
+    p.kf = kf; p.vf = vf; p.ks = ks; p.kb = kb; p.bo = static_cast<const float*>(bo);
+    p.ln_stat = stat ? stat : st; p.ln_parts = stat ? parts : 1; p.ln_part_w = stat ? part_w : C; p.ln_eps = ln_eps;
+    p.stat_out = stat_out;
+    p.M = (int)M; p.B = B; p.rows_per_image = rows_per_image;
+    if (!xattn_folded_supported(p)) { set_error("sd_op_xattn_folded: unsupported problem"); return SD_ERR_UNSUPPORTED; }
+    hipEvent_t e0 = nullptr, e1 = nullptr, e2 = nullptr;
+    if (iters > 0) { SD_HIP_CHECK(hipEventCreate(&e0)); SD_HIP_CHECK(hipEventCreate(&e1)); SD_HIP_CHECK(hipEventCreate(&e2)); }
+    rc = launch_xattn_fold(fp, s);
+    if (!rc) rc = launch_xattn_folded(p, s);
+    if (!rc && iters > 0) {
+        SD_HIP_CHECK(hipEventRecord(e0, s));
+        rc = launch_xattn_fold(fp, s);
+        SD_HIP_CHECK(hipEventRecord(e1, s));
+        for (int it = 0; it < iters && !rc; ++it) rc = launch_xattn_folded(p, s);
+        SD_HIP_CHECK(hipEventRecord(e2, s));
+        SD_HIP_CHECK(hipEventSynchronize(e2));
+        float ms = 0.f;
+        SD_HIP_CHECK(hipEventElapsedTime(&ms, e1, e2));
+        ms2[0] = ms / (float)iters;
+        SD_HIP_CHECK(hipEventElapsedTime(&ms, e0, e1));
+        ms2[1] = ms;
+    }
+    if (e0) { (void)hipEventDestroy(e0); (void)hipEventDestroy(e1); (void)hipEventDestroy(e2); }
+    hipError_t e = hipStreamSynchronize(s);
+    if (!rc && e != hipSuccess) { set_error(hipGetErrorString(e)); rc = SD_ERR_HIP; }
+    return rc;
+}
+
 int sd_op_ip_cross_attention(const void* q, const void* k, const void* v, const void* k_ip, const void* v_ip, void* out,
                              int B, int Tq, int L, int T_ip, int heads, int d, int ldq, int ldk, int ldv, int ldk_ip,
                              int ldv_ip, int ldo, float ip_scale, int prescaled, int iters, float* ms_per_launch,
diff --git a/stablediffusion_amd/csrc/controlnet.cpp b/stablediffusion_amd/csrc/controlnet.cpp
--- a/stablediffusion_amd/csrc/controlnet.cpp
+++ b/stablediffusion_amd/csrc/controlnet.cpp
@@ -159,7 +159,9 @@
     }
     const View ip_kv = c.ip_kv;
     c.ip_kv = View();
+    c.in_controlnet = true;
     const int rc = cn->run(c, sample, timesteps, kv, L, add_text, add_time_ids, B, H, W, View(cond, C0, C0), sites, mid);
+    c.in_controlnet = false;
     c.ip_kv = ip_kv;
     return rc;
 }
diff --git a/stablediffusion_amd/csrc/engine.h b/stablediffusion_amd/csrc/engine.h
--- a/stablediffusion_amd/csrc/engine.h
+++ b/stablediffusion_amd/csrc/engine.h
@@ -74,6 +74,13 @@
     int C = 0;
 };
 
+struct XattnFolded {
+    half_t* kf = nullptr;
+    half_t* vf = nullptr;
+    float* ks = nullptr;
+    float* kb = nullptr;
+};
+
 struct RawTensor {
     std::vector<int64_t> shape;
     half_t* dev = nullptr;
@@ -118,6 +125,8 @@
     View ip_kv;
     int ip_T = 0;
     float ip_scale = 1.f;
+    const XattnFolded* xf = nullptr;
+    bool in_controlnet = false;
 };
 void ctx_gnpool_init(Ctx& c, int N, long HW_max, int G);
 GnStatBuf* ctx_gnbuf(Ctx& c);
@@ -141,6 +150,8 @@
                 const ConvFuse* fuse = nullptr);
 void op_layernorm(Ctx& c, const NormW& n, View x, View y, long rows, float eps);
 bool op_ffn_fused(Ctx& c, const ConvW& ff1, const ConvW& ff2, View x, const RowStat& x_stat, float ln_eps, long M, View y);
+void op_xattn_folded(Ctx& c, const XattnFolded& f, const ConvW& out2, View x, const RowStat& x_stat, float ln_eps, int B,
+                     long rows_per_image, View y, RowStat* y_stat);
 void op_attention(Ctx& c, View q, View k, View v, View out, int B, int Tq, int Tk, int heads, int d, int causal = 0,
                   int prescaled = 0);
 void op_ip_attention(Ctx& c, View q, View k, View v, View k_ip, View v_ip, View out, int B, int Tq, int L, int T_ip,
diff --git a/stablediffusion_amd/csrc/kernels.h b/stablediffusion_amd/csrc/kernels.h
--- a/stablediffusion_amd/csrc/kernels.h
+++ b/stablediffusion_amd/csrc/kernels.h
@@ -85,6 +85,42 @@
 bool ffn_fused_supported(const FfnParams& p);
 int launch_ffn_fused(const FfnParams& p, hipStream_t s);
 
+struct XattnFoldParams {
+    const half_t* k; long ldk;
+    const half_t* v; long ldv;
+    const half_t* wq; const float* bq;
+    const half_t* wo;
+    half_t* kf; half_t* vf; float* ks; float* kb;
+    int B, L, C, heads;
+};
+struct XattnParams {
+    const half_t* x; long ldx;
+    half_t* y; long ldy;
+    const half_t* kf; const half_t* vf; const float* ks; const float* kb;
+    const float* bo;
+    const float* ln_stat; int ln_parts; int ln_part_w; float ln_eps;
+    float* stat_out;
+    int M, B; long rows_per_image;
+};
+struct XattnSite {
+    int C = 0, heads = 0;
+    long rows_per_image = 0;
+    int B = 0, L = 0;
+    bool ln_fold = false;
+    bool kv_cached = false;
+    bool ip_active = false;
+    bool controlnet = false;
+};
+bool xattn_fold_switch_on();
+bool xattn_folded_shape_ok(int C, int heads, long rows_per_image, int B, int L);
+bool xattn_fold_eligible(const XattnSite& s);
+long xattn_fold_kf_halves(int B);
+long xattn_fold_vf_halves(int B);
+long xattn_fold_aux_floats(int B);
+int launch_xattn_fold(const XattnFoldParams& p, hipStream_t s);
+bool xattn_folded_supported(const XattnParams& p);
+int launch_xattn_folded(const XattnParams& p, hipStream_t s);
+
 long gn_scratch_floats(int N, long HW, int C, int G);
 struct GnStats {
     const float* part = nullptr;
diff --git a/stablediffusion_amd/csrc/model.h b/stablediffusion_amd/csrc/model.h
--- a/stablediffusion_amd/csrc/model.h
+++ b/stablediffusion_amd/csrc/model.h
@@ -21,6 +21,7 @@
     int kv_off = 0;
     int ip_kv_off = 0;
     bool fold = false;
+    int xf_site = -1;
 };
 struct Xformer {
     NormW gn;
@@ -163,6 +164,13 @@
     size_t kv_cap = 0;
     const half_t* kv_src = nullptr;
     int kv_B = 0, kv_L = 0;
+
+    std::vector<const TBlock*> xf_blocks;
+    std::vector<XattnFolded> xf_ops;
+    char* xf_cache = nullptr;
+    size_t xf_cap = 0;
+    bool xf_valid = false;
+    int xf_B = 0;
 
     IPAdapter* ip = nullptr;
     float ip_scale = 1.f;
diff --git a/stablediffusion_amd/csrc/runtime.cpp b/stablediffusion_amd/csrc/runtime.cpp
--- a/stablediffusion_amd/csrc/runtime.cpp
+++ b/stablediffusion_amd/csrc/runtime.cpp
@@ -477,6 +477,22 @@
     return true;
 }
 
+void op_xattn_folded(Ctx& c, const XattnFolded& f, const ConvW& out2, View x, const RowStat& x_stat, float ln_eps, int B,
+                     long rows_per_image, View y, RowStat* y_stat) {
+    if (y_stat) { y_stat->parts = 2; y_stat->width = 160; }
+    if (c.dry || c.err) return;
+    XattnParams p;
+    p.x = x.p; p.ldx = x.ld; p.y = y.p; p.ldy = y.ld;
+    p.kf = f.kf; p.vf = f.vf; p.ks = f.ks; p.kb = f.kb; p.bo = out2.bias;
+    p.ln_stat = x_stat.p; p.ln_parts = x_stat.parts; p.ln_part_w = x_stat.width; p.ln_eps = ln_eps;
+    p.stat_out = y_stat ? y_stat->p : nullptr;
+    p.B = B; p.rows_per_image = rows_per_image; p.M = (int)(B * rows_per_image);
+    const double M = (double)p.M;
+    prof_open(c.stream, "xattn_folded_kernel", 2.0 * M * 320.0 * (640.0 + 768.0), 2.0 * (M * 320.0 * 2 + B * 320.0 * (640.0 + 768.0)));
+    c.err = launch_xattn_folded(p, c.stream);
+    prof_close(c.stream);
+}
+
 void op_layernorm(Ctx& c, const NormW& n, View x, View y, long rows, float eps) {
     if (c.dry || c.err) return;
     prof_open(c.stream, "layernorm_kernel", 0.0, 4.0 * rows * n.C);
diff --git a/stablediffusion_amd/csrc/unet.cpp b/stablediffusion_amd/csrc/unet.cpp
--- a/stablediffusion_amd/csrc/unet.cpp
+++ b/stablediffusion_amd/csrc/unet.cpp
@@ -250,6 +250,14 @@
     if ((rc = ws.pack_rows(tw, tb, &temb_stack))) return rc;
     if (!kv_keys.empty() && (rc = ws.pack_rows(kv_keys, {}, &kv_all))) return rc;
     kv_keys.clear();
+    xf_blocks.clear();
+    auto sites = [&](Xformer& x) {
+        for (TBlock& b : x.blocks)
+            if (b.fold && xattn_folded_shape_ok(x.C, x.heads, 128, 1, 1)) { b.xf_site = (int)xf_blocks.size(); xf_blocks.push_back(&b); }
+    };
+    for (auto& v : down_att) for (Xformer& x : v) sites(x);
+    sites(mid_att);
+    for (auto& v : up_att) for (Xformer& x : v) sites(x);
     SD_HIP_CHECK(hipDeviceSynchronize());
     ws.free_raw();
     finalized = true;
@@ -405,7 +413,13 @@
         View t2(a.alloc_h(M * C), C, C);
         op_conv(c, b.out1, att, Np, H, W, t2, 1, 0, nullptr, 0, &cur, 0, -1, 0, fold ? &f_t2 : nullptr);
         View q(a.alloc_h(M * C), C, C);
-        if (fold) {
+        XattnSite xs;
+        xs.C = C; xs.heads = t.heads; xs.rows_per_image = T; xs.B = N; xs.L = L;
+        xs.ln_fold = fold; xs.kv_cached = c.xf != nullptr && b.xf_site >= 0;
+        xs.ip_active = c.ip_kv.p && c.ip_scale != 0.f; xs.controlnet = c.in_controlnet;
+        const bool folded = xattn_fold_eligible(xs);
+        if (folded) {
+        } else if (fold) {
             op_conv(c, b.q2, t2, Np, H, W, q, 1, 0, nullptr, 0, nullptr, 0, -1, 0, &f_ln2);
         } else {
             op_layernorm(c, b.ln2, t2, n, Mp, 1e-5f);
@@ -414,9 +428,16 @@
         if (Np != N) {
             std::vector<RowDupSeg> segs = share->segs;
             for (const View& v : {q, t2, x}) {
+                if (folded && v.p == q.p) continue;
                 RowDupSeg g;
                 g.src = v.p; g.dst = v.p + Mp * v.ld;
                 g.ld_bytes = v.ld * 2; g.row_bytes = (long)v.C * 2; g.rows = Mp;
+                segs.push_back(g);
+            }
+            if (folded) {
+                RowDupSeg g;
+                g.src = st_t2.p; g.dst = st_t2.p + Mp * st_t2.parts * 2;
+                g.ld_bytes = g.row_bytes = Mp * st_t2.parts * 2 * (long)sizeof(float); g.rows = 1;
                 segs.push_back(g);
             }
             if (!c.dry && !c.err) {
@@ -428,13 +449,15 @@
             }
             Np = N; Mp = M;
         }
-        if (c.ip_kv.p && c.ip_scale != 0.f)
+        View t3(a.alloc_h(M * C), C, C);
+        if (folded)
+            op_xattn_folded(c, c.xf[b.xf_site], b.out2, t2, st_t2, 1e-5f, N, T, t3, &st_t3);
+        else if (c.ip_kv.p && c.ip_scale != 0.f)
             op_ip_attention(c, q, text_kv.slice(b.kv_off, C), text_kv.slice(b.kv_off + C, C), c.ip_kv.slice(b.ip_kv_off, C),
                             c.ip_kv.slice(b.ip_kv_off + C, C), att, N, T, L, c.ip_T, t.heads, d, c.ip_scale);
         else
             op_attention(c, q, text_kv.slice(b.kv_off, C), text_kv.slice(b.kv_off + C, C), att, N, T, L, t.heads, d, 0, 1);
-        View t3(a.alloc_h(M * C), C, C);
-        op_conv(c, b.out2, att, N, H, W, t3, 1, 0, nullptr, 0, &t2, 0, -1, 0, fold ? &f_t3 : nullptr);
+        if (!folded) op_conv(c, b.out2, att, N, H, W, t3, 1, 0, nullptr, 0, &t2, 0, -1, 0, fold ? &f_t3 : nullptr);
         if (!(fold && !more && op_ffn_fused(c, b.ff1, b.ff2, t3, st_t3, 1e-5f, M, nxt))) {
             View g(a.alloc_h(M * 4 * C), 4 * C, 4 * C);
             if (fold) {
@@ -636,6 +659,26 @@
     if (!(kv_cached && kv_valid && kv_src == ehs && kv_B == B && kv_L == L)) {
         op_conv(c, kv_all, View(const_cast<half_t*>(ehs), cfg.cross_attention_dim, cfg.cross_attention_dim), B, L, 1, text_kv);
         if (kv_cached && go && !c.err) { kv_valid = true; kv_src = ehs; kv_B = B; kv_L = L; }
+        if (go) xf_valid = false;
+    }
+    c.xf = nullptr;
+    if (kv_cached && xf_cache && xf_B == B && !xf_blocks.empty() && xattn_fold_switch_on() && xattn_folded_shape_ok(320, 8, 128, B, L)) {
+        if (go && !c.err && !xf_valid) {
+            for (size_t i = 0; i < xf_blocks.size() && !c.err; ++i) {
+                const TBlock& tb = *xf_blocks[i];
+                XattnFoldParams fp;
+                fp.k = text_kv.p + tb.kv_off; fp.ldk = text_kv.ld;
+                fp.v = text_kv.p + tb.kv_off + 320; fp.ldv = text_kv.ld;
+                fp.wq = tb.q2.w; fp.bq = tb.q2.bias; fp.wo = tb.out2.w;
+                fp.kf = xf_ops[i].kf; fp.vf = xf_ops[i].vf; fp.ks = xf_ops[i].ks; fp.kb = xf_ops[i].kb;
+                fp.B = B; fp.L = L; fp.C = 320; fp.heads = 8;
+                prof_open(s, "xattn_fold_kernel", 2.0 * B * 40.0 * 320.0 * (640.0 + 768.0), 2.0 * B * 320.0 * (640.0 + 768.0));
+                c.err = launch_xattn_fold(fp, s);
+                prof_close(s);
+            }
+            if (!c.err) xf_valid = true;
+        }
+        c.xf = xf_ops.data();
     }
 
     if (ip && image_embeds) {
@@ -889,6 +932,7 @@
     if (gstream) (void)hipStreamDestroy(gstream);
     if (io_slab) (void)hipFree(io_slab);
     if (kv_cache) (void)hipFree(kv_cache);
+    if (xf_cache) (void)hipFree(xf_cache);
     if (ipkv_cache) (void)hipFree(ipkv_cache);
     if (cond_cache) (void)hipFree(cond_cache);
     if (cnkv_cache) (void)hipFree(cnkv_cache);
@@ -1003,9 +1047,31 @@
         if (need > kv_cap) {
             SD_HIP_CHECK(hipDeviceSynchronize());
             if (kv_cache) (void)hipFree(kv_cache);
-            kv_cache = nullptr; kv_cap = 0; kv_valid = false;
+            kv_cache = nullptr; kv_cap = 0; kv_valid = false; xf_valid = false;
             SD_HIP_CHECK(hipMalloc(reinterpret_cast<void**>(&kv_cache), need));
             kv_cap = need;
+        }
+        if (!xf_blocks.empty() && xattn_fold_switch_on() && !graph_enabled && (xf_B != B || !xf_cache)) {
+            const size_t kfb = (size_t)xattn_fold_kf_halves(B) * 2, vfb = (size_t)xattn_fold_vf_halves(B) * 2;
+            const size_t axb = ((size_t)xattn_fold_aux_floats(B) * 4 + 255) & ~size_t(255);
+            const size_t site = kfb + vfb + 2 * axb, need_xf = site * xf_blocks.size();
+            if (need_xf > xf_cap) {
+                SD_HIP_CHECK(hipDeviceSynchronize());
+                if (xf_cache) (void)hipFree(xf_cache);
+                xf_cache = nullptr; xf_cap = 0;
+                SD_HIP_CHECK(hipMalloc(reinterpret_cast<void**>(&xf_cache), need_xf));
+                xf_cap = need_xf;
+            }
+            xf_ops.resize(xf_blocks.size());
+            for (size_t i = 0; i < xf_blocks.size(); ++i) {
+                char* base = xf_cache + i * site;
+                xf_ops[i].kf = reinterpret_cast<half_t*>(base);
+                xf_ops[i].vf = reinterpret_cast<half_t*>(base + kfb);
+                xf_ops[i].ks = reinterpret_cast<float*>(base + kfb + vfb);
+                xf_ops[i].kb = reinterpret_cast<float*>(base + kfb + vfb + axb);
+            }
+            xf_B = B;
+            xf_valid = false;
         }
         if (ip) {
             const size_t ineed = (size_t)B * n_img * ip->n_tok * ip->kv_total * sizeof(half_t);
diff --git a/stablediffusion_amd/csrc/xattn.hip b/stablediffusion_amd/csrc/xattn.hip
--- /dev/null
+++ b/stablediffusion_amd/csrc/xattn.hip
@@ -0,0 +1,345 @@
+#include <cstdlib>
+
+#include "kernels.h"
+
+namespace sd {
+namespace {
+
+constexpr int XA_C = 320, XA_BM = 128, XA_HEADS = 8, XA_D = 40, XA_SLOTS = 80, XA_HID = XA_HEADS * XA_SLOTS;
+constexpr int XA_VK = 96, XA_VLD = XA_HEADS * XA_VK;
+constexpr int XA_STAGES = 5;
+constexpr int kXaMaxLnParts = 20;
+constexpr float kXaMasked = -1e30f;
+
+template <int N>
+__device__ __forceinline__ void xa_wait_vmcnt() {
+    asm volatile("s_waitcnt vmcnt(%0)" ::"n"(N) : "memory");
+}
+
+struct XaLds {
+    static constexpr int STAGE = 160 * 64 * 2;
+    static constexpr int RING = XA_STAGES * STAGE;
+    static constexpr int H = 3 * XA_BM * 64 * 2;
+    static constexpr int AUX = 2 * XA_HID * 4;
+    static constexpr int STAT = XA_BM * 2 * 4;
+    static constexpr int TOTAL = RING + H + AUX + STAT;
+};
+
+__global__ __launch_bounds__(320) void xattn_fold_kernel(XattnFoldParams p) {
+    __shared__ float sk[XA_D];
+    __shared__ float red[320 / 64];
+    const int b = blockIdx.y, t = threadIdx.x;
+    if (blockIdx.x < XA_HID) {
+        const int r = blockIdx.x, h = r / XA_SLOTS, j = r % XA_SLOTS;
+        half_t* dst = p.kf + ((long)b * XA_HID + r) * XA_C;
+        if (j >= p.L) {
+            dst[t] = (half_t)0.f;
+            if (t == 0) { p.ks[(long)b * XA_HID + r] = 0.f; p.kb[(long)b * XA_HID + r] = kXaMasked; }
+            return;
+        }
+        if (t < XA_D) sk[t] = (float)p.k[((long)b * p.L + j) * p.ldk + h * XA_D + t];
+        __syncthreads();
+        float acc = 0.f;
+#pragma unroll 8
+        for (int d = 0; d < XA_D; ++d) acc += sk[d] * (float)p.wq[(long)(h * XA_D + d) * XA_C + t];
+        const half_t o = (half_t)acc;
+        dst[t] = o;
+        float s = (float)o;
+#pragma unroll
+        for (int m = 32; m >= 1; m >>= 1) s += __shfl_xor(s, m);
+        if ((t & 63) == 0) red[t >> 6] = s;
+        __syncthreads();
+        if (t == 0) {
+            float ks = 0.f, kb = 0.f;
+            for (int w = 0; w < 320 / 64; ++w) ks += red[w];
+            for (int d = 0; d < XA_D; ++d) kb += sk[d] * p.bq[h * XA_D + d];
+            p.ks[(long)b * XA_HID + r] = ks;
+            p.kb[(long)b * XA_HID + r] = kb;
+        }
+    } else {
+        const int oc = blockIdx.x - XA_HID;
+        half_t* dst = p.vf + ((long)b * XA_C + oc) * XA_VLD;
+        for (int col = t; col < XA_VLD; col += 320) {
+            const int h = col / XA_VK, j = col % XA_VK;
+            float acc = 0.f;
+            if (j < p.L && j < XA_SLOTS) {
+                const half_t* vr = p.v + ((long)b * p.L + j) * p.ldv + h * XA_D;
+                const half_t* wr = p.wo + (long)oc * XA_C + h * XA_D;
+#pragma unroll 8
+                for (int d = 0; d < XA_D; ++d) acc += (float)vr[d] * (float)wr[d];
+            }
+            dst[col] = (half_t)acc;
+        }
+    }
+}
+
+__global__ __launch_bounds__(512) void xattn_folded_kernel(XattnParams p) {
+#if defined(__HIP_DEVICE_COMPILE__)
+    constexpr unsigned kOOB = 0x80000000u;
+    constexpr int BM = XA_BM, C = XA_C, NKS = XA_C / 64, NVS = 6, STAGES = XA_STAGES, LA = STAGES - 1, NSTEP = XA_HEADS / 2;
+    constexpr int TM = 2;
+    constexpr int STAGE_HALVES = XaLds::STAGE / 2;
+    extern __shared__ __attribute__((aligned(16))) char smem[];
+    half_t* ring = reinterpret_cast<half_t*>(smem);
+    half_t* sH = reinterpret_cast<half_t*>(smem + XaLds::RING);
+    float* sAux = reinterpret_cast<float*>(smem + XaLds::RING + XaLds::H);
+    float* sStat = reinterpret_cast<float*>(smem + XaLds::RING + XaLds::H + XaLds::AUX);
+
+    const int tid = threadIdx.x, lane = tid & 63;
+    const int wave = __builtin_amdgcn_readfirstlane(tid >> 6);
+    const int wm = wave >> 1, wn = wave & 1;
+    const int fr = lane & 15, fq = lane >> 4;
+    const int bid = xcd_remap(blockIdx.x, gridDim.x);
+    const int m0 = bid * BM;
+    const int img = m0 / p.rows_per_image;
+
+    h8 xf[TM][2 * NKS];
+#pragma unroll
+    for (int i = 0; i < TM; ++i) {
+        const half_t* xr = p.x + (long)(m0 + wm * 32 + i * 16 + fr) * p.ldx + fq * 8;
+#pragma unroll
+        for (int ks = 0; ks < 2 * NKS; ++ks) xf[i][ks] = *reinterpret_cast<const h8*>(xr + ks * 32);
+    }
+    if (tid < BM) {
+        float2 pv[kXaMaxLnParts];
+        const float2* src = reinterpret_cast<const float2*>(p.ln_stat) + (long)(m0 + tid) * p.ln_parts;
+#pragma unroll
+        for (int k = 0; k < kXaMaxLnParts; ++k) pv[k] = src[k < p.ln_parts ? k : p.ln_parts - 1];
+        float mean, rstd;
+        ln_row_stats(pv, p.ln_parts, p.ln_part_w, C, p.ln_eps, mean, rstd);
+        sStat[tid * 2] = mean;
+        sStat[tid * 2 + 1] = rstd;
+    }
+    for (int t = tid; t < 2 * XA_HID; t += 512)
+        sAux[t] = t < XA_HID ? p.ks[(long)img * XA_HID + t] : p.kb[(long)img * XA_HID + t - XA_HID];
+    {
+        const int pr = tid >> 2, w = tid & 3;
+        const int slab = 1 + (w >> 1), ch = (w >> 1) * 4 + 2 + (w & 1);
+        *reinterpret_cast<h8*>(sH + slab * (BM * 64) + pr * 64 + ((ch ^ (pr & 7)) << 3)) = h8{0, 0, 0, 0, 0, 0, 0, 0};
+    }
+    __syncthreads();
+
+    __amdgpu_buffer_rsrc_t rk = __builtin_amdgcn_make_buffer_rsrc(const_cast<half_t*>(p.kf + (long)img * XA_HID * C), 0, XA_HID * C * 2, 0x00020000);
+    __amdgpu_buffer_rsrc_t rv = __builtin_amdgcn_make_buffer_rsrc(const_cast<half_t*>(p.vf + (long)img * C * XA_VLD), 0, C * XA_VLD * 2, 0x00020000);
+    const int lrow = lane >> 3;
+    const int chunk = (lane & 7) ^ (lrow & 7);
+
+    int s_it = 0, s_q = 0, s_slot = 0;
+    auto issue = [&]() {
+        half_t* dst = ring + s_slot * STAGE_HALVES;
+        const bool live = s_it < NSTEP;
+        const bool isk = s_q < NKS;
+        const int w = s_q - NKS;
+        const unsigned sb = isk ? (unsigned)((s_it * 160 * C + s_q * 64) * 2)
+                                : (unsigned)(((w & 1) * 80 * XA_VLD + s_it * 2 * XA_VK + (w >> 1) * 64) * 2);
+#pragma unroll
+        for (int j = 0; j < 3; ++j)
+            if (wave + 8 * j < 20) {
+                const int r = (wave + 8 * j) * 8 + lrow;
+                const unsigned k_off = (unsigned)((r * C + chunk * 8) * 2);
+                const unsigned v_off = (unsigned)(((160 * (r / 80) + (r % 80)) * XA_VLD + chunk * 8) * 2);
+                if (isk)
+                    __builtin_amdgcn_raw_ptr_buffer_load_lds(rk, (__attribute__((address_space(3))) void*)(dst + (wave + 8 * j) * 512), 16,
+                                                             live ? k_off + sb : kOOB, 0, 0, 0);
+                else
+                    __builtin_amdgcn_raw_ptr_buffer_load_lds(rv, (__attribute__((address_space(3))) void*)(dst + (wave + 8 * j) * 512), 16,
+                                                             live ? v_off + sb : kOOB, 0, 0, 0);
+            }
+        if (++s_q == NKS + NVS) { s_q = 0; ++s_it; }
+        if (++s_slot == STAGES) s_slot = 0;
+    };
+#pragma unroll
+    for (int s = 0; s < LA; ++s) issue();
+
+    f4 acc1[TM][5], acc2[2][TM][5];
+#pragma unroll
+    for (int i = 0; i < TM; ++i)
+#pragma unroll
+        for (int j = 0; j < 5; ++j) {
+            acc1[i][j] = f4{0.f, 0.f, 0.f, 0.f};
+            acc2[0][i][j] = f4{0.f, 0.f, 0.f, 0.f};
+            acc2[1][i][j] = f4{0.f, 0.f, 0.f, 0.f};
+        }
+
+    int lb[2];
+#pragma unroll
+    for (int ks = 0; ks < 2; ++ks) lb[ks] = fr * 64 + (((ks * 4 + fq) ^ (fr & 7)) << 3);
+    const int rowH = wm * 32 * 64, rowB = wn * 80 * 64;
+    int c_slot = 0;
+    auto slab_begin = [&]() -> const half_t* {
+        if (wave < 4) xa_wait_vmcnt<3 * (LA - 1)>(); else xa_wait_vmcnt<2 * (LA - 1)>();
+        asm volatile("s_waitcnt lgkmcnt(0)" ::: "memory");
+        __builtin_amdgcn_s_barrier();
+        issue();
+        const half_t* cB = ring + c_slot * STAGE_HALVES;
+        if (++c_slot == STAGES) c_slot = 0;
+        return cB;
+    };
+
+#pragma unroll 1
+    for (int it = 0; it < NSTEP; ++it) {
+#pragma unroll
+        for (int q = 0; q < NKS; ++q) {
+            const half_t* cB = slab_begin();
+#pragma unroll
+            for (int ks = 0; ks < 2; ++ks) {
+                h8 fb[5];
+#pragma unroll
+                for (int j = 0; j < 5; ++j) fb[j] = *reinterpret_cast<const h8*>(cB + rowB + j * 1024 + lb[ks]);
+#pragma unroll
+                for (int i = 0; i < TM; ++i)
+#pragma unroll
+                    for (int j = 0; j < 5; ++j)
+                        acc1[i][j] = __builtin_amdgcn_mfma_f32_16x16x32_f16(fb[j], xf[i][q * 2 + ks], acc1[i][j], 0, 0, 0);
+            }
+        }
+        {
+            int fr_ = fr, fq_ = fq;
+            asm volatile("" : "+v"(fr_), "+v"(fq_));
+            const float* ax = sAux + (it * 2 + wn) * XA_SLOTS + fq_ * 4;
+#pragma unroll
+            for (int i = 0; i < TM; ++i) {
+                const int pr = wm * 32 + i * 16 + fr_;
+                const float2 mr = *reinterpret_cast<const float2*>(sStat + pr * 2);
+                float mx = -3.0e38f;
+#pragma unroll
+                for (int j = 0; j < 5; ++j) {
+                    const f4 ks4 = *reinterpret_cast<const f4*>(ax + j * 16), kb4 = *reinterpret_cast<const f4*>(ax + XA_HID + j * 16);
+                    acc1[i][j] = (acc1[i][j] - mr.x * ks4) * mr.y + kb4;
+#pragma unroll
+                    for (int e = 0; e < 4; ++e) mx = fmaxf(mx, acc1[i][j][e]);
+                }
+                mx = fmaxf(mx, __shfl_xor(mx, 16));
+                mx = fmaxf(mx, __shfl_xor(mx, 32));
+                float sum = 0.f;
+#pragma unroll
+                for (int j = 0; j < 5; ++j)
+#pragma unroll
+                    for (int e = 0; e < 4; ++e) {
+                        acc1[i][j][e] = __builtin_amdgcn_exp2f(acc1[i][j][e] - mx);
+                        sum += acc1[i][j][e];
+                    }
+                sum += __shfl_xor(sum, 16);
+                sum += __shfl_xor(sum, 32);
+                const float inv = 1.0f / sum;
+#pragma unroll
+                for (int j = 0; j < 5; ++j) {
+                    h4 o;
+#pragma unroll
+                    for (int e = 0; e < 4; ++e) o[e] = (half_t)(acc1[i][j][e] * inv);
+                    acc1[i][j] = f4{0.f, 0.f, 0.f, 0.f};
+                    const int k = wn * XA_VK + j * 16 + fq_ * 4;
+                    const int kl = k & 63;
+                    *reinterpret_cast<h4*>(sH + (k >> 6) * (BM * 64) + pr * 64 + (((kl >> 3) ^ (pr & 7)) << 3) + (kl & 7)) = o;
+                }
+            }
+        }
+#pragma unroll
+        for (int kc = 0; kc < 3; ++kc) {
+#pragma unroll
+            for (int s = 0; s < 2; ++s) {
+                const half_t* cB = slab_begin();
+#pragma unroll
+                for (int ks = 0; ks < 2; ++ks) {
+                    h8 fa[TM], fb[5];
+#pragma unroll
+                    for (int i = 0; i < TM; ++i) fa[i] = *reinterpret_cast<const h8*>(sH + kc * (BM * 64) + rowH + i * 1024 + lb[ks]);
+#pragma unroll
+                    for (int j = 0; j < 5; ++j) fb[j] = *reinterpret_cast<const h8*>(cB + rowB + j * 1024 + lb[ks]);
+#pragma unroll
+                    for (int i = 0; i < TM; ++i)
+#pragma unroll
+                        for (int j = 0; j < 5; ++j)
+                            acc2[s][i][j] = __builtin_amdgcn_mfma_f32_16x16x32_f16(fb[j], fa[i], acc2[s][i][j], 0, 0, 0);
+                }
+            }
+        }
+    }
+    xa_wait_vmcnt<0>();
+
+#pragma unroll
+    for (int i = 0; i < TM; ++i) {
+        const long m = m0 + wm * 32 + i * 16 + fr;
+        float pv = 0.f, ss = 0.f, qq = 0.f;
+#pragma unroll
+        for (int s = 0; s < 2; ++s) {
+#pragma unroll
+            for (int j = 0; j < 5; ++j) {
+                const int col = 160 * wn + 80 * s + j * 16 + fq * 4;
+                const f4 bo = *reinterpret_cast<const f4*>(p.bo + col);
+                const f4 v = acc2[s][i][j] + bo;
+                const h4 xr = *reinterpret_cast<const h4*>(p.x + m * p.ldx + col);
+                h4 o;
+#pragma unroll
+                for (int e = 0; e < 4; ++e) o[e] = (half_t)((float)(half_t)v[e] + (float)xr[e]);
+                *reinterpret_cast<h4*>(p.y + m * p.ldy + col) = o;
+                if (s == 0 && j == 0) pv = (float)o[0];
+#pragma unroll
+                for (int e = 0; e < 4; ++e) { const float d = (float)o[e] - pv; ss += d; qq += d * d; }
+            }
+        }
+        const float a = ss * (1.0f / 40.0f);
+        float n = 40.f, mean = pv + a, m2 = qq - ss * a;
+#pragma unroll
+        for (int sh = 16; sh <= 32; sh <<= 1) {
+            const float om = __shfl_xor(mean, sh), oq = __shfl_xor(m2, sh);
+            stat_merge(n, mean, m2, n, om, oq);
+        }
+        if (p.stat_out && fq == 0) *reinterpret_cast<float2*>(p.stat_out + (m * 2 + wn) * 2) = float2{mean, m2};
+    }
+#endif
+}
+
+}
+
+bool xattn_fold_switch_on() {
+    static const bool off = getenv("SD_NO_XATTN_FOLD") != nullptr;
+    return !off;
+}
+
+bool xattn_folded_shape_ok(int C, int heads, long rows_per_image, int B, int L) {
+    return C == XA_C && heads == XA_HEADS && B >= 1 && rows_per_image >= XA_BM && rows_per_image % XA_BM == 0 && L >= 1 &&
+           L <= XA_SLOTS && (long)B * rows_per_image * XA_C * 2 < (1L << 31);
+}
+
+bool xattn_fold_eligible(const XattnSite& s) {
+    return xattn_fold_switch_on() && xattn_folded_shape_ok(s.C, s.heads, s.rows_per_image, s.B, s.L) &&
+           (long)s.B * s.rows_per_image / XA_BM >= 64 && s.ln_fold && s.kv_cached && !s.ip_active && !s.controlnet;
+}
+
+long xattn_fold_kf_halves(int B) { return (long)B * XA_HID * XA_C; }
+long xattn_fold_vf_halves(int B) { return (long)B * XA_C * XA_VLD; }
+long xattn_fold_aux_floats(int B) { return (long)B * XA_HID; }
+
+int launch_xattn_fold(const XattnFoldParams& p, hipStream_t s) {
+    if (!xattn_folded_shape_ok(p.C, p.heads, XA_BM, p.B, p.L) || !p.k || !p.v || !p.wq || !p.bq || !p.wo || !p.kf || !p.vf ||
+        !p.ks || !p.kb || p.ldk < XA_C || p.ldv < XA_C) {
+        set_error("xattn_fold: unsupported problem");
+        return 1;
+    }
+    hipLaunchKernelGGL(xattn_fold_kernel, dim3(XA_HID + XA_C, p.B), dim3(320), 0, s, p);
+    SD_HIP_CHECK(hipGetLastError());
+    return 0;
+}
+
+bool xattn_folded_supported(const XattnParams& p) {
+    return p.B >= 1 && p.rows_per_image >= XA_BM && p.rows_per_image % XA_BM == 0 && (long)p.M == (long)p.B * p.rows_per_image &&
+           p.x && p.y && p.kf && p.vf && p.ks && p.kb && p.bo && p.ln_stat && p.ln_parts >= 1 && p.ln_parts <= kXaMaxLnParts &&
+           p.ldx >= XA_C && p.ldy >= XA_C && p.ldx % 8 == 0 && p.ldy % 4 == 0 && (long)p.M * p.ldx * 2 < (1L << 31) &&
+           (long)p.M * p.ldy * 2 < (1L << 31);
+}
+
+int launch_xattn_folded(const XattnParams& p, hipStream_t s) {
+    if (!xattn_folded_supported(p)) { set_error("xattn_folded: unsupported problem"); return 1; }
+    static_assert(XaLds::TOTAL <= 160 * 1024, "LDS budget");
+    static PerDeviceOnce attr_once;
+    if (attr_once.first()) {
+        SD_HIP_CHECK(hipFuncSetAttribute(reinterpret_cast<const void*>(&xattn_folded_kernel),
+                                         hipFuncAttributeMaxDynamicSharedMemorySize, XaLds::TOTAL));
+    }
+    hipLaunchKernelGGL(xattn_folded_kernel, dim3(p.M / XA_BM), dim3(512), XaLds::TOTAL, s, p);
+    SD_HIP_CHECK(hipGetLastError());
+    return 0;
+}
+
+}
```

Result: no change. 7.790 latents/s (median of 6 runs) (+0.5%).
